# WGLab/NanoRepeat

Measured on NVIDIA B200. Metric: GCUPS, higher is better.
Workload: dtype u16x2 (2*score + mark + 64 per half, two reads per word); s32 (score*65536 - span) for reads > 384 bases

## Files before the change

### nanorepeat_b200/csrc/nr_api.cu

```cuda
#include "nr_batch.h"

#include <algorithm>
#if defined(__x86_64__)
#include <tmmintrin.h>
#endif
#include <atomic>
#include <cstdarg>
#include <cstdio>
#include <cstdlib>
#include <cstring>
#include <mutex>
#include <new>
#include <string>
#include <thread>
#include <memory>
#include <unordered_map>
#include <vector>

using namespace nrh;

namespace {

thread_local std::string g_err;
thread_local int g_code = 0;
thread_local nr_stats_t g_last_stats = {};

}

int nrh::fail(int code, const char* fmt, ...) {
    char buf[512];
    va_list ap;
    va_start(ap, fmt);
    vsnprintf(buf, sizeof buf, fmt, ap);
    va_end(ap);
    g_err = buf;
    g_code = code;
    return code;
}

namespace {

#define CUDA_TRY(expr)                                                                          \
    do {                                                                                        \
        cudaError_t e__ = (expr);                                                               \
        if (e__ != cudaSuccess)                                                                 \
            return fail(NR_ERR_CUDA, "%s failed: %s (%s:%d)", #expr, cudaGetErrorString(e__),   \
                        __FILE__, __LINE__);                                                    \
    } while (0)

using nr::kWarpsPerBlock;

enum BufKind { BUF_DEV = 0, BUF_PIN = 1, BUF_SCRATCH = 2 };
struct BufCache {
    std::unordered_map<size_t, std::vector<void*>> free_dev, free_pin, free_scratch;
    std::unordered_map<void*, long long> scratch_era;
    std::unordered_map<size_t, std::vector<void*>>& of(int kind) { return kind == BUF_PIN ? free_pin : kind == BUF_SCRATCH ? free_scratch : free_dev; }
    static size_t klass(size_t bytes) {
        size_t c = 4096;
        while (c < bytes) c <<= 1;
        return c;
    }
};

struct Context {
    bool ready = false;
    int device = -1;
    int sm_count = 0;
    int clock_khz = 0;
    cudaStream_t stream = nullptr;
    BufCache cache;
};
Context g_ctx;
std::mutex g_ctx_mu;
std::atomic<int> g_ladder_mode{3};
std::atomic<long long> g_launch_no{0};
constexpr long long kEpochs = 1023;
std::atomic<int> g_timing{0};

int ensure_init(int device) {
    std::lock_guard<std::mutex> lk(g_ctx_mu);
    if (g_ctx.ready) {
        if (device >= 0 && device != g_ctx.device)
            return fail(NR_ERR_ARG, "the library is already initialised on device %d (requested %d); call nr_shutdown() first",
                        g_ctx.device, device);
        cudaSetDevice(g_ctx.device);
        return NR_OK;
    }
    if (device < 0) {
        const char* e = getenv("NR_DEVICE");
        if (!e) e = getenv("LOCAL_RANK");
        device = e ? atoi(e) : 0;
    }
    int n = 0;
    cudaError_t err = cudaGetDeviceCount(&n);
    if (err != cudaSuccess || n == 0)
        return fail(NR_ERR_CUDA, "no CUDA device available (%s); libnanorepeat_b200 has no CPU fallback",
                    err == cudaSuccess ? "device count 0" : cudaGetErrorString(err));
    if (device >= n)
        return fail(NR_ERR_ARG, "device %d requested but only %d CUDA device(s) are visible", device, n);
    CUDA_TRY(cudaSetDevice(device));
    cudaDeviceProp prop;
    CUDA_TRY(cudaGetDeviceProperties(&prop, device));
    if (prop.major < 10)
        return fail(NR_ERR_CUDA, "device %d (%s, sm_%d%d) is not a Blackwell sm_100 part", device, prop.name,
                    prop.major, prop.minor);
    CUDA_TRY(cudaStreamCreateWithFlags(&g_ctx.stream, cudaStreamNonBlocking));
    g_ctx.device = device;
    g_ctx.sm_count = prop.multiProcessorCount;
    g_ctx.clock_khz = prop.clockRate;
    g_ctx.ready = true;
    return NR_OK;
}

void trim_cache_locked() {
    for (auto& kv : g_ctx.cache.free_dev) for (void* p : kv.second) cudaFree(p);
    for (auto& kv : g_ctx.cache.free_scratch) for (void* p : kv.second) { cudaFree(p); g_ctx.cache.scratch_era.erase(p); }
    for (auto& kv : g_ctx.cache.free_pin) for (void* p : kv.second) cudaFreeHost(p);
    g_ctx.cache.free_dev.clear(); g_ctx.cache.free_scratch.clear(); g_ctx.cache.free_pin.clear();
}

int cached_alloc(void** p, size_t bytes, int kind) {
    const size_t k = BufCache::klass(bytes);
    {
        std::lock_guard<std::mutex> lk(g_ctx_mu);
        auto& fl = g_ctx.cache.of(kind)[k];
        if (!fl.empty()) { *p = fl.back(); fl.pop_back(); return NR_OK; }
    }
    auto raw = [&]() { return kind == BUF_PIN ? cudaMallocHost(p, k) : cudaMalloc(p, k); };
    cudaError_t e = raw();
    if (e != cudaSuccess) {
        cudaGetLastError();
        { std::lock_guard<std::mutex> lk(g_ctx_mu); cudaDeviceSynchronize(); trim_cache_locked(); }
        e = raw();
    }
    if (e != cudaSuccess) {
        cudaGetLastError();
        return fail(NR_ERR_CUDA, "%s of %zu bytes failed: %s", kind == BUF_PIN ? "cudaMallocHost" : "cudaMalloc", k, cudaGetErrorString(e));
    }
    if (kind == BUF_SCRATCH) {
        CUDA_TRY(cudaMemsetAsync(*p, 0, k, g_ctx.stream));
        CUDA_TRY(cudaStreamSynchronize(g_ctx.stream));
        std::lock_guard<std::mutex> lk(g_ctx_mu);
        g_ctx.cache.scratch_era[*p] = g_launch_no.load() / kEpochs;
    }
    return NR_OK;
}

void cached_free(void* p, size_t bytes, int kind) {
    if (!p) return;
    std::lock_guard<std::mutex> lk(g_ctx_mu);
    g_ctx.cache.of(kind)[BufCache::klass(bytes)].push_back(p);
}

struct BadTable {
    uint8_t t[256];
    BadTable() {
        memset(t, 1, sizeof t);
        for (const char* p = "ACGTacgt"; *p; ++p) t[(unsigned char)*p] = 0;
    }
};
const BadTable g_bad;

#if defined(__x86_64__)
__attribute__((target("ssse3"))) inline uint32_t pack16_ssse3(const unsigned char* u, unsigned& bad) {
    const __m128i v = _mm_loadu_si128(reinterpret_cast<const __m128i*>(u));
    const __m128i l = _mm_or_si128(v, _mm_set1_epi8(0x20));
    const __m128i ok = _mm_or_si128(_mm_or_si128(_mm_cmpeq_epi8(l, _mm_set1_epi8('a')), _mm_cmpeq_epi8(l, _mm_set1_epi8('c'))),
                                    _mm_or_si128(_mm_cmpeq_epi8(l, _mm_set1_epi8('g')), _mm_cmpeq_epi8(l, _mm_set1_epi8('t'))));
    bad |= (unsigned)_mm_movemask_epi8(ok) ^ 0xffffu;
    const __m128i c = _mm_and_si128(_mm_srli_epi16(v, 1), _mm_set1_epi8(3));
    const __m128i p = _mm_maddubs_epi16(c, _mm_set1_epi16(0x0104));
    const __m128i q = _mm_madd_epi16(p, _mm_set1_epi32(0x00010010));
    const __m128i r = _mm_shuffle_epi8(q, _mm_set_epi8(-1, -1, -1, -1, -1, -1, -1, -1, -1, -1, -1, -1, 0, 4, 8, 12));
    return (uint32_t)_mm_cvtsi128_si32(r);
}
const bool g_have_ssse3 = __builtin_cpu_supports("ssse3");
#else
const bool g_have_ssse3 = false;
#endif

bool pack_seq(const char* s, int len, uint32_t* w) {
    const unsigned char* u = reinterpret_cast<const unsigned char*>(s);
    unsigned bad = 0;
    int i = 0;
    for (; i + 16 <= len; i += 16) {
#if defined(__x86_64__)
        if (g_have_ssse3) { w[i >> 4] = pack16_ssse3(u + i, bad); continue; }
#endif
        for (int j = 0; j < 16; ++j) bad |= g_bad.t[u[i + j]];
        uint32_t v = 0;
        for (int j = 0; j < 16; ++j) v |= ((u[i + j] >> 1) & 3u) << (30 - 2 * j);
        w[i >> 4] = v;
    }
    if (i < len) {
        uint32_t v = 0;
        for (int j = 0; i + j < len; ++j) {
            bad |= g_bad.t[u[i + j]];
            v |= ((u[i + j] >> 1) & 3u) << (30 - 2 * j);
        }
        w[i >> 4] = v;
    }
    return bad == 0;
}

void ambiguity_plane(const char* s, int len, uint32_t* m) {
    for (int i = 0; i < len; ++i)
        if (g_bad.t[(unsigned char)s[i]]) m[i >> 5] |= 1u << (i & 31);
}

template <class F>
void parallel_for(int n, int grain, F fn) {
    static const int share = [] { const char* e = getenv("LOCAL_WORLD_SIZE"); return e && atoi(e) > 0 ? atoi(e) : 1; }();
    int nt = (int)std::min<unsigned>(std::max(1u, std::thread::hardware_concurrency() / (unsigned)share), 8u);
    nt = std::min(nt, std::max(1, n / std::max(1, grain)));
    if (nt <= 1) { for (int i = 0; i < n; ++i) fn(i); return; }
    std::vector<std::thread> th;
    th.reserve(nt - 1);
    auto body = [&](int t) { for (int i = (int)((long long)n * t / nt), e = (int)((long long)n * (t + 1) / nt); i < e; ++i) fn(i); };
    for (int t = 1; t < nt; ++t) th.emplace_back(body, t);
    body(0);
    for (auto& x : th) x.join();
}


int exact_smem_int4(int R) { return 4 * ((R + 3) / 4) * 32; }
int ladder_smem_int4(int R) { return exact_smem_int4(R) + R * 32; }
int pair_ladder_smem_int4(int pair_R, int rest_R) { return std::max(exact_smem_int4(pair_R) + 3 * pair_R * 8, rest_R ? ladder_smem_int4(rest_R) : 0); }

int check_scoring(const nr_scoring_t* sc) {
    if (!sc) return fail(NR_ERR_ARG, "scoring is NULL");
    if (sc->match <= 0 || sc->mismatch < 0 || sc->gap_open1 < 0 || sc->gap_ext1 <= 0 || sc->gap_open2 < 0 ||
        sc->gap_ext2 <= 0)
        return fail(NR_ERR_ARG, "scoring values out of range");
    if (sc->ambiguous < 0 || sc->ambiguous > 4096) return fail(NR_ERR_ARG, "scoring values out of range");
    if (sc->gap_open1 + sc->gap_ext1 > 4096 || sc->gap_open2 + sc->gap_ext2 > 4096 || sc->mismatch > 4096 ||
        sc->match > 4096)
        return fail(NR_ERR_ARG, "scoring values too large for the packed kernels");
    return NR_OK;
}

nr::ScoreW score_words(const nr_scoring_t& sc) {
    nr::ScoreW k;
    k.sub_match = (sc.match << 16) - 1;
    k.sub_mismatch = -(sc.mismatch << 16) - 1;
    k.sub_amb = -(sc.ambiguous << 16) - 1;
    k.h_open1 = -((sc.gap_open1 + sc.gap_ext1) << 16) - 1;
    k.h_ext1 = -(sc.gap_ext1 << 16) - 1;
    k.h_open2 = -((sc.gap_open2 + sc.gap_ext2) << 16) - 1;
    k.h_ext2 = -(sc.gap_ext2 << 16) - 1;
    k.v_open1 = -((sc.gap_open1 + sc.gap_ext1) << 16);
    k.v_ext1 = -(sc.gap_ext1 << 16);
    k.v_open2 = -((sc.gap_open2 + sc.gap_ext2) << 16);
    k.v_ext2 = -(sc.gap_ext2 << 16);
    k.refund1 = sc.gap_open1 << 16;
    k.refund2 = sc.gap_open2 << 16;
    k.one = 1;
    k.mone = -1;
    k.four = 4u;
    k.min_score = std::max(1, sc.min_dp_score);
    return k;
}

int upload_batch(nr_batch* b) {
    PhaseTrace trace;
    int rc;
    if ((rc = cached_alloc(&b->d_blob, b->blob_bytes, BUF_DEV))) return rc;
    if ((rc = cached_alloc(&b->h_blob, b->blob_bytes, BUF_PIN))) return rc;
    if ((rc = cached_alloc((void**)&b->d_out, b->out_bytes, BUF_DEV))) return rc;
    if ((rc = cached_alloc((void**)&b->h_out, b->out_bytes, BUF_PIN))) return rc;
    if (b->scratch_bytes && (rc = cached_alloc((void**)&b->d_scratch, b->scratch_bytes, BUF_SCRATCH))) return rc;
    if (b->flags_bytes && (rc = cached_alloc((void**)&b->d_flags, b->flags_bytes, BUF_DEV))) return rc;
    if (b->state_bytes && (rc = cached_alloc((void**)&b->d_state, b->state_bytes, BUF_DEV))) return rc;
    if (b->round2_exit &&
        (rc = cached_alloc((void**)&b->d_kept, sizeof(uint32_t) * 128 * kWarpsPerBlock * (size_t)g_ctx.sm_count, BUF_DEV))) return rc;
    if (b->flag) {
        if ((rc = cached_alloc((void**)&b->d_sel, b->sel_bytes, BUF_DEV))) return rc;
        if ((rc = cached_alloc((void**)&b->h_sel, b->sel_bytes, BUF_PIN))) return rc;
    }
    if (!b->pairs3.empty()) {
        if ((rc = cached_alloc((void**)&b->d_prung, b->prung_bytes, BUF_DEV))) return rc;
        if ((rc = cached_alloc((void**)&b->d_redo, b->redo_bytes, BUF_DEV))) return rc;
        if ((rc = cached_alloc((void**)&b->h_redo_count, 64, BUF_PIN))) return rc;
        b->h_redo_count[0] = b->h_redo_count[1] = 0;
    }
    trace.mark("buffers (cached alloc)");
    char* h = static_cast<char*>(b->h_blob);
    char* d = static_cast<char*>(b->d_blob);
    for (const Section& s : b->blob) {
        if (s.bytes) memcpy(h + s.off, s.src, s.bytes);
        memset(h + s.off + s.bytes, 0, s.zeros);
    }
    memset(h + b->blob_bytes - 256, 0, 256);
    b->d_tasks = reinterpret_cast<nr::Task*>(d + b->blob[SEC_TASKS].off);
    b->d_ltasks = reinterpret_cast<nr::LadderTask*>(d + b->blob[SEC_TASKS].off);
    b->d_lregs = reinterpret_cast<nr::LadderRegion*>(d + b->blob[SEC_LREGS].off);
    b->d_order = reinterpret_cast<int32_t*>(d + b->blob[SEC_ORDER].off);
    b->d_pairs = d + b->blob[SEC_PAIRS].off;
    b->d_coop = reinterpret_cast<nr::CoopInfo*>(d + b->blob[SEC_COOP].off);
    b->d_coop_idx = reinterpret_cast<int32_t*>(d + b->blob[SEC_COOP_IDX].off);
    b->d_pool = reinterpret_cast<uint32_t*>(d + b->blob[SEC_POOL].off);
    b->d_counters = reinterpret_cast<int*>(d + b->blob_bytes - 256);
    trace.mark("blob staging (memcpy)");
    cudaStream_t st = g_ctx.stream;
    CUDA_TRY(cudaMemcpyAsync(d, h, b->blob_bytes, cudaMemcpyHostToDevice, st));
    CUDA_TRY(cudaMemsetAsync(b->d_out, 0, b->out_bytes, st));
    if (b->d_sel) CUDA_TRY(cudaMemsetAsync(b->d_sel, 0, b->sel_bytes, st));
    CUDA_TRY(cudaEventRecord(b->ev_uploaded, st));
    trace.mark("upload + memsets (async)");
    b->committed = true;
    return NR_OK;
}

int commit_batch(nr_batch* b) {
    const int rc = plan_batch(b, g_ctx.sm_count);
    return rc ? rc : upload_batch(b);
}

constexpr int kSpinSlot = 16;

int rest_args(nr_batch* b, const int32_t* order, int count, cudaStream_t st, nr::RestArgs* out) {
    nr::RestArgs ra;
    ra.order = order; ra.n_order = count;
    ra.scratch = b->d_scratch; ra.coop = b->d_coop; ra.coop_idx = b->d_coop_idx; ra.flags = b->d_flags;
    ra.spin = b->d_counters + kSpinSlot;
    ra.redo_long = b->d_redo ? b->d_redo + b->ltasks.size() : nullptr;
    ra.redo_long_count = b->d_counters + 4;
    const long long no = g_launch_no.fetch_add(1);
    ra.epoch = (int)(no % kEpochs) + 1;
    if (b->d_scratch) {
        bool stale;
        {
            std::lock_guard<std::mutex> lk(g_ctx_mu);
            long long& era = g_ctx.cache.scratch_era[b->d_scratch];
            stale = era != no / kEpochs;
            era = no / kEpochs;
        }
        if (stale) CUDA_TRY(cudaMemsetAsync(b->d_scratch, 0, b->scratch_bytes, st));
    }
    *out = ra;
    return NR_OK;
}

int launch_rest(nr_batch* b, cudaStream_t st, const nr::ScoreW& k, const int32_t* order, int count, int blocks,
                int R, const int* count_dev, int* counter) {
    const Launch& L = b->launch;
    nr::RestArgs ra;
    int rc;
    if ((rc = rest_args(b, order, count, st, &ra))) return rc;
    if (L.ladder) {
        if (!L.fixed) return fail(NR_ERR_ARG, "the ladder kernels are built for map-ont scoring only");
        const int stride = ladder_smem_int4(R);
        int wpb = kWarpsPerBlock;
        while (wpb > 4 && (size_t)wpb * stride * sizeof(int4) > nrl::kMaxDynShared) wpb -= 4;
        const size_t smem = (size_t)wpb * stride * sizeof(int4);
        if (smem > nrl::kMaxDynShared) return fail(NR_ERR_ARG, "launch needs %zu bytes of shared memory", smem);
        CUDA_TRY(nrl::launch_ladder(b->flag, blocks, wpb * 32, smem, st, b->d_ltasks, ra, count_dev,
                                    b->qsrc ? b->qsrc->d_pool : b->d_pool, b->d_pool, b->d_lregs, k, counter, stride, b->d_out, b->d_sel));
    } else {
        const int stride = exact_smem_int4(R);
        const size_t smem = (size_t)kWarpsPerBlock * stride * sizeof(int4);
        if (smem > nrl::kMaxDynShared) return fail(NR_ERR_ARG, "launch needs %zu bytes of shared memory", smem);
        CUDA_TRY(nrl::launch_exact(L.fixed, blocks, kWarpsPerBlock * 32, smem, st, b->d_tasks, ra, b->d_pool, k, counter, stride, b->d_out));
    }
    return NR_OK;
}

thread_local cudaStream_t t_aux_stream = nullptr;
cudaStream_t aux_stream_for(const nr_batch* b) {
    static const bool off = getenv("NR_ONE_STREAM") != nullptr;
    if (off || !b->coop.empty()) return nullptr;
    if (!t_aux_stream && cudaStreamCreateWithFlags(&t_aux_stream, cudaStreamNonBlocking) != cudaSuccess) {
        cudaGetLastError();
        t_aux_stream = nullptr;
    }
    return t_aux_stream;
}

int run_batch(nr_batch* b, cudaStream_t st) {
    if (!b->committed) return fail(NR_ERR_ARG, "batch was not committed");
    b->run_stream = st;
    const Launch& L = b->launch;
    const nr::ScoreW k = score_words(b->sc);
    if (st != g_ctx.stream) {
        CUDA_TRY(cudaStreamWaitEvent(st, b->ev_uploaded, 0));
        if (b->qsrc) CUDA_TRY(cudaStreamWaitEvent(st, b->qsrc->ev_uploaded, 0));
    }
    bool resumes = false;
    for (const nr::pr::Pair3& p : b->pairs3) resumes = resumes || p.state_off >= 0;
    if (resumes) {
        if (!b->qsrc->ran) return fail(NR_ERR_ARG, "nr_batch_run: the round-2 batch this round-3 batch resumes from has not been run");
        if (b->qsrc->run_stream != st) CUDA_TRY(cudaStreamWaitEvent(st, b->qsrc->ev_done, 0));
    }
    CUDA_TRY(cudaMemsetAsync(b->d_counters, 0, 32 * sizeof(int), st));
    if (b->flags_bytes) CUDA_TRY(cudaMemsetAsync(b->d_flags, 0, b->flags_bytes, st));
    int launches = 0;
    int rc;
    const bool timing = g_timing.load() != 0;
    if (timing)
        for (cudaEvent_t& e : b->ev_t)
            if (!e) CUDA_TRY(cudaEventCreate(&e));
    b->timed[0] = b->timed[1] = b->timed[2] = false;
    auto mark = [&](int i, cudaStream_t s) { return timing ? cudaEventRecord(b->ev_t[i], s) : cudaSuccess; };
    if (L.n_pairs || b->n_long_pairs) {
        const bool ladder_batch = L.ladder;
        nr::RestArgs ra;
        if ((rc = rest_args(b, b->d_order, L.count, st, &ra))) return rc;
        int wpb = kWarpsPerBlock;
        if (const char* e = getenv("NR_WPB")) wpb = std::max(4, std::min(kWarpsPerBlock, atoi(e)));
        const int blocks = std::max(1, std::min(g_ctx.sm_count, L.count + L.n_pairs));
        nr::pr::Deal deal = nr::pr::make_deal(L.count, L.n_pairs, wpb, blocks);
        if (getenv("NR_PLAIN_DEAL")) deal.nb_long = -1;
        CUDA_TRY(mark(2, st));
        if (!ladder_batch) {
            const int stride = std::max(exact_smem_int4(std::max(L.pair_R, L.R)),
                                        b->round2_exit ? exact_smem_int4(L.pair_R) + 3 * L.pair_R * 8 : 0);
            const size_t smem = (size_t)wpb * stride * sizeof(int4);
            if (smem > nrl::kMaxDynShared) return fail(NR_ERR_ARG, "launch needs %zu bytes of shared memory", smem);
            CUDA_TRY(nrl::launch_pair_round2(blocks, wpb * 32, smem, st, static_cast<const nr::pr::Pair2*>(b->d_pairs), deal, b->d_tasks,
                                             ra, b->d_pool, k, b->d_counters, stride, b->d_out, b->d_state, b->d_kept));
        } else {
            const int stride = pair_ladder_smem_int4(L.pair_R, L.R);
            const size_t smem = (size_t)wpb * stride * sizeof(int4);
            if (smem > nrl::kMaxDynShared) return fail(NR_ERR_ARG, "launch needs %zu bytes of shared memory", smem);
            CUDA_TRY(nrl::launch_pair_ladder(blocks, wpb * 32, smem, st, static_cast<const nr::pr::Pair3*>(b->d_pairs), deal, b->d_ltasks,
                                             ra, b->qsrc ? b->qsrc->d_pool : b->d_pool, b->d_pool, b->d_lregs, k, b->d_counters, stride,
                                             b->d_prung, b->d_out, b->d_sel, b->d_counters + 2, b->d_redo,
                                             b->qsrc ? b->qsrc->d_state : nullptr));
        }
        CUDA_TRY(cudaGetLastError());
        CUDA_TRY(mark(3, st));
        b->timed[1] = timing;
        ++launches;
        if (!b->pairs3.empty()) {
            CUDA_TRY(mark(4, st));
            if ((rc = launch_rest(b, st, k, b->d_redo, 0, std::max(1, std::min(g_ctx.sm_count, 2 * L.n_pairs)), L.redo_R,
                                  b->d_counters + 2, b->d_counters + 3))) return rc;
            CUDA_TRY(mark(5, st));
            b->timed[2] = timing;
            CUDA_TRY(cudaMemcpyAsync(b->h_redo_count, b->d_counters + 2, sizeof(int), cudaMemcpyDeviceToHost, st));
            CUDA_TRY(cudaMemcpyAsync(b->h_redo_count + 1, b->d_counters + 4, sizeof(int), cudaMemcpyDeviceToHost, st));
            ++launches;
        }
    } else if (L.count) {
        CUDA_TRY(mark(0, st));
        if ((rc = launch_rest(b, st, k, b->d_order, L.count, L.blocks, L.R, nullptr, b->d_counters))) return rc;
        CUDA_TRY(mark(1, st));
        b->timed[0] = timing;
        ++launches;
    }
    if (b->flag) {
        if (b->n_reads) CUDA_TRY(cudaMemcpyAsync(b->h_sel, b->d_sel, sizeof(int4) * b->n_reads, cudaMemcpyDeviceToHost, st));
    } else if (b->n_out) {
        CUDA_TRY(cudaMemcpyAsync(b->h_out, b->d_out, sizeof(int4) * b->n_out, cudaMemcpyDeviceToHost, st));
    }
    if (b->flags_bytes) {
        if (!b->h_spin) { int rc2 = cached_alloc((void**)&b->h_spin, 64, BUF_PIN); if (rc2) return rc2; }
        CUDA_TRY(cudaMemcpyAsync(b->h_spin, b->d_counters + kSpinSlot, sizeof(int), cudaMemcpyDeviceToHost, st));
    }
    CUDA_TRY(cudaEventRecord(b->ev_done, st));
    b->stats.kernel_launches = launches;
    b->long_redone = false;
    b->ran = true;
    return NR_OK;
}

int redo_long_reads(nr_batch* b);

int fetch_raw(nr_batch* b) {
    if (!b->ran) return fail(NR_ERR_ARG, "batch was not run");
    CUDA_TRY(cudaEventSynchronize(b->ev_done));
    if (b->h_spin && *b->h_spin)
        return fail(NR_ERR_CUDA, "a stripe of a long read gave up waiting for the stripe above it; the results of this batch are not valid");
    if (b->n_long_pairs && b->h_redo_count && b->h_redo_count[1] > 0 && !b->long_redone) return redo_long_reads(b);
    return NR_OK;
}

int add_seq(nr_batch* b, const char* s, int len, const char* what, int idx, uint32_t* word, bool ambiguous_ok = false) {
    if (!s && len > 0) return fail(NR_ERR_ARG, "%s %d is NULL", what, idx);
    if (len < 0) return fail(NR_ERR_ARG, "%s %d has negative length", what, idx);
    long long w = b->pool.add(s, len, ambiguous_ok);
    if (w < 0) return fail(NR_ERR_BAD_BASE, "%s %d contains a character other than ACGT", what, idx);
    if (w > 0xfffffff0LL || b->pool.words.size() > 0xfffffff0ULL) return fail(NR_ERR_TOO_LARGE, "sequence pool exceeds 2^32 words");
    *word = (uint32_t)w;
    return NR_OK;
}

struct ReadSrc {
    const char* const* cores;
    const int32_t* core_len;
    const char* concat;
    const int64_t* off;
    int gap;
    const char* ptr(int r) const { return cores ? cores[r] : concat + off[r]; }
    long long len(int r) const { return cores ? (long long)core_len[r] : (long long)(off[r + 1] - off[r] - gap); }
};

inline bool is_blank(char c) { return c == ' ' || c == '\n' || c == '\r' || c == '\t'; }

int add_reads(nr_batch* b, const ReadSrc& src, int n_reads, std::vector<uint32_t>& q_word, std::vector<int32_t>& q_len) {
    q_word.resize(n_reads);
    q_len.resize(n_reads);
    std::vector<const char*> ptr(n_reads);
    size_t w = b->pool.words.size();
    const size_t w0 = w;
    for (int r = 0; r < n_reads; ++r) {
        long long len = src.len(r);
        if (len < 0 || len > 0x7fffffffLL) return fail(NR_ERR_ARG, "core %d has a bad length", r);
        const char* p = src.ptr(r);
        if (len > 0 && !p) return fail(NR_ERR_ARG, "core %d is NULL", r);
        while (len > 0 && is_blank(p[len - 1])) --len;
        while (len > 0 && is_blank(*p)) { ++p; --len; }
        if (w > 0xfffffff0ULL) return fail(NR_ERR_TOO_LARGE, "sequence pool exceeds 2^32 words");
        ptr[r] = p;
        q_len[r] = (int32_t)len;
        q_word[r] = (uint32_t)w;
        w += (size_t)(len + 15) / 16 + 1;
    }
    b->pool.words.resize(w, 0u);
    uint32_t* words = b->pool.words.data();
    std::vector<uint8_t> amb(n_reads, 0);
    static const int kPackGrain = [] { const char* e = getenv("NR_PACK_GRAIN"); return e && atoi(e) > 0 ? atoi(e) : 8192; }();
    parallel_for(n_reads, kPackGrain, [&](int r) { amb[r] = !pack_seq(ptr[r], q_len[r], words + q_word[r]); });
    for (int r = 0; r < n_reads; ++r)
        if (amb[r]) {
            b->pool.link_plane(q_word[r], ptr[r], q_len[r]);
            ++b->n_ambiguous_reads;
        }
    if (b->pool.words.size() > 0xfffffff0ULL) { b->pool.words.resize(w0); return fail(NR_ERR_TOO_LARGE, "sequence pool exceeds 2^32 words"); }
    return NR_OK;
}

int add_round2(nr_batch* b, const char* left, int32_t n_left, const char* motif, int32_t motif_len, int32_t T,
               int32_t n_reads, const ReadSrc& src) {
    if (!b || b->kind != KIND_ROUND2 || b->committed) return fail(NR_ERR_ARG, "not an open round-2 batch");
    if (n_left < 0 || motif_len <= 0 || T < 0 || n_reads < 0 || !motif || (n_left > 0 && !left))
        return fail(NR_ERR_ARG, "nr_batch_add_round2: bad arguments");
    const size_t pool0 = b->pool.words.size();
    std::string tpl(left ? left : "", (size_t)n_left);
    tpl.reserve((size_t)n_left + (size_t)motif_len * T);
    for (int k = 0; k < T; ++k) tpl.append(motif, (size_t)motif_len);
    uint32_t tw = 0;
    int rc;
    bool bad_template = false;
    if ((rc = add_seq(b, tpl.data(), (int)tpl.size(), "round-2 template", 0, &tw))) {
        if (rc != NR_ERR_BAD_BASE) return rc;
        bad_template = true;
    }
    RegionInfo g;
    g.n_left = n_left; g.motif_len = motif_len; g.first_read = b->n_reads; g.n_reads = n_reads;
    g.left.assign(left ? left : "", (size_t)n_left);
    g.motif.assign(motif, (size_t)motif_len);
    b->regions.push_back(g);
    const size_t base = b->tasks.size();
    b->tasks.resize(base + n_reads);
    std::vector<uint32_t> qw;
    std::vector<int32_t> ql;
    if ((rc = add_reads(b, src, n_reads, qw, ql))) {
        b->tasks.resize(base);
        b->regions.pop_back();
        b->pool.words.resize(pool0);
        return rc;
    }
    for (int r = 0; r < n_reads; ++r) {
        nr::Task& t = b->tasks[base + r];
        t.q_word = qw[r];
        t.q_len = ql[r];
        t.t_word = tw;
        t.t_len = bad_template ? -1 : (int)tpl.size();
    }
    b->n_reads += n_reads;
    return NR_OK;
}

int add_round3_impl(nr_batch* b, const char* left, int32_t n_left, const char* right, int32_t n_right, const char* motif,
                    int32_t motif_len, int32_t n_reads, const ReadSrc& src, const int32_t* kmin, const int32_t* kmax,
                    const nr::Task* reuse) {
    for (int r = 0; r < n_reads; ++r)
        if (kmin[r] < 0) return fail(NR_ERR_ARG, "kmin[%d] < 0", r);
    if (b->flag && 2 * (long long)n_right > 65534)
        return fail(NR_ERR_TOO_LARGE, "right anchor of %d bases exceeds the flag ladder's range (32767); use nr_set_ladder_mode(1)", n_right);
    if (reuse && !b->ladder)
        return fail(NR_ERR_ARG, "reads of a round-2 batch can only be reused by the ladder kernels (nr_set_ladder_mode 1 or 2)");
    RegionInfo g;
    g.n_left = n_left; g.n_right = n_right; g.motif_len = motif_len; g.first_read = b->n_reads; g.n_reads = n_reads;
    const int region = (int)b->regions.size();
    b->regions.push_back(g);
    if (b->rung_off.empty()) b->rung_off.push_back(0);
    int klo = INT32_MAX, khi = -1;
    for (int r = 0; r < n_reads; ++r) {
        const long long n = kmax[r] >= kmin[r] ? (long long)kmax[r] - kmin[r] + 1 : 0;
        b->rung_off.push_back(b->rung_off.back() + n);
        b->kmin.push_back(kmin[r]);
        b->kmax.push_back(kmax[r]);
        b->read_region.push_back(region);
        if (n) { klo = std::min(klo, kmin[r]); khi = std::max(khi, kmax[r]); }
    }
    if (b->rung_off.back() > 0x7fffffffLL) return fail(NR_ERR_TOO_LARGE, "more than 2^31 rungs in one batch");
    const int first = b->n_reads;
    b->n_reads += n_reads;
    b->n_out = (size_t)b->rung_off.back();
    const int64_t* roff = b->rung_off.data() + first;
    int rc;
    bool bad_template = false;
    std::vector<uint32_t> qw;
    std::vector<int32_t> ql;
    if (b->ladder) {
        nr::LadderRegion lr = {};
        lr.n_left = n_left; lr.n_right = n_right; lr.m = motif_len;
        std::string fwd(left ? left : "", (size_t)n_left);
        for (int u = 0; u < std::max(khi, 0); ++u) fwd.append(motif, (size_t)motif_len);
        std::string rev(right ? right : "", (size_t)n_right);
        std::reverse(rev.begin(), rev.end());
        if ((rc = add_seq(b, fwd.data(), (int)fwd.size(), "ladder prefix", 0, &lr.fwd_word)) ||
            (rc = add_seq(b, rev.data(), (int)rev.size(), "right anchor", 0, &lr.rev_word))) {
            if (rc != NR_ERR_BAD_BASE) return rc;
            bad_template = true;
        }
        const int lreg = (int)b->lregs.size();
        b->lregs.push_back(lr);
        if (!reuse && (rc = add_reads(b, src, n_reads, qw, ql))) return rc;
        for (int r = 0; r < n_reads; ++r) {
            if (roff[r + 1] == roff[r]) continue;
            if (bad_template) { ++b->n_skipped; continue; }
            nr::LadderTask t = {};
            if (reuse) { t.q_word = reuse[r].q_word; t.q_len = reuse[r].q_len; }
            else { t.q_word = qw[r]; t.q_len = ql[r]; }
            if (t.q_len == 0) continue;
            t.kmin = kmin[r];
            t.kmax = kmax[r];
            t.out_off = (int32_t)roff[r];
            t.region = lreg;
            t.read = first + r;
            b->ltasks.push_back(t);
            b->lt_src.push_back(reuse ? (int32_t)(reuse - b->qsrc->tasks.data()) + r : -1);
        }
        return NR_OK;
    }
    std::vector<uint32_t> tpl_word;
    if (khi >= klo) {
        std::vector<uint8_t> used(khi - klo + 1, 0);
        for (int r = 0; r < n_reads; ++r)
            for (int k = kmin[r]; k <= kmax[r]; ++k) used[k - klo] = 1;
        tpl_word.assign(khi - klo + 1, 0);
        std::string tpl;
        for (int k = klo; k <= khi && !bad_template; ++k) {
            if (!used[k - klo]) continue;
            tpl.assign(left ? left : "", (size_t)n_left);
            for (int u = 0; u < k; ++u) tpl.append(motif, (size_t)motif_len);
            tpl.append(right ? right : "", (size_t)n_right);
            if ((rc = add_seq(b, tpl.data(), (int)tpl.size(), "ladder template", k, &tpl_word[k - klo]))) {
                if (rc != NR_ERR_BAD_BASE) return rc;
                bad_template = true;
            }
        }
    }
    if ((rc = add_reads(b, src, n_reads, qw, ql))) return rc;
    b->tasks.resize(b->n_out);
    for (int r = 0; r < n_reads; ++r) {
        for (int k = kmin[r]; k <= kmax[r]; ++k) {
            nr::Task& t = b->tasks[(size_t)(roff[r] + (k - kmin[r]))];
            t.q_word = qw[r];
            t.q_len = ql[r];
            t.t_word = bad_template ? 0u : tpl_word[k - klo];
            t.t_len = bad_template ? -1 : n_left + motif_len * k + n_right;
        }
    }
    return NR_OK;
}

int add_round3(nr_batch* b, const char* left, int32_t n_left, const char* right, int32_t n_right, const char* motif,
               int32_t motif_len, int32_t n_reads, const ReadSrc& src, const int32_t* kmin, const int32_t* kmax,
               const nr::Task* reuse = nullptr) {
    if (!b || b->kind != KIND_ROUND3 || b->committed) return fail(NR_ERR_ARG, "not an open round-3 batch");
    if (n_left < 0 || n_right < 0 || motif_len <= 0 || n_reads < 0 || !motif || (n_left > 0 && !left) ||
        (n_right > 0 && !right) || (n_reads > 0 && (!kmin || !kmax)))
        return fail(NR_ERR_ARG, "nr_batch_add_round3: bad arguments");
    const size_t n_regions = b->regions.size(), n_roff = b->rung_off.size(), n_k = b->kmin.size(), n_rr = b->read_region.size(),
                 n_lregs = b->lregs.size(), n_lt = b->ltasks.size(), n_src = b->lt_src.size(), n_tasks = b->tasks.size(),
                 n_words = b->pool.words.size(), n_out = b->n_out;
    const int n_reads0 = b->n_reads, n_skipped0 = b->n_skipped, n_amb0 = b->n_ambiguous_reads;
    const int rc = add_round3_impl(b, left, n_left, right, n_right, motif, motif_len, n_reads, src, kmin, kmax, reuse);
    if (rc) {
        b->regions.resize(n_regions); b->rung_off.resize(n_roff); b->kmin.resize(n_k); b->kmax.resize(n_k);
        b->read_region.resize(n_rr); b->lregs.resize(n_lregs); b->ltasks.resize(n_lt); b->lt_src.resize(n_src);
        b->tasks.resize(n_tasks); b->pool.words.resize(n_words);
        b->n_out = n_out; b->n_reads = n_reads0; b->n_skipped = n_skipped0; b->n_ambiguous_reads = n_amb0;
    }
    return rc;
}

void free_events(nr_batch* b) {
    for (cudaEvent_t* e : {&b->ev_uploaded, &b->ev_done, &b->ev_t[0], &b->ev_t[1], &b->ev_t[2],
                           &b->ev_t[3], &b->ev_t[4], &b->ev_t[5]})
        if (*e) { cudaEventDestroy(*e); *e = nullptr; }
}

nr_batch* new_batch(const nr_scoring_t* sc, BatchKind kind) {
    if (check_scoring(sc)) return nullptr;
    if (ensure_init(-1)) return nullptr;
    nr_batch* b = new (std::nothrow) nr_batch();
    if (!b) { fail(NR_ERR_NOMEM, "out of host memory"); return nullptr; }
    if (cudaEventCreateWithFlags(&b->ev_uploaded, cudaEventDisableTiming) != cudaSuccess ||
        cudaEventCreateWithFlags(&b->ev_done, cudaEventDisableTiming) != cudaSuccess) {
        fail(NR_ERR_CUDA, "cudaEventCreate failed");
        free_events(b);
        delete b;
        return nullptr;
    }
    b->kind = kind;
    b->sc = *sc;
    const int mode = is_map_ont(*sc) ? g_ladder_mode.load() : 0;
    b->ladder = kind == KIND_ROUND3 && mode != 0;
    b->flag = kind == KIND_ROUND3 && mode >= 2;
    b->pair = kind == KIND_ROUND3 && mode == 3;
    return b;
}

int redo_long_reads(nr_batch* b) {
    const int cnt = b->h_redo_count[1];
    std::vector<int32_t> tids((size_t)cnt);
    cudaStream_t st = b->run_stream ? b->run_stream : g_ctx.stream;
    CUDA_TRY(cudaMemcpyAsync(tids.data(), b->d_redo + b->ltasks.size(), sizeof(int32_t) * (size_t)cnt, cudaMemcpyDeviceToHost, st));
    CUDA_TRY(cudaStreamSynchronize(st));
    nr_batch* t = new_batch(&b->sc, KIND_ROUND3);
    if (!t) return g_code;
    t->ladder = true; t->flag = true; t->pair = false;
    t->qsrc = b->qsrc;
    if (t->qsrc) ++t->qsrc->refs;
    t->pool.words = b->pool.words;
    t->lregs = b->lregs;
    t->regions = b->regions;
    t->rung_off.push_back(0);
    for (int j = 0; j < cnt; ++j) {
        if (tids[j] < 0 || tids[j] >= (int)b->ltasks.size()) { nr_batch_destroy(t); return fail(NR_ERR_CUDA, "corrupt redo list"); }
        nr::LadderTask lt = b->ltasks[tids[j]];
        lt.read = j;
        lt.out_off = (int32_t)t->rung_off.back();
        lt.pad = 0;
        t->ltasks.push_back(lt);
        t->lt_src.push_back(-1);
        t->rung_off.push_back(t->rung_off.back() + (lt.kmax - lt.kmin + 1));
        t->kmin.push_back(lt.kmin); t->kmax.push_back(lt.kmax);
        t->read_region.push_back(0);
    }
    t->n_reads = cnt;
    t->n_out = (size_t)t->rung_off.back();
    int rc = commit_batch(t);
    if (!rc) rc = run_batch(t, st);
    if (!rc) rc = fetch_raw(t);
    if (!rc)
        for (int j = 0; j < cnt; ++j) b->h_sel[b->ltasks[tids[j]].read] = t->h_sel[j];
    nr_batch_destroy(t);
    if (!rc) b->long_redone = true;
    return rc;
}

}

extern "C" {

int nr_get_preset(const char* data_type, nr_scoring_t* out) {
    if (!data_type || !out) return fail(NR_ERR_ARG, "nr_get_preset: NULL argument");
    static const char* names[] = {"ont", "ont_sup", "ont_q20", "clr", "hifi"};
    for (const char* n : names) {
        if (strcmp(n, data_type) == 0) {
            nr_scoring_t s = {2, 4, 4, 2, 24, 1, 1, 80};
            *out = s;
            return NR_OK;
        }
    }
    return fail(NR_ERR_UNKNOWN_TYPE, "Unknown data type: %s", data_type);
}

int nr_init(int device) { return ensure_init(device); }

int nr_shutdown(void) {
    std::lock_guard<std::mutex> lk(g_ctx_mu);
    if (g_ctx.ready) {
        trim_cache_locked();
        cudaStreamDestroy(g_ctx.stream);
        g_ctx = Context();
    }
    return NR_OK;
}

const char* nr_last_error(void) { return g_err.c_str(); }

int nr_device_info(int32_t* device, int32_t* sm_count, int32_t* clock_khz) {
    int rc = ensure_init(-1);
    if (rc) return rc;
    if (device) *device = g_ctx.device;
    if (sm_count) *sm_count = g_ctx.sm_count;
    if (clock_khz) *clock_khz = g_ctx.clock_khz;
    return NR_OK;
}

int nr_set_ladder_mode(int mode) {
    if (mode < 0 || mode > 3) return fail(NR_ERR_ARG, "nr_set_ladder_mode: mode must be 0, 1, 2 or 3");
    g_ladder_mode.store(mode);
    return NR_OK;
}

int nr_limits(int32_t* max_score, int32_t* max_tlen) {
    if (max_score) *max_score = kMaxScore;
    if (max_tlen) *max_tlen = kMaxTlen;
    return NR_OK;
}

void nr_batch_destroy(nr_batch_t* b) {
    if (!b) return;
    if (--b->refs > 0) return;
    if (b->committed && b->ev_uploaded) cudaEventSynchronize(b->ev_uploaded);
    if (b->ran && b->ev_done) cudaEventSynchronize(b->ev_done);
    else if (b->ran && b->run_stream) cudaStreamSynchronize(b->run_stream);
    cached_free(b->d_blob, b->blob_bytes, BUF_DEV);
    cached_free(b->h_blob, b->blob_bytes, BUF_PIN);
    cached_free(b->d_out, b->out_bytes, BUF_DEV);
    cached_free(b->h_out, b->out_bytes, BUF_PIN);
    cached_free(b->d_scratch, b->scratch_bytes, BUF_SCRATCH);
    cached_free(b->d_flags, b->flags_bytes, BUF_DEV);
    cached_free(b->d_state, b->state_bytes, BUF_DEV);
    if (b->d_kept) cached_free(b->d_kept, sizeof(uint32_t) * 128 * kWarpsPerBlock * (size_t)g_ctx.sm_count, BUF_DEV);
    cached_free(b->d_sel, b->sel_bytes, BUF_DEV);
    cached_free(b->h_sel, b->sel_bytes, BUF_PIN);
    cached_free(b->d_prung, b->prung_bytes, BUF_DEV);
    cached_free(b->d_redo, b->redo_bytes, BUF_DEV);
    cached_free(b->h_redo_count, 64, BUF_PIN);
    cached_free(b->h_spin, 64, BUF_PIN);
    nr_batch* src = b->qsrc;
    free_events(b);
    delete b;
    if (src) nr_batch_destroy(src);
}

nr_batch_t* nr_batch_begin_round3_from(nr_batch_t* round2) {
    if (!round2 || round2->kind != KIND_ROUND2 || !round2->committed) {
        fail(NR_ERR_ARG, "nr_batch_begin_round3_from: needs a committed round-2 batch");
        return nullptr;
    }
    nr_batch* b = new_batch(&round2->sc, KIND_ROUND3);
    if (!b) return nullptr;
    if (!b->ladder) {
        fail(NR_ERR_ARG, "nr_batch_begin_round3_from: needs a ladder mode (nr_set_ladder_mode 1 or 2)");
        free_events(b);
        delete b;
        return nullptr;
    }
    b->qsrc = round2;
    ++round2->refs;
    return b;
}

int nr_batch_add_round3_reuse(nr_batch_t* b, int32_t region_index, const char* right, int32_t n_right,
                              const int32_t* kmin, const int32_t* kmax) {
    if (!b || !b->qsrc) return fail(NR_ERR_ARG, "nr_batch_add_round3_reuse: batch was not begun with nr_batch_begin_round3_from");
    const nr_batch* src = b->qsrc;
    if (region_index < 0 || region_index >= (int)src->regions.size())
        return fail(NR_ERR_ARG, "nr_batch_add_round3_reuse: region %d is not in the round-2 batch", region_index);
    const RegionInfo& g = src->regions[region_index];
    ReadSrc none = {nullptr, nullptr, nullptr, nullptr, 0};
    return add_round3(b, g.left.data(), g.n_left, right, n_right, g.motif.data(), g.motif_len, g.n_reads, none, kmin, kmax,
                      src->tasks.data() + g.first_read);
}

nr_batch_t* nr_batch_begin(const nr_scoring_t* sc, int32_t kind) {
    if (kind != NR_KIND_ROUND2 && kind != NR_KIND_ROUND3 && kind != NR_KIND_ROUND2_FLAGS) {
        fail(NR_ERR_ARG, "nr_batch_begin: kind must be NR_KIND_ROUND2, NR_KIND_ROUND2_FLAGS or NR_KIND_ROUND3");
        return nullptr;
    }
    nr_batch* b = new_batch(sc, kind == NR_KIND_ROUND3 ? KIND_ROUND3 : KIND_ROUND2);
    if (b && kind == NR_KIND_ROUND2_FLAGS) b->r2flags = b->pair = true;
    return b;
}

int nr_batch_add_round2(nr_batch_t* b, const char* left, int32_t n_left, const char* motif, int32_t motif_len,
                        int32_t T, int32_t n_reads, const char* cores_concat, const int64_t* core_off) {
    if (n_reads > 0 && (!cores_concat || !core_off)) return fail(NR_ERR_ARG, "nr_batch_add_round2: NULL reads");
    ReadSrc src = {nullptr, nullptr, cores_concat, core_off, 0};
    return add_round2(b, left, n_left, motif, motif_len, T, n_reads, src);
}

int nr_batch_add_round2_lines(nr_batch_t* b, const char* left, int32_t n_left, const char* motif, int32_t motif_len,
                              int32_t T, int32_t n_reads, const char* lines, int64_t lines_len) {
    if (n_reads < 0 || lines_len < 0 || (n_reads > 0 && !lines)) return fail(NR_ERR_ARG, "nr_batch_add_round2_lines: bad arguments");
    std::vector<int64_t> off;
    if (n_reads > 0) {
        off.reserve((size_t)n_reads + 1);
        int64_t pos = 0;
        for (;;) {
            off.push_back(pos);
            const char* nl = pos < lines_len ? static_cast<const char*>(memchr(lines + pos, '\n', (size_t)(lines_len - pos))) : nullptr;
            if (!nl) break;
            pos = nl - lines + 1;
        }
        off.push_back(lines_len + 1);
        if ((int64_t)off.size() != (int64_t)n_reads + 1)
            return fail(NR_ERR_BAD_BASE, "nr_batch_add_round2_lines: %lld lines for %d reads (a core holds a newline?)",
                        (long long)off.size() - 1, n_reads);
    }
    ReadSrc src = {nullptr, nullptr, lines, off.data(), 1};
    return add_round2(b, left, n_left, motif, motif_len, T, n_reads, src);
}

int nr_batch_add_round3(nr_batch_t* b, const char* left, int32_t n_left, const char* right, int32_t n_right,
                        const char* motif, int32_t motif_len, int32_t n_reads, const char* cores_concat,
                        const int64_t* core_off, const int32_t* kmin, const int32_t* kmax) {
    if (n_reads > 0 && (!cores_concat || !core_off)) return fail(NR_ERR_ARG, "nr_batch_add_round3: NULL reads");
    if (b && b->qsrc) return fail(NR_ERR_ARG, "nr_batch_add_round3: this batch reuses a round-2 batch's reads (nr_batch_add_round3_reuse)");
    ReadSrc src = {nullptr, nullptr, cores_concat, core_off, 0};
    return add_round3(b, left, n_left, right, n_right, motif, motif_len, n_reads, src, kmin, kmax);
}

int nr_batch_commit(nr_batch_t* b) {
    if (!b || b->committed) return fail(NR_ERR_ARG, "nr_batch_commit: NULL or already committed batch");
    return commit_batch(b);
}

nr_batch_t* nr_batch_create_tasks(const nr_scoring_t* sc, int32_t n_tasks, const char* const* queries,
                                  const int32_t* qlen, const char* const* targets, const int32_t* tlen) {
    if (n_tasks < 0 || (n_tasks > 0 && (!queries || !qlen || !targets || !tlen))) {
        fail(NR_ERR_ARG, "nr_batch_create_tasks: bad arguments");
        return nullptr;
    }
    nr_batch* b = new_batch(sc, KIND_TASKS);
    if (!b) return nullptr;
    b->tasks.resize(n_tasks);
    std::unordered_map<const char*, std::pair<int, uint32_t>> seen;
    for (int i = 0; i < n_tasks; ++i) {
        nr::Task& t = b->tasks[i];
        t.q_len = qlen[i];
        t.t_len = tlen[i];
        const char* ptrs[2] = {queries[i], targets[i]};
        const int lens[2] = {qlen[i], tlen[i]};
        uint32_t words[2];
        for (int s = 0; s < 2; ++s) {
            auto it = seen.find(ptrs[s]);
            if (it != seen.end() && it->second.first == lens[s]) { words[s] = it->second.second; continue; }
            const int rc = add_seq(b, ptrs[s], lens[s], s ? "target" : "query", i, &words[s], s == 0);
            if (rc == NR_ERR_BAD_BASE && s == 1) { words[1] = 0; t.t_len = -1; continue; }
            if (rc) { nr_batch_destroy(b); return nullptr; }
            seen[ptrs[s]] = std::make_pair(lens[s], words[s]);
        }
        t.q_word = words[0];
        t.t_word = words[1];
    }
    if (commit_batch(b)) { nr_batch_destroy(b); return nullptr; }
    return b;
}

nr_batch_t* nr_batch_create_round2(const nr_scoring_t* sc, const char* left, int32_t n_left, const char* motif,
                                   int32_t motif_len, int32_t T, int32_t n_reads, const char* const* cores,
                                   const int32_t* core_len) {
    if (n_reads > 0 && (!cores || !core_len)) { fail(NR_ERR_ARG, "nr_batch_create_round2: NULL reads"); return nullptr; }
    nr_batch* b = new_batch(sc, KIND_ROUND2);
    if (!b) return nullptr;
    ReadSrc src = {cores, core_len, nullptr, nullptr, 0};
    if (add_round2(b, left, n_left, motif, motif_len, T, n_reads, src) || commit_batch(b)) { nr_batch_destroy(b); return nullptr; }
    return b;
}

nr_batch_t* nr_batch_create_round3(const nr_scoring_t* sc, const char* left, int32_t n_left, const char* right,
                                   int32_t n_right, const char* motif, int32_t motif_len, int32_t n_reads,
                                   const char* const* cores, const int32_t* core_len, const int32_t* kmin,
                                   const int32_t* kmax) {
    if (n_reads > 0 && (!cores || !core_len)) { fail(NR_ERR_ARG, "nr_batch_create_round3: NULL reads"); return nullptr; }
    nr_batch* b = new_batch(sc, KIND_ROUND3);
    if (!b) return nullptr;
    ReadSrc src = {cores, core_len, nullptr, nullptr, 0};
    if (add_round3(b, left, n_left, right, n_right, motif, motif_len, n_reads, src, kmin, kmax) || commit_batch(b)) {
        nr_batch_destroy(b);
        return nullptr;
    }
    return b;
}

int nr_batch_run(nr_batch_t* b, void* stream) {
    if (!b) return fail(NR_ERR_ARG, "nr_batch_run: NULL batch");
    return run_batch(b, stream ? (cudaStream_t)stream : g_ctx.stream);
}

int nr_batch_fetch_alns(nr_batch_t* b, nr_aln_t* out) {
    if (!b || (!out && b->n_out)) return fail(NR_ERR_ARG, "nr_batch_fetch_alns: NULL argument");
    if (b->flag) return fail(NR_ERR_ARG, "nr_batch_fetch_alns: a flag-ladder batch has no (tstart, tend) records; use nr_batch_fetch_round3 or nr_set_ladder_mode(1)");
    if (b->r2flags) return fail(NR_ERR_ARG, "nr_batch_fetch_alns: a NR_KIND_ROUND2_FLAGS batch has no tstart; use nr_batch_fetch_round2");
    int rc = fetch_raw(b);
    if (rc) return rc;
    for (size_t i = 0; i < b->n_out; ++i) {
        out[i].score = b->h_out[i].x;
        out[i].tstart = b->h_out[i].y;
        out[i].tend = b->h_out[i].z;
    }
    return NR_OK;
}

int nr_batch_fetch_round2(nr_batch_t* b, int32_t* score, int32_t* tend, uint8_t* starts_by_left) {
    if (!b || b->kind != KIND_ROUND2) return fail(NR_ERR_ARG, "nr_batch_fetch_round2: not a round-2 batch");
    if (b->n_out && (!score || !tend || !starts_by_left)) return fail(NR_ERR_ARG, "nr_batch_fetch_round2: NULL output");
    int rc = fetch_raw(b);
    if (rc) return rc;
    for (const RegionInfo& g : b->regions)
        for (int r = g.first_read; r < g.first_read + g.n_reads; ++r) {
            const int4 a = b->h_out[r];
            score[r] = a.x;
            tend[r] = a.z;
            starts_by_left[r] = a.y <= g.n_left;
        }
    return NR_OK;
}

int nr_batch_fetch_round3(nr_batch_t* b, const int64_t* rung_offset, nr_rung_t* rungs, int64_t* sum_k,
                          int32_t* n_k, int32_t* top_score) {
    if (!b || b->kind != KIND_ROUND3) return fail(NR_ERR_ARG, "nr_batch_fetch_round3: not a round-3 batch");
    if (b->n_reads > 0 && (!sum_k || !n_k || !top_score)) return fail(NR_ERR_ARG, "nr_batch_fetch_round3: NULL output");
    if (rungs && !rung_offset) return fail(NR_ERR_ARG, "rungs given without rung_offset");
    if (rungs && b->pair) return fail(NR_ERR_ARG, "nr_batch_fetch_round3: the paired ladder (mode 3) keeps no rung records; use nr_set_ladder_mode(2)");
    if (b->flag) {
        int rc0 = fetch_raw(b);
        if (rc0) return rc0;
        if (rungs && b->n_out) {
            cudaStream_t st = b->run_stream ? b->run_stream : g_ctx.stream;
            CUDA_TRY(cudaMemcpyAsync(b->h_out, b->d_out, sizeof(int4) * b->n_out, cudaMemcpyDeviceToHost, st));
            CUDA_TRY(cudaStreamSynchronize(st));
        }
        for (int r = 0; r < b->n_reads; ++r) {
            const int4 v = b->h_sel[r];
            top_score[r] = v.x;
            n_k[r] = v.y;
            sum_k[r] = (int64_t)(((uint64_t)(uint32_t)v.w << 32) | (uint32_t)v.z);
        }
        if (rungs) {
            for (int r = 0; r < b->n_reads; ++r) {
                const int64_t o = b->rung_off[r];
                const int n = (int)(b->rung_off[r + 1] - o);
                for (int i = 0; i < n; ++i) {
                    const int4 a = b->h_out[o + i];
                    nr_rung_t& rg = rungs[rung_offset[r] + i];
                    rg.score = a.x;
                    rg.starts_in_left = a.y != 0;
                    rg.ends_in_right = a.z != 0;
                    rg.pad[0] = rg.pad[1] = 0;
                }
            }
        }
        b->stats.d2h_bytes = (int64_t)sizeof(int4) * (b->n_reads + (rungs ? (int64_t)b->n_out : 0));
        return NR_OK;
    }
    int rc = fetch_raw(b);
    if (rc) return rc;
    const int min_score = std::max(1, b->sc.min_dp_score);
    for (int r = 0; r < b->n_reads; ++r) {
        const RegionInfo& g = b->regions[b->read_region[r]];
        const int64_t o = b->rung_off[r];
        const int n = (int)(b->rung_off[r + 1] - o);
        int top = 0;
        for (int i = 0; i < n; ++i) {
            int s = b->h_out[o + i].x;
            if (s >= min_score && s > top) top = s;
        }
        int64_t sum = 0;
        int cnt = 0;
        for (int i = 0; i < n; ++i) {
            const int4 a = b->h_out[o + i];
            const int k = b->kmin[r] + i;
            const int tlen = g.n_left + g.motif_len * k + g.n_right;
            const bool in_right = a.x > 0 && tlen - a.z < g.n_right;
            const bool in_left = in_right && a.y < g.n_left;
            if (rungs) {
                nr_rung_t& rg = rungs[rung_offset[r] + i];
                rg.score = a.x;
                rg.starts_in_left = in_left;
                rg.ends_in_right = in_right;
                rg.pad[0] = rg.pad[1] = 0;
            }
            if (top > 0 && a.x == top && in_left) { sum += k; ++cnt; }
        }
        sum_k[r] = sum;
        n_k[r] = cnt;
        top_score[r] = top;
    }
    return NR_OK;
}

int nr_set_timing(int on) {
    g_timing.store(on ? 1 : 0);
    return NR_OK;
}

int nr_batch_launch_info(nr_batch_t* b, nr_launch_info_t* out) {
    if (!b || !out) return fail(NR_ERR_ARG, "nr_batch_launch_info: NULL argument");
    if (!b->committed) return fail(NR_ERR_ARG, "nr_batch_launch_info: batch was not committed");
    *out = {};
    out->paired_cells = out->planned_paired_cells = b->paired_cells;
    out->rest_cells = b->rest_cells;
    out->paired_useful_cells = out->planned_paired_useful_cells = b->paired_useful;
    out->rest_useful_cells = b->rest_useful;
    out->n_pairs = b->launch.n_pairs;
    out->n_rest = b->launch.count;
    if (b->ran) {
        CUDA_TRY(cudaEventSynchronize(b->ev_done));
        if (b->round2_exit) {
            unsigned long long skipped[2];
            CUDA_TRY(cudaMemcpy(skipped, b->d_counters + nr::pr::kExitSlot, sizeof(skipped), cudaMemcpyDeviceToHost));
            out->paired_cells -= 2 * (int64_t)skipped[0];
            out->paired_useful_cells -= (int64_t)(skipped[1] / 32);
        }
        if (b->h_redo_count) out->n_redo = *b->h_redo_count;
        if (b->timed[0]) CUDA_TRY(cudaEventElapsedTime(&out->rest_ms, b->ev_t[0], b->ev_t[1]));
        if (b->timed[1]) CUDA_TRY(cudaEventElapsedTime(&out->paired_ms, b->ev_t[2], b->ev_t[3]));
        if (b->timed[2]) CUDA_TRY(cudaEventElapsedTime(&out->redo_ms, b->ev_t[4], b->ev_t[5]));
    }
    return NR_OK;
}

int nr_batch_stats(const nr_batch_t* b, nr_stats_t* out) {
    if (!b || !out) return fail(NR_ERR_ARG, "nr_batch_stats: NULL argument");
    *out = b->stats;
    return NR_OK;
}

int nr_last_stats(nr_stats_t* out) {
    if (!out) return fail(NR_ERR_ARG, "nr_last_stats: NULL argument");
    *out = g_last_stats;
    return NR_OK;
}

int nr_score_tasks(const nr_scoring_t* sc, int32_t n_tasks, const char* const* queries, const int32_t* qlen,
                   const char* const* targets, const int32_t* tlen, nr_aln_t* out) {
    if (n_tasks > 0 && !out) return fail(NR_ERR_ARG, "nr_score_tasks: out is NULL");
    nr_batch_t* b = nr_batch_create_tasks(sc, n_tasks, queries, qlen, targets, tlen);
    if (!b) return g_code;
    int rc = nr_batch_run(b, nullptr);
    if (!rc) rc = nr_batch_fetch_alns(b, out);
    g_last_stats = b->stats;
    nr_batch_destroy(b);
    return rc;
}

int nr_round2_region(const nr_scoring_t* sc, const char* left, int32_t n_left, const char* motif,
                     int32_t motif_len, int32_t T, int32_t n_reads, const char* const* cores,
                     const int32_t* core_len, nr_aln_t* out) {
    if (n_reads > 0 && !out) return fail(NR_ERR_ARG, "nr_round2_region: out is NULL");
    nr_batch_t* b = nr_batch_create_round2(sc, left, n_left, motif, motif_len, T, n_reads, cores, core_len);
    if (!b) return g_code;
    int rc = nr_batch_run(b, nullptr);
    if (!rc) rc = nr_batch_fetch_alns(b, out);
    g_last_stats = b->stats;
    nr_batch_destroy(b);
    return rc;
}

int nr_round3_region(const nr_scoring_t* sc, const char* left, int32_t n_left, const char* right, int32_t n_right,
                     const char* motif, int32_t motif_len, int32_t n_reads, const char* const* cores,
                     const int32_t* core_len, const int32_t* kmin, const int32_t* kmax,
                     const int64_t* rung_offset, nr_rung_t* rungs, int64_t* sum_k, int32_t* n_k,
                     int32_t* top_score) {
    nr_batch_t* b = nr_batch_create_round3(sc, left, n_left, right, n_right, motif, motif_len, n_reads, cores,
                                           core_len, kmin, kmax);
    if (!b) return g_code;
    int rc = nr_batch_run(b, nullptr);
    if (!rc) rc = nr_batch_fetch_round3(b, rung_offset, rungs, sum_k, n_k, top_score);
    g_last_stats = b->stats;
    nr_batch_destroy(b);
    return rc;
}

}

namespace {

struct Group {
    int r0, r1;
    nr_batch* b2 = nullptr;
    nr_batch* b3 = nullptr;
    std::vector<int> regs;
    int rc = NR_OK;
    std::string err;
};

int host_threads() {
    static const int share = [] { const char* e = getenv("LOCAL_WORLD_SIZE"); return e && atoi(e) > 0 ? atoi(e) : 1; }();
    return (int)std::max(1u, std::thread::hardware_concurrency() / (unsigned)share);
}

int estimate_regions(const nr_scoring_t* sc, int fast_mode, int n_regions, const nr_region_t* regs, double* r1, double* r2,
                     uint8_t* r2_valid, double* r3, uint8_t* r3_state, int32_t* T_out, nr_stats_t* stats) {
    std::vector<long long> first(n_regions + 1, 0);
    for (int g = 0; g < n_regions; ++g) {
        const nr_region_t& R = regs[g];
        if (R.n_reads < 0 || R.motif_len <= 0 || !R.motif || (R.n_reads > 0 && (!R.reads || !R.dist_between_anchors)))
            return fail(NR_ERR_ARG, "nr_estimate_regions: region %d has bad arguments", g);
        first[g + 1] = first[g] + R.n_reads;
    }
    const long long total = first[n_regions];
    for (long long i = 0; i < total; ++i) { r2_valid[i] = 0; r3_state[i] = 0; r2[i] = 0.0; r3[i] = 0.0; }
    std::vector<int32_t> T(n_regions, 0);
    for (int g = 0; g < n_regions; ++g) {
        const nr_region_t& R = regs[g];
        if (R.n_reads == 0) continue;
        const double m = (double)R.motif_len;
        double mx = 0.0;
        for (int r = 0; r < R.n_reads; ++r) {
            const double v = (double)R.dist_between_anchors[r] / m;
            r1[first[g] + r] = v;
            if (r == 0 || v > mx) mx = v;
        }
        if (R.has_round1_max_dist) { const double v = (double)R.round1_max_dist / m; if (v > mx) mx = v; }
        int t = (int)(mx * 1.5) + 1;
        if ((double)t < mx + 10.0) t = (int)(mx + 10.0);
        if (t < 0) t = 0;
        T[g] = t;
        if (T_out) T_out[g] = t;
    }
    long long kMinReads = total >= 12288 ? 16384 : 4096;
    if (const char* e = getenv("NR_GROUP_READS")) kMinReads = std::max(256, atoi(e));
    long long total_bases = 0;
    for (int g = 0; g < n_regions; ++g) total_bases += regs[g].reads_len;
    const bool long_reads = total > 0 && total_bases / total > 1000;
    const int n_groups = long_reads ? 1 : (int)std::max<long long>(1, std::min<long long>(8, total / kMinReads));
    std::vector<Group> groups;
    {
        const double target = (double)total / n_groups;
        long long acc = 0;
        int start = 0;
        for (int g = 0; g < n_regions; ++g) {
            acc += regs[g].n_reads;
            if (acc >= target * (double)(groups.size() + 1) && (int)groups.size() < n_groups - 1) {
                Group G; G.r0 = start; G.r1 = g + 1; groups.push_back(G);
                start = g + 1;
            }
        }
        Group G; G.r0 = start; G.r1 = n_regions; groups.push_back(G);
    }
    int rc = NR_OK;
    auto cleanup = [&]() { for (Group& G : groups) { if (G.b3) nr_batch_destroy(G.b3); if (G.b2) nr_batch_destroy(G.b2); G.b2 = G.b3 = nullptr; } };
    auto add_stats = [&](const nr_batch* b) {
        if (!stats) return;
        stats->algorithmic_cells += b->stats.algorithmic_cells; stats->executed_cells += b->stats.executed_cells;
        stats->n_tasks += b->stats.n_tasks; stats->kernel_launches += b->stats.kernel_launches;
        stats->n_skipped += b->stats.n_skipped; stats->h2d_bytes += b->stats.h2d_bytes; stats->d2h_bytes += b->stats.d2h_bytes;
    };
    if (stats) *stats = {};
    const int min_score = std::max(1, sc->min_dp_score);
    PhaseTrace trace;
    trace.mark("estimate: round 1, grouping");
    for (Group& G : groups) {
        long long bases = 0;
        for (int g = G.r0; g < G.r1; ++g)
            if (regs[g].n_reads > 0) { G.regs.push_back(g); bases += regs[g].reads_len + regs[g].n_left + (long long)regs[g].motif_len * T[g]; }
        if (G.regs.empty()) continue;
        if (!(G.b2 = nr_batch_begin(sc, NR_KIND_ROUND2_FLAGS))) { cleanup(); return g_code; }
        G.b2->pool.words.reserve((size_t)(bases / 16 + 2 * (long long)G.regs.size() + 64));
        long long n_reads = 0;
        for (int g : G.regs) n_reads += regs[g].n_reads;
        G.b2->pool.words.reserve((size_t)(bases / 16 + 2 * n_reads + 4 * (long long)G.regs.size() + 64));
        G.b2->tasks.reserve((size_t)n_reads);
    }
    static const long long kPackJobReads = [] { const char* e = getenv("NR_PACK_JOB_READS"); return e && atoi(e) > 0 ? (long long)atoi(e) : 4096LL; }();
    struct Job { Group* G; size_t i0, i1; std::unique_ptr<nr_batch> part; int rc = NR_OK; std::string err; };
    std::vector<Job> jobs;
    {
        const int nt_all = host_threads();
        for (Group& G : groups) {
            if (!G.b2) continue;
            long long n_reads = 0;
            for (int g : G.regs) n_reads += regs[g].n_reads;
            const int parts = (int)std::max<long long>(1, std::min<long long>(std::min<long long>(nt_all, 16), n_reads / kPackJobReads));
            const double per = (double)n_reads / parts;
            long long acc = 0;
            size_t start = 0;
            int made = 0;
            for (size_t i = 0; i < G.regs.size(); ++i) {
                acc += regs[G.regs[i]].n_reads;
                if (made < parts - 1 && acc >= per * (made + 1)) { jobs.push_back({&G, start, i + 1, nullptr}); start = i + 1; ++made; }
            }
            if (start < G.regs.size()) jobs.push_back({&G, start, G.regs.size(), nullptr});
        }
        auto pack_job = [&](Job& J) {
            J.part.reset(new (std::nothrow) nr_batch());
            if (!J.part) { J.rc = NR_ERR_NOMEM; J.err = "out of host memory"; return; }
            nr_batch* pb = J.part.get();
            pb->kind = KIND_ROUND2;
            pb->sc = *sc;
            long long bases = 0, n_reads = 0;
            for (size_t i = J.i0; i < J.i1; ++i) {
                const nr_region_t& R = regs[J.G->regs[i]];
                bases += R.reads_len + R.n_left + (long long)R.motif_len * T[J.G->regs[i]];
                n_reads += R.n_reads;
            }
            pb->pool.words.reserve((size_t)(bases / 16 + 2 * n_reads + 4 * (long long)(J.i1 - J.i0) + 64));
            pb->tasks.reserve((size_t)n_reads);
            for (size_t i = J.i0; i < J.i1; ++i) {
                const int g = J.G->regs[i];
                const nr_region_t& R = regs[g];
                const int rc1 = nr_batch_add_round2_lines(pb, R.left, R.n_left, R.motif, R.motif_len, T[g], R.n_reads, R.reads, R.reads_len);
                if (rc1) { J.rc = rc1; J.err = g_err; return; }
            }
        };
        const int nt = std::min<int>((int)jobs.size(), nt_all);
        if (nt <= 1) {
            for (Job& J : jobs) pack_job(J);
        } else {
            std::atomic<int> next{0};
            auto work = [&]() { for (int i; (i = next.fetch_add(1)) < (int)jobs.size();) pack_job(jobs[i]); };
            std::vector<std::thread> th;
            for (int t = 1; t < nt; ++t) th.emplace_back(work);
            work();
            for (auto& x : th) x.join();
        }
        for (Job& J : jobs) {
            Group& G = *J.G;
            if (G.rc) continue;
            if (J.rc) { G.rc = J.rc; G.err = J.err; continue; }
            nr_batch* pb = J.part.get();
            nr_batch* b = G.b2;
            const size_t base_w = b->pool.words.size();
            if (base_w + pb->pool.words.size() > 0xfffffff0ULL) { G.rc = NR_ERR_TOO_LARGE; G.err = "sequence pool exceeds 2^32 words"; continue; }
            b->pool.words.insert(b->pool.words.end(), pb->pool.words.begin(), pb->pool.words.end());
            const size_t base_t = b->tasks.size();
            b->tasks.insert(b->tasks.end(), pb->tasks.begin(), pb->tasks.end());
            for (size_t t = base_t; t < b->tasks.size(); ++t) { b->tasks[t].q_word += (uint32_t)base_w; b->tasks[t].t_word += (uint32_t)base_w; }
            for (RegionInfo& ri : pb->regions) { ri.first_read += b->n_reads; b->regions.push_back(std::move(ri)); }
            b->n_reads += pb->n_reads;
            b->n_ambiguous_reads += pb->n_ambiguous_reads;
            J.part.reset();
        }
    }
    trace.mark("estimate: round-2 add (pack, threads)");
    for (Group& G : groups) {
        if (G.rc) { const int rc1 = G.rc; const std::string msg = G.err; cleanup(); return fail(rc1, "%s", msg.c_str()); }
        if (G.b2 && ((rc = nr_batch_commit(G.b2)) || (rc = nr_batch_run(G.b2, aux_stream_for(G.b2))))) { cleanup(); return rc; }
        trace.mark("estimate: round-2 commit + run");
    }
    std::vector<int32_t> kmin, kmax;
    for (Group& G : groups) {
        if (!G.b2) continue;
        if ((rc = fetch_raw(G.b2))) { cleanup(); return rc; }
        trace.mark("estimate: wait for round 2");
        if (!(G.b3 = nr_batch_begin_round3_from(G.b2))) { cleanup(); return g_code; }
        for (size_t i = 0; i < G.regs.size(); ++i) {
            const int g = G.regs[i];
            const nr_region_t& R = regs[g];
            const RegionInfo& info = G.b2->regions[i];
            const double m = (double)R.motif_len;
            kmin.assign(R.n_reads, 0);
            kmax.assign(R.n_reads, -1);
            for (int r = 0; r < R.n_reads; ++r) {
                const int4 a = G.b2->h_out[info.first_read + r];
                if (a.x < min_score || a.y > R.n_left || a.z < R.n_left) continue;
                const double v = (double)(a.z - R.n_left) / m;
                r2[first[g] + r] = v;
                r2_valid[first[g] + r] = 1;
                int buffer = std::max(15, (int)(v * 0.05));
                if (buffer > 150) buffer = 150;
                if (fast_mode) buffer = 15;
                kmax[r] = (int)(v + (double)buffer);
                kmin[r] = std::max((int)(v - (double)buffer), 0);
            }
            if ((rc = nr_batch_add_round3_reuse(G.b3, (int)i, R.right, R.n_right, kmin.data(), kmax.data()))) { cleanup(); return rc; }
        }
        trace.mark("estimate: select 2 + round-3 add");
        if ((rc = nr_batch_commit(G.b3)) || (rc = nr_batch_run(G.b3, aux_stream_for(G.b3)))) { cleanup(); return rc; }
        trace.mark("estimate: round-3 commit + run");
    }
    for (Group& G : groups) {
        if (!G.b3) continue;
        if ((rc = fetch_raw(G.b3))) { cleanup(); return rc; }
        trace.mark("estimate: wait for round 3");
        for (size_t i = 0; i < G.regs.size(); ++i) {
            const int g = G.regs[i];
            const RegionInfo& info = G.b3->regions[i];
            for (int r = 0; r < regs[g].n_reads; ++r) {
                const long long o = first[g] + r;
                if (!r2_valid[o]) continue;
                const int4 v = G.b3->h_sel[info.first_read + r];
                if (v.x <= 0) continue;
                if (v.y > 0) {
                    const long long sum = (long long)(((unsigned long long)(unsigned)v.w << 32) | (unsigned)v.z);
                    r3[o] = (double)sum / (double)v.y;
                    r3_state[o] = 1;
                } else {
                    r3[o] = r2[o];
                    r3_state[o] = 2;
                }
            }
        }
        add_stats(G.b2);
        add_stats(G.b3);
    }
    trace.mark("estimate: select 3");
    cleanup();
    trace.mark("estimate: destroy batches");
    return NR_OK;
}

}

extern "C" int nr_estimate_regions(const nr_scoring_t* sc, int32_t fast_mode, int32_t n_regions, const nr_region_t* regions,
                                   double* r1, double* r2, uint8_t* r2_valid, double* r3, uint8_t* r3_state, int32_t* T_out,
                                   nr_stats_t* stats) {
    if (check_scoring(sc)) return g_code;
    if (n_regions < 0 || (n_regions > 0 && !regions)) return fail(NR_ERR_ARG, "nr_estimate_regions: bad arguments");
    long long total = 0;
    for (int g = 0; g < n_regions; ++g) total += std::max(0, regions[g].n_reads);
    if (total > 0 && (!r1 || !r2 || !r2_valid || !r3 || !r3_state)) return fail(NR_ERR_ARG, "nr_estimate_regions: NULL output");
    if (!is_map_ont(*sc) || g_ladder_mode.load() == 0)
        return fail(NR_ERR_ARG, "nr_estimate_regions needs map-ont scoring and a shared-sweep ladder mode (1-3)");
    return estimate_regions(sc, fast_mode, n_regions, regions, r1, r2, r2_valid, r3, r3_state, T_out, stats);
}

namespace nri {
int ensure_init() { return ::ensure_init(-1); }
cudaStream_t stream() { return g_ctx.stream; }
int sm_count() { return g_ctx.sm_count; }
int fail_msg(int code, const char* msg) { return fail(code, "%s", msg); }
int last_code() { return g_code; }
bool pack(const char* s, int len, uint32_t* w) { return pack_seq(s, len, w); }
void ambiguity(const char* s, int len, uint32_t* m) { ambiguity_plane(s, len, m); }
int alloc(void** p, size_t bytes, bool pinned) { return cached_alloc(p, bytes, pinned ? BUF_PIN : BUF_DEV); }
void release(void* p, size_t bytes, bool pinned) { cached_free(p, bytes, pinned ? BUF_PIN : BUF_DEV); }
int check(const nr_scoring_t* sc) { return check_scoring(sc); }
}
```

### nanorepeat_b200/csrc/nr_batch.h

```cpp
#pragma once
#include "nr_internal.h"
#include "nr_launch.h"

#include <chrono>
#include <cmath>
#include <cstdio>
#include <cstdlib>
#include <functional>
#include <string>
#include <thread>
#include <vector>

namespace nrh {

constexpr int kMaxScore = 32767;
constexpr int kMaxTlen = 65535 - 64;

int fail(int code, const char* fmt, ...);

struct Pool {
    std::vector<uint32_t> words;
    long long add(const char* s, int len, bool ambiguous_ok = false) {
        const size_t w0 = words.size();
        const size_t nw = (size_t)(len + 15) / 16 + 1;
        words.resize(w0 + nw, 0u);
        if (!nri::pack(s, len, words.data() + w0)) {
            if (!ambiguous_ok) { words.resize(w0); return -1; }
            link_plane(w0, s, len);
        }
        return (long long)w0;
    }
    void link_plane(size_t w0, const char* s, int len) {
        const size_t at = words.size();
        words.resize(at + (size_t)(len + 31) / 32, 0u);
        nri::ambiguity(s, len, words.data() + at);
        words[w0 + (size_t)(len + 15) / 16] = (uint32_t)(at - w0);
    }
};

struct Launch {
    bool ladder;
    int R;
    int count;
    int blocks;
    bool fixed;
    int n_pairs;
    int pair_R;
    int pair_blocks;
    int redo_R;
};

struct RegionInfo {
    int n_left = 0, n_right = 0, motif_len = 0;
    int first_read = 0, n_reads = 0;
    std::string left, motif;
};

enum BlobSection { SEC_TASKS, SEC_LREGS, SEC_ORDER, SEC_PAIRS, SEC_COOP, SEC_COOP_IDX, SEC_POOL, kBlobSections };
struct Section {
    const void* src;
    size_t bytes, zeros;
    size_t off;
};

enum BatchKind { KIND_TASKS = 0, KIND_ROUND2 = NR_KIND_ROUND2, KIND_ROUND3 = NR_KIND_ROUND3 };

inline size_t align_up(size_t x, size_t a) { return (x + a - 1) / a * a; }

inline bool is_map_ont(const nr_scoring_t& c) {
    return c.match == 2 && c.mismatch == 4 && c.gap_open1 == 4 && c.gap_ext1 == 2 && c.gap_open2 == 24 && c.gap_ext2 == 1 &&
           c.ambiguous == 1;
}

struct PhaseTrace {
    const bool on = getenv("NR_TRACE") != nullptr;
    std::chrono::steady_clock::time_point t0 = std::chrono::steady_clock::now();
    void mark(const char* what) {
        if (!on) return;
        const auto t1 = std::chrono::steady_clock::now();
        fprintf(stderr, "[nr trace] %-28s %8.1f us   (ends at %10.1f us, thread %04x)\n", what,
                std::chrono::duration<double, std::micro>(t1 - t0).count(), std::fmod(std::chrono::duration<double, std::micro>(t1.time_since_epoch()).count(), 1e8),
                (unsigned)(std::hash<std::thread::id>()(std::this_thread::get_id()) & 0xffff));
        t0 = t1;
    }
};

}

struct nr_batch {
    nrh::BatchKind kind = nrh::KIND_TASKS;
    nr_scoring_t sc = {};
    bool committed = false;
    std::vector<nr::Task> tasks;
    std::vector<nr::LadderTask> ltasks;
    std::vector<nr::LadderRegion> lregs;
    bool ladder = false;
    bool flag = false;
    bool pair = false;
    bool r2flags = false;
    std::vector<nr::pr::Pair2> pairs2;
    std::vector<nr::pr::Pair3> pairs3;
    int n_pairs2_single = 0, n_pairs3_single = 0;
    bool long_redone = false;
    int n_long_pairs = 0;
    void* d_pairs = nullptr;
    uint2* d_prung = nullptr;
    size_t prung_bytes = 0;
    int32_t* d_redo = nullptr;
    size_t redo_bytes = 0;
    cudaEvent_t ev_t[6] = {};
    bool timed[3] = {};
    int* h_redo_count = nullptr;
    int* h_spin = nullptr;
    long long paired_cells = 0, rest_cells = 0;
    long long paired_useful = 0, rest_useful = 0;
    bool round2_exit = false;
    size_t n_out = 0;
    std::vector<int32_t> order;
    std::vector<nr::CoopInfo> coop;
    std::vector<int32_t> coop_idx;
    nr::CoopInfo* d_coop = nullptr;
    int32_t* d_coop_idx = nullptr;
    std::vector<int32_t> lt_src;
    uint32_t* d_state = nullptr;
    uint32_t* d_kept = nullptr;
    size_t state_bytes = 0;
    int* d_flags = nullptr;
    size_t flags_bytes = 0;
    nrh::Launch launch = {};
    nrh::Pool pool;
    std::vector<nrh::RegionInfo> regions;
    int n_reads = 0;
    int n_skipped = 0;
    int n_ambiguous_reads = 0;
    std::vector<int32_t> read_region;
    std::vector<int32_t> kmin, kmax;
    std::vector<int64_t> rung_off;
    nrh::Section blob[nrh::kBlobSections] = {};
    void* d_blob = nullptr;
    size_t blob_bytes = 0;
    void* h_blob = nullptr;
    nr::Task* d_tasks = nullptr;
    nr::LadderTask* d_ltasks = nullptr;
    nr::LadderRegion* d_lregs = nullptr;
    int32_t* d_order = nullptr;
    uint32_t* d_pool = nullptr;
    int* d_counters = nullptr;
    int4* d_out = nullptr;
    size_t out_bytes = 0;
    int4* d_scratch = nullptr;
    size_t scratch_bytes = 0;
    int4* h_out = nullptr;
    int4* d_sel = nullptr;
    int4* h_sel = nullptr;
    size_t sel_bytes = 0;
    nr_stats_t stats = {};
    bool ran = false;
    cudaStream_t run_stream = nullptr;
    cudaEvent_t ev_uploaded = nullptr;
    cudaEvent_t ev_done = nullptr;
    int refs = 1;
    nr_batch* qsrc = nullptr;
};

namespace nrh {
int plan_batch(nr_batch* b, int sm_count);
}
```

### nanorepeat_b200/csrc/nr_kernels.cuh

```cuda
#pragma once
#include <cuda_runtime.h>
#include <stdint.h>

namespace nr {

struct Task {
    uint32_t q_word;
    int32_t  q_len;
    uint32_t t_word;
    int32_t  t_len;
};

struct LadderTask {
    uint32_t q_word;
    int32_t  q_len;
    int32_t  kmin, kmax;
    int32_t  out_off;
    int32_t  region;
    int32_t  read;
    int32_t  pad;
};

struct LadderRegion {
    uint32_t fwd_word;
    uint32_t rev_word;
    int32_t  n_left, n_right, m;
};

struct ScoreW {
    int sub_match, sub_mismatch;
    int sub_amb;
    int h_open1, h_ext1, h_open2, h_ext2;
    int v_open1, v_ext1, v_open2, v_ext2;
    int refund1, refund2;
    int one, mone;
    unsigned four;
    int min_score;
};

template <bool FIXED> struct ScoreView;
template <> struct ScoreView<false> : ScoreW {
    __device__ __forceinline__ explicit ScoreView(const ScoreW& w) : ScoreW(w) {}
};
template <> struct ScoreView<true> {
    static constexpr int sub_match = (2 << 16) - 1, sub_mismatch = -(4 << 16) - 1, sub_amb = -(1 << 16) - 1;
    static constexpr int h_open1 = -(6 << 16) - 1, h_ext1 = -(2 << 16) - 1, h_open2 = -(25 << 16) - 1, h_ext2 = -(1 << 16) - 1;
    static constexpr int v_open1 = -(6 << 16), v_ext1 = -(2 << 16), v_open2 = -(25 << 16), v_ext2 = -(1 << 16);
    static constexpr int refund1 = 4 << 16, refund2 = 24 << 16;
    int one, mone;
    unsigned four;
    int min_score;
    __device__ __forceinline__ explicit ScoreView(const ScoreW& w) : one(w.one), mone(w.mone), four(w.four), min_score(w.min_score) {}
};

constexpr int kPadScore = -(16384 << 16);
constexpr unsigned kFull = 0xffffffffu;
constexpr int kExact = 0, kBwd = 1, kFwd = 2;
typedef unsigned long long u64;

__device__ __forceinline__ int w_cap(int w) { return (w + 0xffff) & (int)0xffff0000; }

__device__ __forceinline__ int madd(int a, int mul, int b) {
    int d;
    asm("mad.lo.s32 %0, %1, %2, %3;" : "=r"(d) : "r"(a), "r"(mul), "r"(b));
    return d;
}

template <class SC>
__device__ __forceinline__ void cell_w32(int hd, int dmul, int s, const SC& sc, int& h, int& e1, int& e2, int& f1,
                                         int& f2) {
    const int t = __vimax3_s32(madd(hd, dmul, s), e1, e2);
    h = __vimax3_s32_relu(t, f1, f2);
    e1 = __viaddmax_s32(h, sc.h_open1, madd(e1, sc.one, sc.h_ext1));
    e2 = __viaddmax_s32(h, sc.h_open2, madd(e2, sc.one, sc.h_ext2));
    f1 = __viaddmax_s32(h, sc.v_open1, madd(f1, sc.one, sc.v_ext1));
    f2 = __viaddmax_s32(h, sc.v_open2, madd(f2, sc.one, sc.v_ext2));
}

template <class SC>
__device__ __forceinline__ void jcand(int wf, int wb, const SC& sc, int& bhi, int& blo) {
    const int cf = madd(wf, sc.one, -1) | 0xffff;
    const int khi = madd(cf, sc.one, wb);
    const int klo = madd(cf, sc.mone, wf);
    if (khi > bhi) { bhi = khi; blo = klo; }
    else if (khi == bhi) blo = max(blo, klo);
}
constexpr int kJuncNone = -(3 << 29);
__device__ __forceinline__ void junction_unbias(int& bhi, int& blo) {
    if (bhi == kJuncNone) { bhi = 0; blo = 0; } else { bhi += 1; blo -= 1; }
}

__device__ __forceinline__ u64 key_of_best(int w, int j) {
    if (w <= 0) return 0ull;
    const unsigned cap = (unsigned)w_cap(w);
    const unsigned span = cap - (unsigned)w;
    return ((u64)(cap >> 16) << 32) | ((u64)(0xffffu - (unsigned)j) << 16) | (u64)(0xffffu - span);
}

__device__ __forceinline__ u64 key_of_junction(int khi, int klo) {
    if (khi <= 0) return 0ull;
    const unsigned cap = (unsigned)w_cap(khi);
    const unsigned ext = cap - (unsigned)khi;
    return ((u64)(cap >> 16) << 32) | ((u64)(0xffffu - ext) << 16) | (u64)(0xffffu - (unsigned)(-klo));
}

__device__ __forceinline__ ulonglong2 load_bnd(const ulonglong2* p) {
    ulonglong2 v;
    asm volatile("ld.volatile.global.v2.u64 {%0, %1}, [%2];" : "=l"(v.x), "=l"(v.y) : "l"(p) : "memory");
    return v;
}
__device__ __forceinline__ void store_bnd(ulonglong2* p, int h, int f1, int f2, int tag) {
    const unsigned long long t = (unsigned long long)(unsigned)tag << 48;
    const unsigned long long lo = (unsigned long long)(unsigned)h | ((unsigned long long)((unsigned)f1 & 0xffffu) << 32) | t;
    const unsigned long long hi = (unsigned long long)((unsigned)f1 >> 16) | ((unsigned long long)(unsigned)f2 << 16) | t;
    asm volatile("st.global.cg.v2.u64 [%0], {%1, %2};" :: "l"(p), "l"(lo), "l"(hi) : "memory");
}
__device__ __forceinline__ bool bnd_valid(const ulonglong2& v, int tag) {
    return (int)(v.x >> 48) == tag && (int)(v.y >> 48) == tag;
}
__device__ __forceinline__ int4 unpack_bnd(const ulonglong2& v) {
    return make_int4((int)(unsigned)v.x, (int)((unsigned)(v.x >> 32) & 0xffffu) | (int)((unsigned)v.y << 16), (int)(unsigned)(v.y >> 16), 0);
}
__device__ __forceinline__ ulonglong2 load_tok(const ulonglong2* p) {
    ulonglong2 v;
    asm volatile("ld.volatile.global.v2.u64 {%0, %1}, [%2];" : "=l"(v.x), "=l"(v.y) : "l"(p) : "memory");
    return v;
}
__device__ __forceinline__ int peek_cols(const int* flag) {
    int v;
    asm volatile("ld.acquire.gpu.global.s32 %0, [%1];" : "=r"(v) : "l"(flag) : "memory");
    return v;
}
constexpr int kSpinLimit = 1 << 23;
__device__ __forceinline__ void wait_cols(const int* flag, int need, int lane, int* spin) {
    if (lane == 0)
        for (int tries = 0; peek_cols(flag) < need; ++tries) {
            if (tries > kSpinLimit) { *spin = 1; break; }
            __nanosleep(100);
        }
    __syncwarp();
}

__device__ __forceinline__ u64 shfl_up64(u64 v) {
    unsigned lo = __shfl_up_sync(kFull, (unsigned)v, 1);
    unsigned hi = __shfl_up_sync(kFull, (unsigned)(v >> 32), 1);
    return ((u64)hi << 32) | lo;
}

__device__ __forceinline__ u64 warp_max64(u64 key) {
#pragma unroll
    for (int o = 16; o > 0; o >>= 1) {
        u64 other = __shfl_xor_sync(kFull, key, o);
        key = other > key ? other : key;
    }
    return key;
}

__device__ __forceinline__ int4 finalize_rung(u64 P, u64 J, int c, int r_score, int r_end, int r_start) {
    int bs = 0, be = 0, bst = 0;
    if (P) {
        const int s = (int)(P >> 32), j = 0xffff - (int)((P >> 16) & 0xffffu), span = 0xffff - (int)(P & 0xffffu);
        bs = s; be = j; bst = j - span;
    }
    if (J) {
        const int s = (int)(J >> 32), e = c + 0xffff - (int)((J >> 16) & 0xffffu), st = c - (0xffff - (int)(J & 0xffffu));
        if (s > bs || (s == bs && (e < be || (e == be && st > bst)))) { bs = s; be = e; bst = st; }
    }
    if (r_score > 0) {
        const int e = c + r_end, st = c + r_start;
        if (r_score > bs || (r_score == bs && (e < be || (e == be && st > bst)))) { bs = r_score; be = e; bst = st; }
    }
    return make_int4(bs, bst, be, 0);
}

__device__ __forceinline__ int4 finalize_flag_rung(int P, int J, int rcand) {
    const int np = max(J, rcand);
    const int s_np = np > 0 ? w_cap(np) : 0;
    const int s_p = w_cap(P);
    const int in_right = s_np > s_p;
    return make_int4(max(s_p, s_np) >> 16, in_right & np & 1, in_right, 0);
}

template <int R>
struct StripeCfg {
    static constexpr int CH = (R + 3) / 4;
    static constexpr int PROF_INT4 = 4 * CH * 32;
    static constexpr int BVEC_INT4 = R * 32;
};

__device__ __forceinline__ uint32_t read_ambiguity_plane(const uint32_t* __restrict__ qwords, int q_len) {
    return qwords[(q_len + 15) >> 4];
}
__device__ __forceinline__ bool read_base_ambiguous(const uint32_t* __restrict__ qwords, uint32_t plane, int qi) {
    return (qwords[plane + (qi >> 5)] >> (qi & 31)) & 1u;
}

template <int R, class SC>
__device__ __forceinline__ void build_profile(int4* prof, const uint32_t* __restrict__ qwords, int q_len,
                                              int row0, int lane, const SC& sc, bool reverse) {
    constexpr int CH = StripeCfg<R>::CH;
    int* p = reinterpret_cast<int*>(prof);
    const uint32_t amb = q_len > 0 ? read_ambiguity_plane(qwords, q_len) : 0u;
#pragma unroll
    for (int r = 0; r < 4 * CH; ++r) {
        const int i = row0 + r;
        int code = 4;
        if (r < R && i < q_len) {
            const int qi = reverse ? q_len - 1 - i : i;
            code = (qwords[qi >> 4] >> (30 - 2 * (qi & 15))) & 3;
            if (amb && read_base_ambiguous(qwords, amb, qi)) code = 5;
        }
#pragma unroll
        for (int c = 0; c < 4; ++c) {
            const int v = (code == 4) ? kPadScore : code == 5 ? sc.sub_amb : (code == c ? sc.sub_match : sc.sub_mismatch);
            p[((c * CH + (r >> 2)) * 32 + lane) * 4 + (r & 3)] = v;
        }
    }
}

template <int R>
__device__ __forceinline__ int bvec_pos(int idx0) {
    const int stripe = idx0 / (32 * R), in = idx0 - stripe * (32 * R);
    return stripe * (32 * R) + (in % R) * 32 + in / R;
}

template <class SC, int DEC>
struct ModeScore {
    int sub_match, sub_mismatch, sub_amb, h_open1, h_ext1, h_open2, h_ext2, v_open1, v_ext1, v_open2, v_ext2, one;
    __device__ __forceinline__ explicit ModeScore(const SC& sc)
        : sub_match(sc.sub_match + 1 - DEC), sub_mismatch(sc.sub_mismatch + 1 - DEC), sub_amb(sc.sub_amb + 1 - DEC),
          h_open1(sc.h_open1 + 1 - DEC),
          h_ext1(sc.h_ext1 + 1 - DEC), h_open2(sc.h_open2 + 1 - DEC), h_ext2(sc.h_ext2 + 1 - DEC), v_open1(sc.v_open1),
          v_ext1(sc.v_ext1), v_open2(sc.v_open2), v_ext2(sc.v_ext2), one(sc.one) {}
};

constexpr int kBwdF = 3, kFwdF = 4;

template <int R, int MODE, bool MULTI>
struct Sweep {
    static constexpr bool kIsFwd = MODE == kFwd || MODE == kFwdF;
    static constexpr bool kIsBwd = MODE == kBwd || MODE == kBwdF;
    static constexpr int DEC = MODE == kFwdF ? 0 : MODE == kBwdF ? 2 : 1;
    const int4* prof;
    const uint32_t* twords;
    int t_len, lane;
    bool top, bot;
    const ulonglong2* bnd_in;
    ulonglong2* bnd_out;
    int tag_in, tag_out;
    int* spin;
    int4* bdst;
    int q_len, brow0;
    const int4* bsm;
    int4* bsm_w;
    const int4* bglob_rows;
    const int* bdone;
    int bdone_need, n_right;
    bool late_pending;
    const ulonglong2* tok_in;
    ulonglong2* tok_out;
    int4* out;
    int jnext, m, kcnt, zone_start;
    int r_score, r_end, r_start;
    int rcand, mark_col;
    int k0, min_score;
    int sel_top, sel_n;
    long long sel_sum;
    int H[R], E1[R], E2[R];
    int hup_prev, h_out, f1_out, f2_out;
    int best, bestor, bestst;
    int nz;
    uint32_t twl, w0, w1;
    int wi, wmax, wsh;
    const char* prof_lane;
    int4 bcur;
    ulonglong2 bnxt;
    u64 tokP, tokJ;

    __device__ __forceinline__ uint32_t tword(int i) const { return __ldg(&twords[min(max(i, 0), wmax)]); }

    template <class MS>
    __device__ __forceinline__ void init(const MS& sc) {
#pragma unroll
        for (int r = 0; r < R; ++r) { H[r] = 0; E1[r] = sc.h_open1; E2[r] = sc.h_open2; }
        hup_prev = 0;
        h_out = 0; f1_out = 0; f2_out = 0;
        best = 0; bestor = kIsBwd ? 0 : 0xffff; bestst = 0;
        nz = lane != 0;
        wmax = (t_len + 15) >> 4;
        wi = (-lane) >> 4;
        wsh = 2 * ((-lane) & 15);
        w0 = tword(wi); w1 = tword(wi + 1);
        twl = 0;
        prof_lane = reinterpret_cast<const char*>(prof + lane);
        bcur = make_int4(0, 0, 0, 0); bnxt = make_ulonglong2(0ull, 0ull);
        if (MULTI && top) bnxt = load_bnd(&bnd_in[lane < t_len ? lane : t_len - 1]);
        tokP = 0; tokJ = 0;
    }

    __device__ __forceinline__ void refill() {
        twl = __funnelshift_l(w1, w0, wsh);
        w0 = w1;
        ++wi;
        w1 = tword(wi + 1);
    }

    __device__ __forceinline__ unsigned next_base(unsigned four) {
        unsigned lo, hi;
        asm("{\n\t.reg .u64 p;\n\tmul.wide.u32 p, %2, %3;\n\tmov.b64 {%0, %1}, p;\n\t}" : "=r"(lo), "=r"(hi) : "r"(twl), "r"(four));
        twl = lo;
        return hi;
    }

    __device__ __forceinline__ int best_col() const { return bestst - lane + 1; }

    template <bool JUNC, class MS, class SC>
    __device__ __forceinline__ int cells(const int4* pp, int hd, int mul0, int cm, int& f1, int& f2, const MS& ms,
                                         const SC& sc, int& jhi, int& jlo) {
        constexpr int CH = StripeCfg<R>::CH;
#pragma unroll
        for (int c = 0; c < CH; ++c) {
            const int4 sv = pp[c * 32];
            const int s4[4] = {sv.x, sv.y, sv.z, sv.w};
#pragma unroll
            for (int u = 0; u < 4; ++u) {
                const int r = 4 * c + u;
                if (r < R) {
                    const int hleft = H[r];
                    const int e1pre = E1[r], e2pre = E2[r];
                    int h;
                    cell_w32(hd, r == 0 ? mul0 : ms.one, s4[u], ms, h, E1[r], E2[r], f1, f2);
                    if (JUNC) {
                        const int4 b = bsm[r * 32 + lane];
                        if (MODE == kFwdF) {
                            jhi = __vimax3_s32(jhi, madd(h, ms.one, b.x), madd(e1pre, ms.one, b.y));
                            jhi = max(jhi, madd(e2pre, ms.one, b.z));
                        } else {
                            jcand(h, b.x, sc, jhi, jlo);
                            jcand(e1pre, b.y, sc, jhi, jlo);
                            jcand(e2pre, b.z, sc, jhi, jlo);
                        }
                    }
                    hd = hleft;
                    H[r] = h;
                    if (r & 1) cm = __vimax3_s32(cm, h, H[r - 1]);
                    else if (r == R - 1) cm = max(cm, h);
                }
            }
        }
        return cm;
    }

    __device__ __forceinline__ void select_rung(const int4& rec, int k) {
        if (rec.x >= min_score) {
            if (rec.x > sel_top) { sel_top = rec.x; sel_n = 0; sel_sum = 0; }
            if (rec.x == sel_top && rec.y) { ++sel_n; sel_sum += k; }
        }
    }

    __device__ __forceinline__ void mark_started_in_left() {
#pragma unroll
        for (int r = 0; r < R; ++r) {
            H[r] = __viaddmax_s32(H[r], -1, 0);
            E1[r] -= E1[r] > 0;
            E2[r] -= E2[r] > 0;
        }
        hup_prev = __viaddmax_s32(hup_prev, -1, 0);
    }

    template <bool FAST, bool ZONE, class MS, class SC>
    __device__ __forceinline__ void step(int st, const MS& ms, const SC& sc) {
        constexpr bool zone = !FAST && kIsFwd && ZONE;
        constexpr int CH = StripeCfg<R>::CH;
        int hup = __shfl_up_sync(kFull, h_out, 1);
        int f1 = __shfl_up_sync(kFull, f1_out, 1);
        int f2 = __shfl_up_sync(kFull, f2_out, 1);
        u64 tP = 0, tJ = 0;
        if (zone) {
            if (MODE == kFwdF) {
                tP = (unsigned)__shfl_up_sync(kFull, (int)tokP, 1);
                tJ = (unsigned)__shfl_up_sync(kFull, (int)tokJ, 1);
            } else {
                tP = shfl_up64(tokP); tJ = shfl_up64(tokJ);
            }
        }
        int mul0;
        if (MULTI && top) {
            if ((st & 31) == 0) {
                ulonglong2 raw = bnxt;
                const int cj = st + lane;
                for (int tries = 0; !__all_sync(kFull, bnd_valid(raw, tag_in) || cj >= t_len); ++tries) {
                    if (tries > kSpinLimit) { *spin = 1; break; }
                    if (tries > 3) __nanosleep(32);
                    raw = load_bnd(&bnd_in[cj < t_len ? cj : t_len - 1]);
                }
                bcur = unpack_bnd(raw);
                const int nj = st + 32 + lane;
                bnxt = load_bnd(&bnd_in[nj < t_len ? nj : t_len - 1]);
            }
            const int bh = __shfl_sync(kFull, bcur.x, st & 31);
            const int bf1 = __shfl_sync(kFull, bcur.y, st & 31);
            const int bf2 = __shfl_sync(kFull, bcur.z, st & 31);
            if (lane == 0) { hup = bh; f1 = bf1; f2 = bf2; }
            mul0 = ms.one;
        } else {
            f1 = madd(f1, nz, 0);
            f2 = madd(f2, nz, 0);
            mul0 = nz;
        }
        const unsigned tb = next_base(sc.four);
        const int jj = st - lane;
        if (FAST || (jj >= 0 && jj < t_len)) {
            const int4* pp = reinterpret_cast<const int4*>(prof_lane + tb * (unsigned)(CH * 512));
            const int hd = hup_prev;
            hup_prev = hup;
            const bool last_col = !FAST && kIsBwd && jj == t_len - 1;
            if (kIsBwd && !FAST) {
                if (last_col) {
#pragma unroll
                    for (int r = 0; r < R; ++r) {
                        const int idx0 = q_len - 2 - (brow0 + r);
                        if (idx0 >= 0) {
                            int* d = reinterpret_cast<int*>(&bdst[bvec_pos<R>(idx0)]);
                            d[1] = E1[r] + sc.refund1;
                            d[2] = E2[r] + sc.refund2;
                        }
                    }
                }
            }
            int cm, jhi = kJuncNone, jlo = 0;
            const bool junc = zone && (jj + 1 == jnext);
            const int cm0 = MODE == kFwdF ? best : 0;
            cm = cells<zone>(pp, hd, mul0, cm0, f1, f2, ms, sc, jhi, jlo);
            h_out = H[R - 1]; f1_out = f1; f2_out = f2;
            if (kIsBwd) {
                const int key = madd(cm, ms.one, DEC * st);
                if (key > bestor) { bestor = key; bestst = st; }
                if (last_col) {
#pragma unroll
                    for (int r = 0; r < R; ++r) {
                        const int idx0 = q_len - 2 - (brow0 + r);
                        if (idx0 >= 0) reinterpret_cast<int*>(&bdst[bvec_pos<R>(idx0)])[0] = H[r];
                    }
                }
            } else if (MODE == kFwdF) {
                best = cm;
                if (!FAST && jj == mark_col) mark_started_in_left();
            } else {
                if (cm > bestor) { best = cm; bestor = cm | 0xffff; bestst = st; }
            }
            if (junc) {
                if (MODE == kFwdF) {
                    if (lane == 0) {
                        if (MULTI && top) {
                            ulonglong2 t = load_tok(&tok_in[kcnt]);
                            for (int tries = 0; (int)(t.x >> 32) != tag_in || (int)(t.y >> 32) != tag_in; ++tries) {
                                if (tries > kSpinLimit) { *spin = 1; break; }
                                if (tries > 3) __nanosleep(32);
                                t = load_tok(&tok_in[kcnt]);
                            }
                            tP = (unsigned)t.x; tJ = (unsigned)t.y;
                        } else { tP = 0; tJ = (unsigned)kJuncNone; }
                    }
                    const int myP = max((int)tP, best), myJ = max((int)tJ, jj == mark_col ? jhi - 1 : jhi);
                    tokP = (unsigned)myP; tokJ = (unsigned)myJ;
                    if (lane == 31) {
                        if (MULTI && bot) __stcg(&tok_out[kcnt], make_ulonglong2(tokP | ((u64)(unsigned)tag_out << 32), tokJ | ((u64)(unsigned)tag_out << 32)));
                        else {
                            const int4 rec = finalize_flag_rung(myP, myJ, rcand);
                            out[kcnt] = rec;
                            select_rung(rec, k0 + kcnt);
                        }
                    }
                } else {
                    junction_unbias(jhi, jlo);
                    if (lane == 0) {
                        if (MULTI && top) { __threadfence(); const ulonglong2 t = load_tok(&tok_in[kcnt]); tP = t.x; tJ = t.y; }
                        else { tP = 0; tJ = 0; }
                    }
                    const u64 myP = key_of_best(best, best_col()), myJ = key_of_junction(jhi, jlo);
                    tokP = myP > tP ? myP : tP;
                    tokJ = myJ > tJ ? myJ : tJ;
                    if (lane == 31) {
                        if (MULTI && bot) { __stcg(&tok_out[kcnt], make_ulonglong2(tokP, tokJ)); __threadfence(); }
                        else out[kcnt] = finalize_rung(tokP, tokJ, jj + 1, r_score, r_end, r_start);
                    }
                }
                jnext += m;
                ++kcnt;
            }
            if (MULTI && bot && lane == 31) store_bnd(&bnd_out[jj], h_out, f1_out, f2_out, tag_out);
        }
    }

    __device__ __forceinline__ void late_load() {
        u64 rkey = 0;
        if (bglob_rows) {
            wait_cols(bdone, bdone_need, lane, spin);
            rkey = __ldcg(reinterpret_cast<const u64*>(bdone + 2));
        }
#pragma unroll
        for (int r = 0; r < R; ++r)
            bsm_w[r * 32 + lane] = (bglob_rows && brow0 + r < q_len - 1) ? __ldcg(&bglob_rows[r * 32 + lane])
                                   : (brow0 + r < q_len ? make_int4(0, kPadScore, kPadScore, 0) : make_int4(kPadScore, kPadScore, kPadScore, 0));
        r_score = 0; r_end = 0; r_start = 0; rcand = kJuncNone;
        if (rkey) {
            if (MODE == kFwdF) {
                rcand = (int)(unsigned)rkey - 2 * n_right;
            } else {
                r_score = (int)(rkey >> 32);
                r_end = n_right - (int)((rkey >> 16) & 0xffffu);
                r_start = n_right - (0xffff - (int)(rkey & 0xffffu));
            }
        }
        __syncwarp();
        late_pending = false;
    }

    template <class MS, class SC>
    __device__ __forceinline__ void slow_until(int& st, int end, const MS& ms, const SC& sc) {
        const int pre = kIsFwd ? min(end, zone_start) : end;
#pragma unroll 1
        for (; st < pre; ++st) {
            if ((st & 15) == 0) refill();
            step<false, false>(st, ms, sc);
        }
        if (kIsFwd) {
#pragma unroll 1
            for (; st < end; ++st) {
                if (MULTI && late_pending) late_load();
                if ((st & 15) == 0) refill();
                step<false, true>(st, ms, sc);
            }
        }
    }

    static constexpr int kUnroll = (MULTI && MODE != kExact) ? 1 : 4;
    template <class MS, class SC>
    __device__ __forceinline__ void fast_until(int& st, int end, const MS& ms, const SC& sc) {
        for (; st + 16 <= end; st += 16) {
            refill();
#pragma unroll 1
            for (int b = 0; b < 16; b += kUnroll) {
#pragma unroll
                for (int u = 0; u < kUnroll; ++u) step<true, false>(st + b + u, ms, sc);
            }
        }
    }

    template <class SC>
    __device__ __forceinline__ void run(const SC& sc, int zone_start_) {
        const ModeScore<SC, DEC> ms(sc);
        init(ms);
        zone_start = zone_start_;
        const int nsteps = t_len + 31;
        int fast_end = ((t_len - 1) >> 4) << 4;
        if (kIsFwd) fast_end = min(fast_end, (zone_start >> 4) << 4);
        int st = 0;
        slow_until(st, min(32, nsteps), ms, sc);
        if (MODE == kFwdF && mark_col >= 0) {
            fast_until(st, min(fast_end, (mark_col >> 4) << 4), ms, sc);
            slow_until(st, min(nsteps, ((mark_col + 32 + 15) >> 4) << 4), ms, sc);
        }
        fast_until(st, fast_end, ms, sc);
        slow_until(st, nsteps, ms, sc);
    }

    __device__ __forceinline__ void bwd_best(int& key, int& col) const {
        key = bestor - DEC * (lane - 1);
        col = best_col();
    }
};

__host__ __device__ constexpr bool is_coop_height(int R) { return R == 4 || R == 6 || R == 8 || R == 12 || R == 16; }
__host__ __device__ constexpr int coop_height_at_least(int R) { return R <= 4 ? 4 : R <= 6 ? 6 : R <= 8 ? 8 : R <= 12 ? 12 : 16; }

constexpr int kMinR = 4;
constexpr int kMaxRExact = 16;
constexpr int kMaxRLadder = 12;
constexpr int kMaxRLadderOwn = 16;

__host__ __device__ __forceinline__ void stripe_shape(int q_len, int max_r, int& R, int& n_stripes) {
    if (q_len <= 32 * max_r) {
        n_stripes = 1;
        R = (q_len + 31) / 32;
        if (R < kMinR) R = kMinR;
    } else {
        n_stripes = (q_len + 32 * max_r - 1) / (32 * max_r);
        R = (q_len + 32 * n_stripes - 1) / (32 * n_stripes);
    }
}

struct CoopInfo {
    long long data_off;
    int flag_off;
    int bnd_stride, b_stride, tok_stride;
    int n_stripes;
    int rows;
};
constexpr int kCoopFlagInts(int S) { return 2 * S + 4; }
__device__ __forceinline__ int stripe_tag(int epoch, int s) { return ((epoch & 0x3ff) << 6) | (s & 63); }

struct RestArgs {
    const int32_t* order;
    int n_order;
    int4* scratch;
    const CoopInfo* coop;
    const int32_t* coop_idx;
    int* flags;
    int* spin;
    int epoch;
    int32_t* redo_long;
    int* redo_long_count;
};

template <int R, class SC>
__device__ __noinline__ u64 exact_task(const Task& tk, const uint32_t* __restrict__ pool, const SC& sc, int4* prof, int lane) {
    __syncwarp();
    build_profile<R>(prof, pool + tk.q_word, tk.q_len, lane * R, lane, ModeScore<SC, 1>(sc), false);
    __syncwarp();
    Sweep<R, kExact, false> sw;
    sw.prof = prof; sw.twords = pool + tk.t_word; sw.t_len = tk.t_len; sw.lane = lane;
    sw.top = false; sw.bot = false;
    sw.run(sc, 0);
    return key_of_best(sw.best, sw.best_col());
}

template <int R, class SC>
__device__ __forceinline__ u64 exact_dispatch(int r, const Task& tk, const uint32_t* __restrict__ pool, const SC& sc,
                                              int4* prof, int lane) {
    if (r == R) return exact_task<R>(tk, pool, sc, prof, lane);
    if constexpr (R < kMaxRExact) return exact_dispatch<R + 1>(r, tk, pool, sc, prof, lane);
    return 0ull;
}

template <int R, class SC>
__device__ __noinline__ void exact_stripe(const Task& tk, int tid, int s, const CoopInfo& ci, const RestArgs& ra,
                                             const uint32_t* __restrict__ pool, const SC& sc, int4* prof, int lane, int4* out) {
    const int S = ci.n_stripes;
    const int epoch = ra.epoch;
    int* F = ra.flags + ci.flag_off;
    ulonglong2* bnd_a = reinterpret_cast<ulonglong2*>(ra.scratch + ci.data_off);
    ulonglong2* bnd_b = bnd_a + ci.bnd_stride;
    __syncwarp();
    build_profile<R>(prof, pool + tk.q_word, tk.q_len, s * 32 * R + lane * R, lane, ModeScore<SC, 1>(sc), false);
    __syncwarp();
    Sweep<R, kExact, true> sw;
    sw.prof = prof; sw.twords = pool + tk.t_word; sw.t_len = tk.t_len; sw.lane = lane;
    sw.top = s > 0; sw.bot = s + 1 < S;
    sw.bnd_in = (s & 1) ? bnd_a : bnd_b; sw.bnd_out = (s & 1) ? bnd_b : bnd_a;
    sw.tag_in = stripe_tag(epoch, s - 1); sw.tag_out = stripe_tag(epoch, s); sw.spin = ra.spin;
    sw.run(sc, 0);
    const u64 key = warp_max64(key_of_best(sw.best, sw.best_col()));
    if (lane == 0) {
        u64* K = reinterpret_cast<u64*>(F + 2 * S + 2);
        atomicMax(K, key);
        __threadfence();
        if (atomicAdd(F + 2 * S, 1) == S - 1) {
            __threadfence();
            out[tid] = finalize_rung(atomicMax(K, 0ull), 0ull, 0, 0, 0, 0);
        }
    }
}

template <int R, class SC>
__device__ __forceinline__ void exact_stripe_dispatch(int r, const Task& tk, int tid, int s, const CoopInfo& ci, const RestArgs& ra,
                                                      const uint32_t* __restrict__ pool, const SC& sc, int4* prof,
                                                      int lane, int4* out) {
    if constexpr (is_coop_height(R))
        if (r == R) { exact_stripe<R>(tk, tid, s, ci, ra, pool, sc, prof, lane, out); return; }
    if constexpr (R < kMaxRExact) exact_stripe_dispatch<R + 1>(r, tk, tid, s, ci, ra, pool, sc, prof, lane, out);
}

__host__ __device__ __forceinline__ int coop_rows(int q_len, int n_stripes) {
    const int R = (q_len + 32 * n_stripes - 1) / (32 * n_stripes);
    return R < kMinR ? kMinR : R;
}

constexpr int kWarpsPerBlock = 16;

constexpr int kCodeBits = 7, kCodeFwd = 64;
struct TaskCursor {
    int n_order, lane, warp, wpb;
    int* counter;
    bool first;
    __device__ __forceinline__ TaskCursor(int n_order_, int* counter_)
        : n_order(n_order_), lane(threadIdx.x & 31), warp(threadIdx.x >> 5), wpb(blockDim.x >> 5), counter(counter_), first(true) {}
    __device__ __forceinline__ int next() {
        if (first) {
            first = false;
            const int oi = warp * (int)gridDim.x + (int)blockIdx.x;
            return oi < n_order ? oi : -1;
        }
        int oi = 0;
        if (lane == 0) oi = atomicAdd(counter, 1);
        oi = __shfl_sync(kFull, oi, 0) + wpb * (int)gridDim.x;
        return oi < n_order ? oi : -1;
    }
};


template <class SC>
__device__ __forceinline__ void exact_entry(int e, const Task* __restrict__ tasks, const uint32_t* __restrict__ pool, const SC& sc,
                                            const RestArgs& ra, int4* prof, int lane, int4* out) {
    const int tid = e >> kCodeBits, code = e & ((1 << kCodeBits) - 1);
    const Task tk = tasks[tid];
    if (code == 0) {
        int R, n_stripes;
        stripe_shape(tk.q_len, kMaxRExact, R, n_stripes);
        const u64 key = warp_max64(exact_dispatch<kMinR>(R, tk, pool, sc, prof, lane));
        if (lane == 0) out[tid] = finalize_rung(key, 0ull, 0, 0, 0, 0);
    } else {
        const CoopInfo ci = ra.coop[ra.coop_idx[tid]];
        exact_stripe_dispatch<kMinR>(ci.rows, tk, tid, code - 1, ci, ra, pool, sc, prof, lane, out);
    }
}

template <bool FIXED>
__global__ void __launch_bounds__(32 * kWarpsPerBlock, 1)
exact_kernel(const Task* __restrict__ tasks, RestArgs ra, const uint32_t* __restrict__ pool, ScoreW scw, int* counter,
             int smem_stride, int4* out) {
    extern __shared__ int4 smem[];
    const ScoreView<FIXED> sc(scw);
    const int lane = threadIdx.x & 31;
    const int warp = threadIdx.x >> 5;
    int4* prof = smem + warp * smem_stride;
    TaskCursor cur(ra.n_order, counter);
    for (;;) {
        const int oi = cur.next();
        if (oi < 0) break;
        exact_entry(ra.order[oi], tasks, pool, sc, ra, prof, lane, out);
    }
}

struct LadderCtx {
    const uint32_t* qwords;
    const uint32_t* pool;
    LadderRegion reg;
    int q_len;
};

template <bool FLAG>
__device__ __forceinline__ u64 bwd_key(int key, int col) {
    if (key < 65536) return 0ull;
    if (FLAG) return (u64)(unsigned)key;
    return ((u64)((unsigned)key >> 16) << 32) | ((u64)((unsigned)key & 0xffffu) << 16) | (u64)(0xffffu - (unsigned)col);
}

template <bool FLAG>
__device__ __forceinline__ void r_only(u64 rkey, int n_right, int& r_score, int& r_end, int& r_start, int& rcand) {
    r_score = 0; r_end = 0; r_start = 0; rcand = kJuncNone;
    if (!rkey) return;
    if (FLAG) {
        rcand = (int)(unsigned)rkey - 2 * n_right;
    } else {
        r_score = (int)(rkey >> 32);
        r_end = n_right - (int)((rkey >> 16) & 0xffffu);
        r_start = n_right - (0xffff - (int)(rkey & 0xffffu));
    }
}

__device__ __forceinline__ int4 bvec_default(int idx0, int q_len) {
    return idx0 < q_len ? make_int4(0, kPadScore, kPadScore, 0) : make_int4(kPadScore, kPadScore, kPadScore, 0);
}

template <int R, bool MULTI, bool FLAG, class SW, class SC>
__device__ __forceinline__ void setup_fwd(SW& sw, const LadderTask& tk, const LadderCtx& cx, const SC& sc, int4* prof,
                                          const int4* bsm, int lane, int4* out, int r_score, int r_end, int r_start, int rcand) {
    const int c_first = cx.reg.n_left + cx.reg.m * tk.kmin;
    sw.prof = prof; sw.twords = cx.pool + cx.reg.fwd_word; sw.t_len = cx.reg.n_left + cx.reg.m * tk.kmax; sw.lane = lane;
    sw.bsm = bsm;
    sw.out = out + tk.out_off;
    sw.m = cx.reg.m;
    sw.jnext = c_first > 0 ? c_first : cx.reg.m;
    sw.kcnt = c_first > 0 ? 0 : 1;
    sw.r_score = r_score; sw.r_end = r_end; sw.r_start = r_start;
    sw.rcand = rcand; sw.mark_col = cx.reg.n_left - 1;
    sw.k0 = tk.kmin; sw.min_score = sc.min_score;
    sw.sel_top = 0; sw.sel_n = 0; sw.sel_sum = 0;
    if (FLAG && c_first == 0) {
        const int4 rec = finalize_flag_rung(0, kJuncNone, rcand);
        if (rec.x >= sc.min_score) { sw.sel_top = rec.x; sw.sel_n = rec.y ? 1 : 0; }
    }
}

template <bool FLAG, class SW>
__device__ __forceinline__ void finish_read(const SW& sw, const LadderTask& tk, const LadderCtx& cx, int lane, int4* out, int4* sel,
                                            int r_score, int r_end, int r_start, int rcand) {
    if (FLAG) {
        if (lane == 31) sel[tk.read] = make_int4(sw.sel_top, sw.sel_n, (int)(unsigned)sw.sel_sum, (int)(sw.sel_sum >> 32));
    }
    if (cx.reg.n_left + cx.reg.m * tk.kmin == 0 && lane == 0)
        out[tk.out_off] = FLAG ? finalize_flag_rung(0, kJuncNone, rcand) : finalize_rung(0ull, 0ull, 0, r_score, r_end, r_start);
}

template <int R, bool FLAG, class SC>
__device__ __noinline__ void ladder_task(const LadderTask& tk, const LadderCtx& cx, const SC& sc, int4* prof, int lane,
                                            int4* out, int4* sel) {
    constexpr int BWD = FLAG ? kBwdF : kBwd, FWD = FLAG ? kFwdF : kFwd;
    int4* bsm = prof + StripeCfg<R>::PROF_INT4;
    const int q_len = cx.q_len;
    __syncwarp();
#pragma unroll
    for (int r = 0; r < R; ++r) bsm[r * 32 + lane] = bvec_default(lane * R + r, q_len);
    __syncwarp();
    u64 rkey = 0;
    if (cx.reg.n_right > 0) {
        build_profile<R>(prof, cx.qwords, q_len, lane * R, lane, ModeScore<SC, Sweep<R, BWD, false>::DEC>(sc), true);
        __syncwarp();
        Sweep<R, BWD, false> sw;
        sw.prof = prof; sw.twords = cx.pool + cx.reg.rev_word; sw.t_len = cx.reg.n_right; sw.lane = lane;
        sw.top = false; sw.bot = false;
        sw.bdst = bsm; sw.q_len = q_len; sw.brow0 = lane * R;
        sw.run(sc, 0);
        int key, col;
        sw.bwd_best(key, col);
        rkey = warp_max64(bwd_key<FLAG>(key, col));
    }
    int r_score, r_end, r_start, rcand;
    r_only<FLAG>(rkey, cx.reg.n_right, r_score, r_end, r_start, rcand);
    Sweep<R, FWD, false> sw;
    setup_fwd<R, false, FLAG>(sw, tk, cx, sc, prof, bsm, lane, out, r_score, r_end, r_start, rcand);
    sw.top = false; sw.bot = false;
    if (sw.t_len > 0) {
        __syncwarp();
        build_profile<R>(prof, cx.qwords, q_len, lane * R, lane, ModeScore<SC, Sweep<R, FWD, false>::DEC>(sc), false);
        __syncwarp();
        sw.run(sc, sw.jnext - 1);
    }
    finish_read<FLAG>(sw, tk, cx, lane, out, sel, r_score, r_end, r_start, rcand);
}

template <int R, bool FLAG, class SC>
__device__ __noinline__ void ladder_bwd_stripe(const LadderTask& tk, const LadderCtx& cx, int s, const CoopInfo& ci,
                                                  const RestArgs& ra, const SC& sc, int4* prof, int lane) {
    constexpr int BWD = FLAG ? kBwdF : kBwd;
    const int S = ci.n_stripes;
    const int epoch = ra.epoch;
    int* F = ra.flags + ci.flag_off;
    ulonglong2* bnd_a = reinterpret_cast<ulonglong2*>(ra.scratch + ci.data_off);
    ulonglong2* bnd_b = bnd_a + ci.bnd_stride;
    int4* bglob = ra.scratch + ci.data_off + 4 * ci.bnd_stride;
    __syncwarp();
    build_profile<R>(prof, cx.qwords, cx.q_len, s * 32 * R + lane * R, lane, ModeScore<SC, Sweep<R, BWD, true>::DEC>(sc), true);
    __syncwarp();
    Sweep<R, BWD, true> sw;
    sw.prof = prof; sw.twords = cx.pool + cx.reg.rev_word; sw.t_len = cx.reg.n_right; sw.lane = lane;
    sw.top = s > 0; sw.bot = s + 1 < S;
    sw.bnd_in = (s & 1) ? bnd_a : bnd_b; sw.bnd_out = (s & 1) ? bnd_b : bnd_a;
    sw.tag_in = stripe_tag(epoch, s - 1); sw.tag_out = stripe_tag(epoch, s); sw.spin = ra.spin;
    sw.bdst = bglob; sw.q_len = cx.q_len; sw.brow0 = s * 32 * R + lane * R;
    sw.run(sc, 0);
    int key, col;
    sw.bwd_best(key, col);
    const u64 rkey = warp_max64(bwd_key<FLAG>(key, col));
    __syncwarp();
    if (lane == 0) {
        atomicMax(reinterpret_cast<u64*>(F + 2 * S + 2), rkey);
        __threadfence();
        atomicAdd(F + 2 * S, 1);
    }
}

template <int R, bool FLAG, class SC>
__device__ __noinline__ void ladder_fwd_stripe(const LadderTask& tk, const LadderCtx& cx, int s, const CoopInfo& ci,
                                                  const RestArgs& ra, const SC& sc, int4* prof, int lane, int4* out,
                                                  int4* sel) {
    constexpr int FWD = FLAG ? kFwdF : kFwd;
    const int S = ci.n_stripes;
    const int epoch = ra.epoch;
    int* F = ra.flags + ci.flag_off;
    ulonglong2* bnd_a = reinterpret_cast<ulonglong2*>(ra.scratch + ci.data_off + 2 * ci.bnd_stride);
    ulonglong2* bnd_b = bnd_a + ci.bnd_stride;
    int4* bglob = ra.scratch + ci.data_off + 4 * ci.bnd_stride;
    ulonglong2* tok_a = reinterpret_cast<ulonglong2*>(bglob + ci.b_stride);
    ulonglong2* tok_b = tok_a + ci.tok_stride;
    int4* bsm = prof + StripeCfg<R>::PROF_INT4;
    Sweep<R, FWD, true> sw;
    setup_fwd<R, true, FLAG>(sw, tk, cx, sc, prof, bsm, lane, out, 0, 0, 0, kJuncNone);
    sw.top = s > 0; sw.bot = s + 1 < S;
    sw.bsm_w = bsm;
    sw.bglob_rows = cx.reg.n_right > 0 ? bglob + s * 32 * R : nullptr;
    sw.bdone = F + 2 * S; sw.bdone_need = S; sw.n_right = cx.reg.n_right;
    sw.q_len = cx.q_len; sw.brow0 = s * 32 * R + lane * R;
    sw.late_pending = true;
    sw.spin = ra.spin;
    __syncwarp();
    if (sw.t_len == 0 || cx.reg.n_left + cx.reg.m * tk.kmin == 0) {
        sw.late_load();
        if (FLAG && cx.reg.n_left + cx.reg.m * tk.kmin == 0) {
            const int4 rec = finalize_flag_rung(0, kJuncNone, sw.rcand);
            sw.sel_top = 0; sw.sel_n = 0;
            if (rec.x >= sc.min_score) { sw.sel_top = rec.x; sw.sel_n = rec.y ? 1 : 0; }
        }
    }
    if (sw.t_len > 0) {
        build_profile<R>(prof, cx.qwords, cx.q_len, s * 32 * R + lane * R, lane, ModeScore<SC, Sweep<R, FWD, true>::DEC>(sc), false);
        __syncwarp();
        sw.bnd_in = (s & 1) ? bnd_a : bnd_b; sw.bnd_out = (s & 1) ? bnd_b : bnd_a;
        sw.tok_in = (s & 1) ? tok_a : tok_b; sw.tok_out = (s & 1) ? tok_b : tok_a;
        sw.tag_in = stripe_tag(epoch, s - 1); sw.tag_out = stripe_tag(epoch, s);
        sw.run(sc, sw.jnext - 1);
    }
    if (s == S - 1) finish_read<FLAG>(sw, tk, cx, lane, out, sel, sw.r_score, sw.r_end, sw.r_start, sw.rcand);
}

template <int R, bool FLAG, int MAXR, class SC>
__device__ __forceinline__ void ladder_dispatch(int r, const LadderTask& tk, const LadderCtx& cx, const SC& sc, int4* prof,
                                                int lane, int4* out, int4* sel) {
    if (r == R) { ladder_task<R, FLAG>(tk, cx, sc, prof, lane, out, sel); return; }
    if constexpr (R < MAXR) ladder_dispatch<R + 1, FLAG, MAXR>(r, tk, cx, sc, prof, lane, out, sel);
}

template <int R, bool FLAG, class SC>
__device__ __forceinline__ void ladder_stripe_dispatch(int r, const LadderTask& tk, const LadderCtx& cx, int code, const CoopInfo& ci,
                                                       const RestArgs& ra, const SC& sc, int4* prof, int lane, int4* out,
                                                       int4* sel) {
    if constexpr (is_coop_height(R))
        if (r == R) {
            if (code < kCodeFwd) ladder_bwd_stripe<R, FLAG>(tk, cx, code - 1, ci, ra, sc, prof, lane);
            else ladder_fwd_stripe<R, FLAG>(tk, cx, code - kCodeFwd, ci, ra, sc, prof, lane, out, sel);
            return;
        }
    if constexpr (R < kMaxRLadder) ladder_stripe_dispatch<R + 1, FLAG>(r, tk, cx, code, ci, ra, sc, prof, lane, out, sel);
}

template <bool FLAG, int MAXR, class SC>
__device__ __forceinline__ void ladder_entry(int e, const LadderTask* __restrict__ tasks, const uint32_t* __restrict__ qpool,
                                             const uint32_t* __restrict__ pool, const LadderRegion* __restrict__ regs, const SC& sc,
                                             const RestArgs& ra, int4* prof, int lane, int4* out, int4* sel) {
    const int tid = e >> kCodeBits, code = e & ((1 << kCodeBits) - 1);
    const LadderTask tk = tasks[tid];
    LadderCtx cx;
    cx.qwords = qpool + tk.q_word;
    cx.pool = pool;
    cx.reg = regs[tk.region];
    cx.q_len = tk.q_len;
    if (code == 0) {
        int R, n_stripes;
        stripe_shape(tk.q_len, MAXR, R, n_stripes);
        ladder_dispatch<kMinR, FLAG, MAXR>(R, tk, cx, sc, prof, lane, out, sel);
    } else {
        const CoopInfo ci = ra.coop[tk.pad];
        ladder_stripe_dispatch<kMinR, FLAG>(ci.rows, tk, cx, code, ci, ra, sc, prof, lane, out, sel);
    }
}

template <bool FIXED, bool FLAG>
__global__ void __launch_bounds__(32 * kWarpsPerBlock, 1)
ladder_kernel(const LadderTask* __restrict__ tasks, RestArgs ra, const int* __restrict__ n_order_dev,
              const uint32_t* __restrict__ qpool, const uint32_t* __restrict__ pool, const LadderRegion* __restrict__ regs, ScoreW scw, int* counter,
              int smem_stride, int4* out, int4* sel) {
    extern __shared__ int4 smem[];
    const ScoreView<FIXED> sc(scw);
    const int lane = threadIdx.x & 31;
    const int warp = threadIdx.x >> 5;
    int4* prof = smem + warp * smem_stride;
    TaskCursor cur(n_order_dev ? *n_order_dev : ra.n_order, counter);
    for (;;) {
        const int oi = cur.next();
        if (oi < 0) break;
        ladder_entry<FLAG, kMaxRLadderOwn>(ra.order[oi], tasks, qpool, pool, regs, sc, ra, prof, lane, out, sel);
    }
}

}
```

### nanorepeat_b200/csrc/nr_launch.h

```cpp
#pragma once
#include "nr_kernels.cuh"
#include "nr_pair_kernels.cuh"

namespace nrl {

constexpr size_t kMaxDynShared = (size_t)nr::kWarpsPerBlock * 14 * 1024;

cudaError_t launch_exact(bool fixed, int blocks, int threads, size_t smem, cudaStream_t st, const nr::Task* tasks,
                         const nr::RestArgs& ra, const uint32_t* pool, const nr::ScoreW& k, int* counter, int stride, int4* out);
cudaError_t launch_ladder(bool flag, int blocks, int threads, size_t smem, cudaStream_t st, const nr::LadderTask* tasks,
                          const nr::RestArgs& ra, const int* n_order_dev, const uint32_t* qpool, const uint32_t* pool,
                          const nr::LadderRegion* regs, const nr::ScoreW& k, int* counter, int stride, int4* out, int4* sel);
cudaError_t launch_pair_round2(int blocks, int threads, size_t smem, cudaStream_t st, const nr::pr::Pair2* pairs,
                               const nr::pr::Deal& deal, const nr::Task* tasks, const nr::RestArgs& ra, const uint32_t* pool,
                               const nr::ScoreW& k, int* counter, int stride, int4* out, uint32_t* state,
                               uint32_t* kept);
cudaError_t launch_pair_ladder(int blocks, int threads, size_t smem, cudaStream_t st, const nr::pr::Pair3* pairs,
                               const nr::pr::Deal& deal, const nr::LadderTask* tasks, const nr::RestArgs& ra,
                               const uint32_t* qpool, const uint32_t* pool, const nr::LadderRegion* regs, const nr::ScoreW& k,
                               int* counter, int stride, uint2* prung, int4* out, int4* sel, int* redo_count, int32_t* redo,
                               const uint32_t* qstate);

template <class F>
inline cudaError_t prepare(F fn, bool& done) {
    if (done) return cudaSuccess;
    cudaError_t e = cudaFuncSetAttribute(fn, cudaFuncAttributeMaxDynamicSharedMemorySize, (int)kMaxDynShared);
    if (e == cudaSuccess) e = cudaFuncSetAttribute(fn, cudaFuncAttributePreferredSharedMemoryCarveout, cudaSharedmemCarveoutMaxShared);
    if (e == cudaSuccess) done = true;
    return e;
}

}
```

### nanorepeat_b200/csrc/nr_launch_ladder.cu

```cuda
#include "nr_launch.h"
#include <mutex>
namespace nrl {
cudaError_t launch_ladder(bool flag, int blocks, int threads, size_t smem, cudaStream_t st, const nr::LadderTask* tasks,
                          const nr::RestArgs& ra, const int* n_order_dev, const uint32_t* qpool, const uint32_t* pool,
                          const nr::LadderRegion* regs, const nr::ScoreW& k, int* counter, int stride, int4* out, int4* sel) {
    static std::mutex mu;
    static bool done[2] = {false, false};
    {
        std::lock_guard<std::mutex> lk(mu);
        cudaError_t e = flag ? prepare(nr::ladder_kernel<true, true>, done[1]) : prepare(nr::ladder_kernel<true, false>, done[0]);
        if (e != cudaSuccess) return e;
    }
    if (flag) nr::ladder_kernel<true, true><<<blocks, threads, smem, st>>>(tasks, ra, n_order_dev, qpool, pool, regs, k, counter, stride, out, sel);
    else nr::ladder_kernel<true, false><<<blocks, threads, smem, st>>>(tasks, ra, n_order_dev, qpool, pool, regs, k, counter, stride, out, sel);
    return cudaGetLastError();
}
}
```

### nanorepeat_b200/csrc/nr_launch_pair2.cu

```cuda
#define NR_DEFINE_PAIR_ROUND2_KERNEL
#include "nr_launch.h"
#include <mutex>
namespace nrl {
cudaError_t launch_pair_round2(int blocks, int threads, size_t smem, cudaStream_t st, const nr::pr::Pair2* pairs,
                               const nr::pr::Deal& deal, const nr::Task* tasks, const nr::RestArgs& ra, const uint32_t* pool,
                               const nr::ScoreW& k, int* counter, int stride, int4* out, uint32_t* state,
                               uint32_t* kept) {
    static std::mutex mu;
    static bool done = false;
    {
        std::lock_guard<std::mutex> lk(mu);
        cudaError_t e = prepare(nr::pr::pair_round2_kernel, done);
        if (e != cudaSuccess) return e;
    }
    nr::pr::pair_round2_kernel<<<blocks, threads, smem, st>>>(pairs, deal, tasks, ra, pool, k, counter, stride, out, state, kept);
    return cudaGetLastError();
}
}
```

### nanorepeat_b200/csrc/nr_launch_pair3.cu

```cuda
#define NR_DEFINE_PAIR_LADDER_KERNEL
#include "nr_launch.h"
#include <mutex>
namespace nrl {
cudaError_t launch_pair_ladder(int blocks, int threads, size_t smem, cudaStream_t st, const nr::pr::Pair3* pairs,
                               const nr::pr::Deal& deal, const nr::LadderTask* tasks, const nr::RestArgs& ra,
                               const uint32_t* qpool, const uint32_t* pool, const nr::LadderRegion* regs, const nr::ScoreW& k,
                               int* counter, int stride, uint2* prung, int4* out, int4* sel, int* redo_count, int32_t* redo,
                               const uint32_t* qstate) {
    static std::mutex mu;
    static bool done = false;
    {
        std::lock_guard<std::mutex> lk(mu);
        cudaError_t e = prepare(nr::pr::pair_ladder_kernel, done);
        if (e != cudaSuccess) return e;
    }
    nr::pr::pair_ladder_kernel<<<blocks, threads, smem, st>>>(pairs, deal, tasks, ra, qpool, pool, regs, k, counter, stride, prung,
                                                             out, sel, redo_count, redo, qstate);
    return cudaGetLastError();
}
}
```

### nanorepeat_b200/csrc/nr_pair_kernels.cuh

```cuda
#pragma once
#include "nr_kernels.cuh"

namespace nr {
namespace pr {

typedef unsigned u32;
constexpr int kBias = 64;
__host__ __device__ constexpr u32 pk2(int hi, int lo) { return ((u32)(hi & 0xffff) << 16) | (u32)(lo & 0xffff); }
__host__ __device__ constexpr u32 pk(int v) { return pk2(v, v); }
__host__ __device__ constexpr u32 sub2(int v) { return 0u - (((u32)v << 16) | (u32)v); }

constexpr int kMatch = 4, kMismatch = 8, kAmbiguous = 2, kOpen1 = 12, kExt1 = 4, kOpen2 = 50, kExt2 = 2, kRefund1 = 8, kRefund2 = 48;
constexpr u32 kFloorFwd = pk(kBias + 1);
constexpr u32 kFloorBwd = pk(kBias);
constexpr u32 kOnes = 0x00010001u;

__device__ __forceinline__ u32 pmadd(u32 a, u32 mul, u32 b) {
    u32 d;
    asm("mad.lo.u32 %0, %1, %2, %3;" : "=r"(d) : "r"(a), "r"(mul), "r"(b));
    return d;
}

template <u32 FLOOR>
__device__ __forceinline__ void cell(u32 hd, u32 s, u32 one, u32& h, u32& e1, u32& e2, u32& f1, u32& f2) {
    const u32 d = __viaddmax_u16x2(hd, s, FLOOR);
    const u32 t = __vimax3_u16x2(d, e1, e2);
    h = __vimax3_u16x2(t, f1, f2);
    e1 = __viaddmax_u16x2(h, pk(-kOpen1), pmadd(e1, one, sub2(kExt1)));
    e2 = __viaddmax_u16x2(h, pk(-kOpen2), pmadd(e2, one, sub2(kExt2)));
    f1 = __viaddmax_u16x2(h, pk(-kOpen1), pmadd(f1, one, sub2(kExt1)));
    f2 = __viaddmax_u16x2(h, pk(-kOpen2), pmadd(f2, one, sub2(kExt2)));
}

struct Pair2 {
    int32_t a, b;
    int32_t mark_col;
    int32_t state_off;
    int32_t check_col;
    int32_t period;
    int32_t pad[2];
};

constexpr int kExitSlot = 24;

struct Pair3 {
    int32_t a, b;
    int32_t rung_off;
    int32_t state_off;
    int32_t R;
    int32_t pad[3];
};

__host__ __device__ constexpr int state_words(int R) { return 3 * R + 1; }

template <int R>
__device__ __forceinline__ void build_profile(uint4* prof, const uint32_t* __restrict__ qa, int q_a,
                                              const uint32_t* __restrict__ qb, int q_b, int row0, int lane, bool reverse) {
    constexpr int CH = StripeCfg<R>::CH;
    u32* p = reinterpret_cast<u32*>(prof);
    const uint32_t amb_a = q_a > 0 ? read_ambiguity_plane(qa, q_a) : 0u, amb_b = q_b > 0 ? read_ambiguity_plane(qb, q_b) : 0u;
#pragma unroll
    for (int r = 0; r < 4 * CH; ++r) {
        const int i = row0 + r;
        int ca = 4, cb = 4;
        if (r < R && i < q_a) {
            const int qi = reverse ? q_a - 1 - i : i;
            ca = (qa[qi >> 4] >> (30 - 2 * (qi & 15))) & 3;
            if (amb_a && read_base_ambiguous(qa, amb_a, qi)) ca = 5;
        }
        if (r < R && i < q_b) {
            const int qi = reverse ? q_b - 1 - i : i;
            cb = (qb[qi >> 4] >> (30 - 2 * (qi & 15))) & 3;
            if (amb_b && read_base_ambiguous(qb, amb_b, qi)) cb = 5;
        }
#pragma unroll
        for (int c = 0; c < 4; ++c)
            p[((c * CH + (r >> 2)) * 32 + lane) * 4 + (r & 3)] =
                pk2(ca == 5 ? -kAmbiguous : ca == c ? kMatch : -kMismatch, cb == 5 ? -kAmbiguous : cb == c ? kMatch : -kMismatch);
    }
}

constexpr int kP2 = 0, kPB = 1, kPF = 2;

template <int R, int MODE, bool MULTI = false>
struct Sweep {
    static constexpr u32 FLOOR = MODE == kPB ? kFloorBwd : kFloorFwd;
    static constexpr bool kMarks = MODE != kPB;
    bool top, bot;
    const ulonglong2* bnd_in;
    ulonglong2* bnd_out;
    int tag_in, tag_out;
    int* spin;
    int4 bcur;
    ulonglong2 bnxt;
    const ulonglong2* tok_in;
    ulonglong2* tok_out;
    const u32* bstage;
    int b_stride, brow0;
    const int* bdone;
    int bdone_need;
    bool late_pending;
    u32* bsm_w;
    const uint4* prof;
    const uint32_t* twords;
    int t_len, lane;
    int mark_col;
    int q_a, q_b;
    const u32* bsm;
    uint2* rung_out;
    int jnext, m, kcnt, zone_start;
    int col0;
    const u32* resume;
    u32* save;
    int save_col;
    bool exits;
    int check_col, period;
    int next_check;
    int exit_st;
    u32* kept_io;
    u32 H[R], E1[R], E2[R];
    u32 hup_prev, h_out, f1_out, f2_out;
    u32 best;
    u32 bestc, raw_hi, raw_lo;
    int st_hi, st_lo;
    u32 nz, bz;
    uint32_t twl, w0, w1;
    int wi, wmax, wsh;
    const char* prof_lane;
    u32 tokP, tokJ;

    __device__ __forceinline__ uint32_t tword(int i) const { return __ldg(&twords[min(max(i, 0), wmax)]); }

    __device__ __forceinline__ void init() {
        if (MODE == kPF && resume) {
#pragma unroll
            for (int r = 0; r < R; ++r) {
                H[r] = __ldcg(&resume[r * 32 + lane]);
                E1[r] = __ldcg(&resume[(R + r) * 32 + lane]);
                E2[r] = __ldcg(&resume[(2 * R + r) * 32 + lane]);
            }
            hup_prev = lane ? __ldcg(&resume[(R - 1) * 32 + lane - 1]) : FLOOR;
            best = __ldcg(&resume[3 * R * 32 + lane]);
        } else {
#pragma unroll
            for (int r = 0; r < R; ++r) { H[r] = FLOOR; E1[r] = FLOOR + sub2(kOpen1); E2[r] = FLOOR + sub2(kOpen2); }
            hup_prev = FLOOR;
            best = 0;
        }
        h_out = FLOOR; f1_out = FLOOR; f2_out = FLOOR;
        bestc = FLOOR | kOnes; raw_hi = 0; raw_lo = 0; st_hi = 0; st_lo = 0;
        nz = lane != 0; bz = lane != 0 ? 0u : FLOOR;
        wmax = (t_len + 15) >> 4;
        wi = (col0 - lane) >> 4;
        wsh = 2 * ((col0 - lane) & 15);
        w0 = tword(wi); w1 = tword(wi + 1);
        twl = 0;
        prof_lane = reinterpret_cast<const char*>(prof + lane);
        tokP = 0; tokJ = 0;
        if (MULTI) {
            bcur = make_int4(0, 0, 0, 0); bnxt = make_ulonglong2(0ull, 0ull);
            if (top) bnxt = load_bnd(&bnd_in[lane < t_len ? lane : t_len - 1]);
            late_pending = MODE == kPF;
        }
    }

    __device__ __forceinline__ void refill() {
        twl = __funnelshift_l(w1, w0, wsh);
        w0 = w1;
        ++wi;
        w1 = tword(wi + 1);
    }

    __device__ __forceinline__ unsigned next_base(unsigned four) {
        unsigned lo, hi;
        asm("{\n\t.reg .u64 p;\n\tmul.wide.u32 p, %2, %3;\n\tmov.b64 {%0, %1}, p;\n\t}" : "=r"(lo), "=r"(hi) : "r"(twl), "r"(four));
        twl = lo;
        return hi;
    }

    template <bool JUNC, bool KEEP_E = false>
    __device__ __forceinline__ u32 cells(const uint4* pp, u32 hd, u32 cm, u32& f1, u32& f2, u32 one, u32& jhi, bool keep = false) {
        constexpr int CH = StripeCfg<R>::CH;
        u32 jprev = 0;
#pragma unroll
        for (int c = 0; c < CH; ++c) {
            const uint4 sv = pp[c * 32];
            const u32 s4[4] = {sv.x, sv.y, sv.z, sv.w};
#pragma unroll
            for (int u = 0; u < 4; ++u) {
                const int r = 4 * c + u;
                if (r < R) {
                    const u32 hleft = H[r];
                    const u32 e1pre = E1[r], e2pre = E2[r];
                    u32 h;
                    cell<FLOOR>(hd, s4[u], one, h, E1[r], E2[r], f1, f2);
                    if (KEEP_E) { E1[r] = keep ? e1pre : E1[r]; E2[r] = keep ? e2pre : E2[r]; }
                    if (JUNC) {
                        const u32 bx = bsm[(0 * R + r) * 32 + lane], by = bsm[(1 * R + r) * 32 + lane], bz = bsm[(2 * R + r) * 32 + lane];
                        const u32 t = __vimax3_u16x2(pmadd(h, one, bx), pmadd(e1pre, one, by), pmadd(e2pre, one, bz));
                        if (r & 1) jhi = __vimax3_u16x2(jhi, jprev, t);
                        else if (r == R - 1) jhi = __vmaxu2(jhi, t);
                        jprev = t;
                    }
                    hd = hleft;
                    H[r] = h;
                    if (r & 1) cm = __vimax3_u16x2(cm, h, H[r - 1]);
                    else if (r == R - 1) cm = __vmaxu2(cm, h);
                }
            }
        }
        return cm;
    }

    __device__ __forceinline__ void mark_started_inside() {
#pragma unroll
        for (int r = 0; r < R; ++r) {
            H[r] = __viaddmax_u16x2(H[r], pk(-1), FLOOR);
            E1[r] = __viaddmax_u16x2(E1[r], pk(-1), __vminu2(E1[r], FLOOR));
            E2[r] = __viaddmax_u16x2(E2[r], pk(-1), __vminu2(E2[r], FLOOR));
        }
        hup_prev = __viaddmax_u16x2(hup_prev, pk(-1), FLOOR);
    }

    __device__ __forceinline__ void late_load() {
        wait_cols(bdone, bdone_need, lane, spin);
#pragma unroll
        for (int r = 0; r < R; ++r) {
            const int idx0 = brow0 + lane * R + r;
            const int ia = q_a - 2 - idx0, ib = q_b - 2 - idx0;
#pragma unroll
            for (int c = 0; c < 3; ++c) {
                const u32 da = c == 0 ? (idx0 < q_a ? (u32)kBias : 0u) : 0u, db = c == 0 ? (idx0 < q_b ? (u32)kBias : 0u) : 0u;
                const u32 a = ia >= 0 ? __ldcg(&bstage[c * b_stride + ia]) >> 16 : da;
                const u32 b = ib >= 0 ? __ldcg(&bstage[c * b_stride + ib]) & 0xffffu : db;
                bsm_w[(c * R + r) * 32 + lane] = (a << 16) | b;
            }
        }
        __syncwarp();
        late_pending = false;
    }

    __device__ __forceinline__ void store_stage(u32* stage, int stride, int row0) {
#pragma unroll
        for (int r = 0; r < R; ++r) {
            const int i = row0 + lane * R + r;
            __stcg(&stage[0 * stride + i], H[r]);
            __stcg(&stage[1 * stride + i], E1[r] + pk(kRefund1));
            __stcg(&stage[2 * stride + i], E2[r] + pk(kRefund2));
        }
    }

    __device__ __forceinline__ void store_junction_vectors(u32* stage, u32* bvec_fwd) {
        __syncwarp();
#pragma unroll
        for (int r = 0; r < R; ++r) {
            stage[(0 * R + r) * 32 + lane] = H[r];
            stage[(1 * R + r) * 32 + lane] = E1[r] + pk(kRefund1);
            stage[(2 * R + r) * 32 + lane] = E2[r] + pk(kRefund2);
        }
        __syncwarp();
#pragma unroll
        for (int r = 0; r < R; ++r) {
            const int idx0 = lane * R + r;
            const int ia = q_a - 2 - idx0, ib = q_b - 2 - idx0;
#pragma unroll
            for (int c = 0; c < 3; ++c) {
                const u32 da = c == 0 ? (idx0 < q_a ? (u32)kBias : 0u) : 0u, db = c == 0 ? (idx0 < q_b ? (u32)kBias : 0u) : 0u;
                const u32 a = ia >= 0 ? stage[(c * R + ia % R) * 32 + ia / R] >> 16 : da;
                const u32 b = ib >= 0 ? stage[(c * R + ib % R) * 32 + ib / R] & 0xffffu : db;
                bvec_fwd[(c * R + r) * 32 + lane] = (a << 16) | b;
            }
        }
    }

    template <bool FAST, bool TRACK, bool SPECIAL = false>
    __device__ __forceinline__ void step(int st, u32 one, unsigned four) {
        const bool zone = MODE == kPF && (FAST ? SPECIAL : st >= zone_start);
        constexpr int CH = StripeCfg<R>::CH;
        u32 hup = __shfl_up_sync(kFull, h_out, 1);
        u32 f1 = __shfl_up_sync(kFull, f1_out, 1);
        u32 f2 = __shfl_up_sync(kFull, f2_out, 1);
        u32 tP = 0, tJ = 0;
        if (zone) {
            tP = __shfl_up_sync(kFull, tokP, 1);
            tJ = __shfl_up_sync(kFull, tokJ, 1);
        }
        if (MULTI && top) {
            if ((st & 31) == 0) {
                ulonglong2 raw = bnxt;
                const int cj = st + lane;
                for (int tries = 0; !__all_sync(kFull, bnd_valid(raw, tag_in) || cj >= t_len); ++tries) {
                    if (tries > kSpinLimit) { *spin = 1; break; }
                    if (tries > 3) __nanosleep(32);
                    raw = load_bnd(&bnd_in[cj < t_len ? cj : t_len - 1]);
                }
                bcur = unpack_bnd(raw);
                const int nj = st + 32 + lane;
                bnxt = load_bnd(&bnd_in[nj < t_len ? nj : t_len - 1]);
            }
            const u32 bh = __shfl_sync(kFull, (u32)bcur.x, st & 31);
            const u32 bf1 = __shfl_sync(kFull, (u32)bcur.y, st & 31);
            const u32 bf2 = __shfl_sync(kFull, (u32)bcur.z, st & 31);
            if (lane == 0) { hup = bh; f1 = bf1; f2 = bf2; }
        } else {
            hup = pmadd(hup, nz, bz);
            f1 = pmadd(f1, nz, bz);
            f2 = pmadd(f2, nz, bz);
        }
        const unsigned tb = next_base(four);
        const int rel = st - lane;
        const int jj = rel + col0;
        const bool anyj = zone && __any_sync(kFull, jj + 1 == jnext && jj < t_len);
        if (FAST || (rel >= 0 && jj < t_len)) {
            const uint4* pp = reinterpret_cast<const uint4*>(prof_lane + tb * (unsigned)(CH * 512));
            const u32 hd = hup_prev;
            hup_prev = hup;
            constexpr bool kChecks = !FAST || SPECIAL;
            const bool last_col = !FAST && MODE == kPB && jj == t_len - 1;
            u32 cm, jhi = 0;
            const u32 cm0 = (MODE == kP2 && TRACK) ? 0u : best;
            if (zone && anyj) cm = cells<true>(pp, hd, cm0, f1, f2, one, jhi);
            else if (MODE == kPB && !FAST) cm = cells<false, true>(pp, hd, cm0, f1, f2, one, jhi, last_col);
            else cm = cells<false>(pp, hd, cm0, f1, f2, one, jhi);
            h_out = H[R - 1]; f1_out = f1; f2_out = f2;
            if (MODE == kP2 && TRACK) {
                const u32 nb = __vmaxu2(bestc, cm | kOnes);
                const u32 x = nb ^ bestc;
                bestc = nb;
                if (x > 0xffffu) { st_hi = st; raw_hi = cm; }
                if (x & 0xffffu) { st_lo = st; raw_lo = cm; }
                if (kChecks && save && jj == save_col) {
#pragma unroll
                    for (int r = 0; r < R; ++r) {
                        __stcg(&save[r * 32 + lane], H[r]);
                        __stcg(&save[(R + r) * 32 + lane], E1[r]);
                        __stcg(&save[(2 * R + r) * 32 + lane], E2[r]);
                    }
                    __stcg(&save[3 * R * 32 + lane], bestc);
                }
            } else {
                best = cm;
            }
            if (zone && jj + 1 == jnext) {
                if (lane == 0) {
                    tP = 0; tJ = 0;
                    if (MULTI && top) {
                        ulonglong2 t = load_tok(&tok_in[kcnt]);
                        for (int tries = 0; (int)(t.x >> 32) != tag_in || (int)(t.y >> 32) != tag_in; ++tries) {
                            if (tries > kSpinLimit) { *spin = 1; break; }
                            if (tries > 3) __nanosleep(32);
                            t = load_tok(&tok_in[kcnt]);
                        }
                        tP = (u32)t.x; tJ = (u32)t.y;
                    }
                }
                const u32 jv = jj == mark_col ? jhi - kOnes : jhi;
                tokP = __vmaxu2(tP, best);
                tokJ = __vmaxu2(tJ, jv);
                if (lane == 31) {
                    if (MULTI && bot) __stcg(&tok_out[kcnt], make_ulonglong2(tokP | ((u64)(unsigned)tag_out << 32), tokJ | ((u64)(unsigned)tag_out << 32)));
                    else rung_out[kcnt] = make_uint2(tokP, tokJ);
                }
                jnext += m;
                ++kcnt;
            }
            if (kMarks && kChecks && jj == mark_col) mark_started_inside();
            if (MULTI && bot && lane == 31) store_bnd(&bnd_out[jj], (int)h_out, (int)f1_out, (int)f2_out, tag_out);
        }
    }

    __device__ __forceinline__ void slow_until(int& st, int end, u32 one, unsigned four) {
#pragma unroll 1
        for (; st < end; ++st) {
            if (MULTI && MODE == kPF && late_pending && st >= zone_start) late_load();
            if ((st & 15) == 0) refill();
            step<false, true>(st, one, four);
        }
    }

#ifndef NR_PAIR3_UNROLL
#define NR_PAIR3_UNROLL 2
#endif
#ifndef NR_PAIR2_UNROLL
#define NR_PAIR2_UNROLL 4
#endif
#ifndef NR_PAIR2_MULTI_UNROLL
#define NR_PAIR2_MULTI_UNROLL 4
#endif
    static constexpr int kUnroll = MODE == kP2 ? (MULTI ? NR_PAIR2_MULTI_UNROLL : NR_PAIR2_UNROLL) : (MULTI ? 1 : NR_PAIR3_UNROLL);
    template <bool TRACK, bool SPECIAL = false, bool EXIT = false>
    __device__ __forceinline__ void fast_until(int& st, int end, u32 one, unsigned four) {
        for (; st + 16 <= end; st += 16) {
            if (EXIT && st == next_check) {
                if (dominated_then_keep()) { exit_st = st; return; }
                next_check += (int)__ldcg(kept_io + 96 + lane);
            }
            refill();
#pragma unroll 1
            for (int b = 0; b < 16; b += kUnroll) {
#pragma unroll
                for (int u = 0; u < kUnroll; ++u) step<true, TRACK, SPECIAL>(st + b + u, one, four);
            }
        }
    }

    __device__ __forceinline__ bool dominated_then_keep() {
        u32* g = kept_io + lane;
        const u32 khp = __ldcg(g), kf1 = __ldcg(g + 32), kf2 = __ldcg(g + 64);
        u32 acc = (__vmaxu2(hup_prev, khp) ^ khp) | (__vmaxu2(f1_out, kf1) ^ kf1) | (__vmaxu2(f2_out, kf2) ^ kf2);
        __stcg(g, hup_prev); __stcg(g + 32, f1_out); __stcg(g + 64, f2_out);
        u32* snap = reinterpret_cast<u32*>(const_cast<uint4*>(prof) + StripeCfg<R>::PROF_INT4);
#pragma unroll
        for (int r = 0; r < R; ++r) {
            u32* k = snap + r * 32 + lane;
            const u32 kh = k[0], ke1 = k[R * 32], ke2 = k[2 * R * 32];
            acc |= (__vmaxu2(H[r], kh) ^ kh) | (__vmaxu2(E1[r], ke1) ^ ke1) | (__vmaxu2(E2[r], ke2) ^ ke2);
            k[0] = H[r]; k[R * 32] = E1[r]; k[2 * R * 32] = E2[r];
        }
        return __all_sync(kFull, acc == 0);
    }

    __device__ __forceinline__ void run(u32 one, unsigned four, int zone_start_) {
        init();
        zone_start = zone_start_;
        exit_st = -1;
        const int n = t_len - col0;
        const int nsteps = n + 31;
        const int inside_end = ((n - 1) >> 4) << 4;
        const int mc = mark_col - col0;
        int st = 0;
        slow_until(st, min(32, nsteps), one, four);
        if (MODE == kPB) {
            fast_until<true>(st, inside_end, one, four);
        } else if (MODE == kP2) {
            if (mc >= 0) {
                const int zs = max(mc - 2, 0);
                const int before = st;
                fast_until<false>(st, min(inside_end, (zs >> 4) << 4), one, four);
                if (st != before) {
                    const u32 nb = __vmaxu2(bestc, best | kOnes);
                    const u32 x = nb ^ bestc;
                    bestc = nb;
                    if (x > 0xffffu) { st_hi = lane; raw_hi = 0; }
                    if (x & 0xffffu) { st_lo = lane; raw_lo = 0; }
                }
                slow_until(st, min(nsteps, ((mc + 32 + 15) >> 4) << 4), one, four);
            }
            if (MULTI) {
                fast_until<true>(st, inside_end, one, four);
            } else {
                next_check = -1;
                if (exits && mc >= 0) {
                    const int c0 = max(st, ((check_col - col0 + 32 + 15) >> 4) << 4);
                    if (c0 + period < inside_end) next_check = c0;
                    __stcg(kept_io + lane, 0u); __stcg(kept_io + 32 + lane, 0u); __stcg(kept_io + 64 + lane, 0u);
                    __stcg(kept_io + 96 + lane, (u32)period);
                }
                fast_until<true, false, true>(st, inside_end, one, four);
                if (exit_st >= 0) return;
            }
        } else {
            const int first = min(zone_start, mc >= 0 ? mc : zone_start);
            fast_until<true>(st, min(inside_end, (first >> 4) << 4), one, four);
            if (MULTI && late_pending && st + 16 <= inside_end) late_load();
            fast_until<true, true>(st, inside_end, one, four);
        }
        slow_until(st, nsteps, one, four);
    }
};

constexpr int kMaxRPair3 = 16;
constexpr int kMaxRPair2 = kMaxRPair3;
constexpr int kPairEntry = 1 << 30;

__host__ __device__ __forceinline__ int pair_rows(int q_len) {
    int R = (q_len + 31) / 32;
    return R < kMinR ? kMinR : R;
}

struct Deal {
    int n_rest, n_pairs;
    int static_rest;
    int nb_long;
    int static_pairs;
};
__host__ __device__ inline Deal make_deal(int n_rest, int n_pairs, int wpb, int grid) {
    Deal d;
    d.n_rest = n_rest; d.n_pairs = n_pairs;
    d.static_rest = n_rest < wpb * grid ? n_rest : wpb * grid;
    d.nb_long = (d.static_rest + wpb - 1) / wpb;
    const int room = wpb * (grid - d.nb_long);
    d.static_pairs = n_pairs < room ? n_pairs : room;
    return d;
}
__device__ __forceinline__ int next_item(const Deal& dl, bool& first, int* counter) {
    if (dl.nb_long < 0) {
        const int n = dl.n_rest + dl.n_pairs;
        if (first) {
            first = false;
            const int i = (threadIdx.x >> 5) * (int)gridDim.x + (int)blockIdx.x;
            return i < n ? i : -1;
        }
        int i = 0;
        if ((threadIdx.x & 31) == 0) i = atomicAdd(counter, 1);
        i = __shfl_sync(kFull, i, 0) + (blockDim.x >> 5) * (int)gridDim.x;
        return i < n ? i : -1;
    }
    if (first) {
        first = false;
        const int wpb = blockDim.x >> 5, warp = threadIdx.x >> 5, blk = (int)blockIdx.x;
        if (blk < dl.nb_long) {
            const int e = blk * wpb + warp;
            if (e < dl.static_rest) return e;
        } else {
            const int p = warp * ((int)gridDim.x - dl.nb_long) + (blk - dl.nb_long);
            if (p < dl.static_pairs) return dl.n_rest + p;
        }
    }
    int d = 0;
    if ((threadIdx.x & 31) == 0) d = atomicAdd(counter, 1);
    d = __shfl_sync(kFull, d, 0);
    const int rest_left = dl.n_rest - dl.static_rest;
    if (d < rest_left) return dl.static_rest + d;
    const int p = dl.static_pairs + d - rest_left;
    return p < dl.n_pairs ? dl.n_rest + p : -1;
}

template <int R>
__device__ __forceinline__ void pair2_task(const Pair2& pt, const Task* __restrict__ tasks, const uint32_t* __restrict__ pool,
                                           uint4* prof, int lane, u32 one, unsigned four, int4* out, u32* state,
                                           unsigned long long* skipped, u32* kept) {
    const Task ta = tasks[pt.a];
    Task tb = ta;
    int q_b = 0;
    if (pt.b >= 0) { tb = tasks[pt.b]; q_b = tb.q_len; }
    __syncwarp();
    build_profile<R>(prof, pool + ta.q_word, ta.q_len, pool + tb.q_word, q_b, lane * R, lane, false);
    __syncwarp();
    Sweep<R, kP2> sw;
    sw.prof = prof; sw.twords = pool + ta.t_word; sw.t_len = ta.t_len; sw.lane = lane;
    sw.mark_col = pt.mark_col;
    sw.col0 = 0; sw.resume = nullptr;
    sw.save_col = pt.mark_col - 2;
    sw.save = (state && pt.state_off >= 0 && sw.save_col >= 0) ? state + (size_t)pt.state_off * 32 : nullptr;
    sw.exits = pt.check_col >= 0;
    sw.check_col = pt.check_col; sw.period = pt.period;
    sw.kept_io = kept + (size_t)((blockIdx.x * (blockDim.x >> 5) + (threadIdx.x >> 5)) * 128);
    sw.run(one, four, 0);
    if (sw.exit_st >= 0 && lane == 0) {
        const unsigned long long cols32 = 32ull * (unsigned)ta.t_len - (32ull * (unsigned)sw.exit_st - 496ull);
        atomicAdd(&skipped[0], (unsigned long long)R * cols32);
        atomicAdd(&skipped[1], (unsigned long long)(ta.q_len + q_b) * cols32);
    }
#pragma unroll
    for (int half = 0; half < 2; ++half) {
        const u32 cls = half ? (sw.bestc & 0xffffu) : (sw.bestc >> 16);
        const u32 raw = half ? (sw.raw_lo & 0xffffu) : (sw.raw_hi >> 16);
        const int st = half ? sw.st_lo : sw.st_hi;
        const int score = (int)(cls - (kBias + 1)) >> 1;
        const int col = st - lane;
        unsigned key = 0;
        if (score > 0) key = ((unsigned)score << 17) | ((0xffffu - (unsigned)col) << 1) | (raw & 1u);
        key = __reduce_max_sync(kFull, key);
        const int tid = half ? pt.b : pt.a;
        if (lane == 0 && tid >= 0) {
            int4 rec = make_int4(0, 0, 0, 0);
            if (key) {
                const int c = 0xffff - (int)((key >> 1) & 0xffffu);
                const bool inside = c <= pt.mark_col || !(key & 1u);
                rec = make_int4((int)(key >> 17), inside ? 0 : pt.mark_col + 1, c + 1, 0);
            }
            out[tid] = rec;
        }
    }
}

template <int R>
__device__ __noinline__ void pair2_stripe(const Pair2& pt, int s, const Task* __restrict__ tasks, const uint32_t* __restrict__ pool,
                                          const RestArgs& ra, uint4* prof, int lane, u32 one, unsigned four, int4* out) {
    const CoopInfo ci = ra.coop[pt.state_off];
    const int S = ci.n_stripes;
    int* F = ra.flags + ci.flag_off;
    ulonglong2* bnd_a = reinterpret_cast<ulonglong2*>(ra.scratch + ci.data_off);
    ulonglong2* bnd_b = bnd_a + ci.bnd_stride;
    const Task ta = tasks[pt.a];
    Task tb = ta;
    int q_b = 0;
    if (pt.b >= 0) { tb = tasks[pt.b]; q_b = tb.q_len; }
    __syncwarp();
    build_profile<R>(prof, pool + ta.q_word, ta.q_len, pool + tb.q_word, q_b, s * 32 * R + lane * R, lane, false);
    __syncwarp();
    Sweep<R, kP2, true> sw;
    sw.prof = prof; sw.twords = pool + ta.t_word; sw.t_len = ta.t_len; sw.lane = lane;
    sw.mark_col = pt.mark_col;
    sw.col0 = 0; sw.resume = nullptr; sw.save = nullptr; sw.save_col = -1;
    sw.top = s > 0; sw.bot = s + 1 < S;
    sw.bnd_in = (s & 1) ? bnd_a : bnd_b; sw.bnd_out = (s & 1) ? bnd_b : bnd_a;
    sw.tag_in = stripe_tag(ra.epoch, s - 1); sw.tag_out = stripe_tag(ra.epoch, s); sw.spin = ra.spin;
    sw.run(one, four, 0);
    unsigned keys[2];
#pragma unroll
    for (int half = 0; half < 2; ++half) {
        const u32 cls = half ? (sw.bestc & 0xffffu) : (sw.bestc >> 16);
        const u32 raw = half ? (sw.raw_lo & 0xffffu) : (sw.raw_hi >> 16);
        const int st = half ? sw.st_lo : sw.st_hi;
        const int score = (int)(cls - (kBias + 1)) >> 1;
        unsigned key = 0;
        if (score > 0) key = ((unsigned)score << 17) | ((0xffffu - (unsigned)(st - lane)) << 1) | (raw & 1u);
        keys[half] = __reduce_max_sync(kFull, key);
    }
    if (lane == 0) {
        unsigned* K = reinterpret_cast<unsigned*>(F + 2 * S + 2);
        atomicMax(&K[0], keys[0]);
        atomicMax(&K[1], keys[1]);
        __threadfence();
        if (atomicAdd(F + 2 * S, 1) == S - 1) {
            __threadfence();
#pragma unroll
            for (int half = 0; half < 2; ++half) {
                const int tid = half ? pt.b : pt.a;
                if (tid < 0) continue;
                const unsigned key = atomicMax(&K[half], 0u);
                int4 rec = make_int4(0, 0, 0, 0);
                if (key) {
                    const int c = 0xffff - (int)((key >> 1) & 0xffffu);
                    const bool inside = c <= pt.mark_col || !(key & 1u);
                    rec = make_int4((int)(key >> 17), inside ? 0 : pt.mark_col + 1, c + 1, 0);
                }
                out[tid] = rec;
            }
        }
    }
}

template <int R>
__device__ __forceinline__ void pair2_stripe_dispatch(int r, const Pair2& pt, int s, const Task* __restrict__ tasks,
                                                      const uint32_t* __restrict__ pool, const RestArgs& ra, uint4* prof, int lane,
                                                      u32 one, unsigned four, int4* out) {
    if constexpr (is_coop_height(R))
        if (r == R) { pair2_stripe<R>(pt, s, tasks, pool, ra, prof, lane, one, four, out); return; }
    if constexpr (R < kMaxRLadder) pair2_stripe_dispatch<R + 1>(r, pt, s, tasks, pool, ra, prof, lane, one, four, out);
}

template <int R>
__device__ __forceinline__ void pair2_dispatch(int r, const Pair2& pt, const Task* __restrict__ tasks,
                                               const uint32_t* __restrict__ pool, uint4* prof, int lane, u32 one,
                                               unsigned four, int4* out, u32* state, unsigned long long* skipped, u32* kept) {
    if (r == R) { pair2_task<R>(pt, tasks, pool, prof, lane, one, four, out, state, skipped, kept); return; }
    if constexpr (R < kMaxRPair2) pair2_dispatch<R + 1>(r, pt, tasks, pool, prof, lane, one, four, out, state, skipped, kept);
}

#ifdef NR_DEFINE_PAIR_ROUND2_KERNEL
__global__ void __launch_bounds__(32 * kWarpsPerBlock, 1)
pair_round2_kernel(const Pair2* __restrict__ pairs, Deal dl, const Task* __restrict__ tasks, RestArgs ra,
                   const uint32_t* __restrict__ pool, ScoreW scw, int* counter, int smem_stride, int4* out, u32* state,
                   u32* kept) {
    extern __shared__ uint4 psmem[];
    const ScoreView<true> sc(scw);
    const int lane = threadIdx.x & 31, warp = threadIdx.x >> 5;
    uint4* prof = psmem + warp * smem_stride;
    bool first = true;
    for (;;) {
        const int i = next_item(dl, first, counter);
        if (i < 0) break;
        if (i < ra.n_order) {
            const int e = ra.order[i];
            if (e & kPairEntry) {
                const Pair2 mp = pairs[(e & ~kPairEntry) >> kCodeBits];
                pair2_stripe_dispatch<kMinR>(ra.coop[mp.state_off].rows, mp, (e & ((1 << kCodeBits) - 1)) - 1, tasks, pool, ra, prof, lane,
                                             (u32)sc.one, sc.four, out);
            } else {
                exact_entry(e, tasks, pool, sc, ra, reinterpret_cast<int4*>(prof), lane, out);
            }
            continue;
        }
        const Pair2 pt = pairs[i - ra.n_order];
        int q = tasks[pt.a].q_len;
        if (pt.b >= 0) q = max(q, tasks[pt.b].q_len);
        pair2_dispatch<kMinR>(pair_rows(q), pt, tasks, pool, prof, lane, (u32)sc.one, sc.four, out, state,
                              reinterpret_cast<unsigned long long*>(counter + kExitSlot), kept);
    }
}
#endif

__device__ __forceinline__ void rung_of(u32 P, u32 J, u32 rc, int& score, bool& in_right, bool& unmarked) {
    const u32 np = max(J, rc);
    const int s_p = (int)(P - kBias) >> 1;
    const int s_np = (int)(np - 2 * kBias) >> 1;
    in_right = s_np > s_p;
    score = max(s_p, s_np);
    unmarked = np & 1u;
}

__device__ __forceinline__ void pair3_select(const Pair3& pt, const LadderTask& ta, const LadderTask& tb, int kmin, u32 rcand,
                                             const uint2* rungs, int lane, int min_score, int4* sel, int* redo_count, int32_t* redo,
                                             int redo_shift) {
#pragma unroll
    for (int half = 0; half < 2; ++half) {
        const int tid = half ? pt.b : pt.a;
        if (tid < 0) continue;
        const LadderTask& tk = half ? tb : ta;
        const u32 rc = half ? (rcand & 0xffffu) : (rcand >> 16);
        int top = 0;
        for (int k = tk.kmin + lane; k <= tk.kmax; k += 32) {
            const uint2 t = rungs[k - kmin];
            int s; bool ir, um;
            rung_of(half ? (t.x & 0xffffu) : (t.x >> 16), half ? (t.y & 0xffffu) : (t.y >> 16), rc, s, ir, um);
            if (s >= min_score) top = max(top, s);
        }
        top = __reduce_max_sync(kFull, top);
        int n = 0, sum = 0, unsure = 0;
        if (top > 0) {
            for (int k = tk.kmin + lane; k <= tk.kmax; k += 32) {
                const uint2 t = rungs[k - kmin];
                int s; bool ir, um;
                rung_of(half ? (t.x & 0xffffu) : (t.x >> 16), half ? (t.y & 0xffffu) : (t.y >> 16), rc, s, ir, um);
                if (s == top && ir) {
                    if (um) unsure = 1;
                    else { ++n; sum += k; }
                }
            }
        }
        n = __reduce_add_sync(kFull, n);
        sum = __reduce_add_sync(kFull, sum);
        unsure = __any_sync(kFull, unsure);
        if (lane == 0) {
            sel[tk.read] = make_int4(top, n, sum, 0);
            if (unsure) redo[atomicAdd(redo_count, 1)] = tid << redo_shift;
        }
    }
}

template <int R>
__device__ __forceinline__ void pair3_task(const Pair3& pt, const LadderTask* __restrict__ tasks,
                                           const uint32_t* __restrict__ qpool, const uint32_t* __restrict__ pool,
                                           const LadderRegion* __restrict__ regs, uint4* prof, int lane, u32 one,
                                           unsigned four, int min_score, uint2* prung, int4* sel, int* redo_count,
                                           int32_t* redo, const u32* __restrict__ qstate) {
    const bool ha = pt.a >= 0, hb = pt.b >= 0;
    const LadderTask tv = tasks[ha ? pt.a : pt.b];
    LadderTask ta = tv, tb = tv;
    int q_a = 0, q_b = 0;
    if (ha) { ta = tasks[pt.a]; q_a = ta.q_len; }
    if (hb) { tb = tasks[pt.b]; q_b = tb.q_len; }
    const LadderRegion reg = regs[tv.region];
    const int kmin = (ha && hb) ? min(ta.kmin, tb.kmin) : tv.kmin;
    const int kmax = (ha && hb) ? max(ta.kmax, tb.kmax) : tv.kmax;
    u32* bsm = reinterpret_cast<u32*>(prof + StripeCfg<R>::PROF_INT4);
    uint2* rungs = prung + pt.rung_off;
    __syncwarp();
    build_profile<R>(prof, qpool + ta.q_word, q_a, qpool + tb.q_word, q_b, lane * R, lane, true);
    __syncwarp();
    u32 rcand;
    {
        Sweep<R, kPB> sw;
        sw.prof = prof; sw.twords = pool + reg.rev_word; sw.t_len = reg.n_right; sw.lane = lane;
        sw.mark_col = -1; sw.q_a = q_a; sw.q_b = q_b;
        sw.col0 = 0; sw.resume = nullptr; sw.save = nullptr; sw.save_col = -1;
        sw.run(one, four, 0);
        const u32 ra = __reduce_max_sync(kFull, sw.best >> 16), rb = __reduce_max_sync(kFull, sw.best & 0xffffu);
        rcand = pk2((int)ra + kBias + 1, (int)rb + kBias + 1);
        sw.store_junction_vectors(reinterpret_cast<u32*>(prof), bsm);
    }
    __syncwarp();
    build_profile<R>(prof, qpool + ta.q_word, q_a, qpool + tb.q_word, q_b, lane * R, lane, false);
    __syncwarp();
    {
        Sweep<R, kPF> sw;
        sw.prof = prof; sw.twords = pool + reg.fwd_word; sw.t_len = reg.n_left + reg.m * kmax; sw.lane = lane;
        sw.mark_col = reg.n_left - 1; sw.bsm = bsm; sw.rung_out = rungs;
        sw.m = reg.m; sw.jnext = reg.n_left + reg.m * kmin; sw.kcnt = 0;
        sw.save = nullptr; sw.save_col = -1;
        const bool resumes = qstate && pt.state_off >= 0;
        sw.col0 = resumes ? reg.n_left - 1 : 0;
        sw.resume = resumes ? qstate + (size_t)pt.state_off * 32 : nullptr;
        sw.run(one, four, sw.jnext - 1 - sw.col0);
    }
    __syncwarp();
    pair3_select(pt, ta, tb, kmin, rcand, rungs, lane, min_score, sel, redo_count, redo, kCodeBits);
}

template <int R>
__device__ __noinline__ void pair3_bwd_stripe(const Pair3& pt, int s, const LadderTask* __restrict__ tasks,
                                              const uint32_t* __restrict__ qpool, const uint32_t* __restrict__ pool,
                                              const LadderRegion* __restrict__ regs, const RestArgs& ra, uint4* prof, int lane,
                                              u32 one, unsigned four) {
    const CoopInfo ci = ra.coop[pt.pad[0]];
    const int S = ci.n_stripes;
    int* F = ra.flags + ci.flag_off;
    ulonglong2* bnd_a = reinterpret_cast<ulonglong2*>(ra.scratch + ci.data_off);
    ulonglong2* bnd_b = bnd_a + ci.bnd_stride;
    u32* stage = reinterpret_cast<u32*>(ra.scratch + ci.data_off + 4 * ci.bnd_stride);
    const LadderTask ta = tasks[pt.a], tb = tasks[pt.b];
    const LadderRegion reg = regs[ta.region];
    __syncwarp();
    build_profile<R>(prof, qpool + ta.q_word, ta.q_len, qpool + tb.q_word, tb.q_len, s * 32 * R + lane * R, lane, true);
    __syncwarp();
    Sweep<R, kPB, true> sw;
    sw.prof = prof; sw.twords = pool + reg.rev_word; sw.t_len = reg.n_right; sw.lane = lane;
    sw.mark_col = -1; sw.q_a = ta.q_len; sw.q_b = tb.q_len;
    sw.col0 = 0; sw.resume = nullptr; sw.save = nullptr; sw.save_col = -1;
    sw.top = s > 0; sw.bot = s + 1 < S;
    sw.bnd_in = (s & 1) ? bnd_a : bnd_b; sw.bnd_out = (s & 1) ? bnd_b : bnd_a;
    sw.tag_in = stripe_tag(ra.epoch, s - 1); sw.tag_out = stripe_tag(ra.epoch, s); sw.spin = ra.spin;
    sw.run(one, four, 0);
    sw.store_stage(stage, ci.b_stride, s * 32 * R);
    const u32 ba = __reduce_max_sync(kFull, sw.best >> 16), bb = __reduce_max_sync(kFull, sw.best & 0xffffu);
    __syncwarp();
    if (lane == 0) {
        unsigned* K = reinterpret_cast<unsigned*>(F + 2 * S + 2);
        atomicMax(&K[0], ba);
        atomicMax(&K[1], bb);
        __threadfence();
        atomicAdd(F + 2 * S, 1);
    }
}

template <int R>
__device__ __noinline__ void pair3_fwd_stripe(const Pair3& pt, int s, const LadderTask* __restrict__ tasks,
                                              const uint32_t* __restrict__ qpool, const uint32_t* __restrict__ pool,
                                              const LadderRegion* __restrict__ regs, const RestArgs& ra, uint4* prof, int lane,
                                              u32 one, unsigned four, int min_score, uint2* prung, int4* sel, int* redo_count,
                                              int32_t* redo) {
    const CoopInfo ci = ra.coop[pt.pad[0]];
    const int S = ci.n_stripes;
    int* F = ra.flags + ci.flag_off;
    ulonglong2* bnd_a = reinterpret_cast<ulonglong2*>(ra.scratch + ci.data_off + 2 * ci.bnd_stride);
    ulonglong2* bnd_b = bnd_a + ci.bnd_stride;
    const u32* stage = reinterpret_cast<const u32*>(ra.scratch + ci.data_off + 4 * ci.bnd_stride);
    ulonglong2* tok_a = reinterpret_cast<ulonglong2*>(ra.scratch + ci.data_off + 4 * ci.bnd_stride + (3 * ci.b_stride + 3) / 4);
    ulonglong2* tok_b = tok_a + ci.tok_stride;
    const LadderTask ta = tasks[pt.a], tb = tasks[pt.b];
    const LadderRegion reg = regs[ta.region];
    const int kmin = min(ta.kmin, tb.kmin), kmax = max(ta.kmax, tb.kmax);
    u32* bsm = reinterpret_cast<u32*>(prof + StripeCfg<R>::PROF_INT4);
    uint2* rungs = prung + pt.rung_off;
    __syncwarp();
    build_profile<R>(prof, qpool + ta.q_word, ta.q_len, qpool + tb.q_word, tb.q_len, s * 32 * R + lane * R, lane, false);
    __syncwarp();
    Sweep<R, kPF, true> sw;
    sw.prof = prof; sw.twords = pool + reg.fwd_word; sw.t_len = reg.n_left + reg.m * kmax; sw.lane = lane;
    sw.mark_col = reg.n_left - 1; sw.bsm = bsm; sw.bsm_w = bsm; sw.rung_out = rungs;
    sw.m = reg.m; sw.jnext = reg.n_left + reg.m * kmin; sw.kcnt = 0;
    sw.q_a = ta.q_len; sw.q_b = tb.q_len;
    sw.save = nullptr; sw.save_col = -1; sw.col0 = 0; sw.resume = nullptr;
    sw.top = s > 0; sw.bot = s + 1 < S;
    sw.bnd_in = (s & 1) ? bnd_a : bnd_b; sw.bnd_out = (s & 1) ? bnd_b : bnd_a;
    sw.tok_in = (s & 1) ? tok_a : tok_b; sw.tok_out = (s & 1) ? tok_b : tok_a;
    sw.tag_in = stripe_tag(ra.epoch, s - 1); sw.tag_out = stripe_tag(ra.epoch, s); sw.spin = ra.spin;
    sw.bstage = stage; sw.b_stride = ci.b_stride; sw.brow0 = s * 32 * R;
    sw.bdone = F + 2 * S; sw.bdone_need = S;
    sw.run(one, four, sw.jnext - 1);
    if (s == S - 1) {
        __syncwarp();
        if (sw.late_pending) wait_cols(sw.bdone, sw.bdone_need, lane, ra.spin);
        const unsigned* K = reinterpret_cast<const unsigned*>(F + 2 * S + 2);
        const u32 rcand = pk2((int)__ldcg(&K[0]) + kBias + 1, (int)__ldcg(&K[1]) + kBias + 1);
        pair3_select(pt, ta, tb, kmin, rcand, rungs, lane, min_score, sel, ra.redo_long_count, ra.redo_long, 0);
    }
}

template <int R>
__device__ __forceinline__ void pair3_stripe_dispatch(int r, const Pair3& pt, int code, const LadderTask* __restrict__ tasks,
                                                      const uint32_t* __restrict__ qpool, const uint32_t* __restrict__ pool,
                                                      const LadderRegion* __restrict__ regs, const RestArgs& ra, uint4* prof,
                                                      int lane, u32 one, unsigned four, int min_score, uint2* prung, int4* sel,
                                                      int* redo_count, int32_t* redo) {
    if constexpr (is_coop_height(R))
        if (r == R) {
            if (code < kCodeFwd) pair3_bwd_stripe<R>(pt, code - 1, tasks, qpool, pool, regs, ra, prof, lane, one, four);
            else pair3_fwd_stripe<R>(pt, code - kCodeFwd, tasks, qpool, pool, regs, ra, prof, lane, one, four, min_score, prung, sel,
                                     redo_count, redo);
            return;
        }
    if constexpr (R < kMaxRLadder)
        pair3_stripe_dispatch<R + 1>(r, pt, code, tasks, qpool, pool, regs, ra, prof, lane, one, four, min_score, prung, sel, redo_count, redo);
}

template <int R>
__device__ __forceinline__ void pair3_dispatch(int r, const Pair3& pt, const LadderTask* __restrict__ tasks,
                                               const uint32_t* __restrict__ qpool, const uint32_t* __restrict__ pool,
                                               const LadderRegion* __restrict__ regs, uint4* prof, int lane, u32 one,
                                               unsigned four, int min_score, uint2* prung, int4* sel, int* redo_count,
                                               int32_t* redo, const u32* __restrict__ qstate) {
    if (r == R) { pair3_task<R>(pt, tasks, qpool, pool, regs, prof, lane, one, four, min_score, prung, sel, redo_count, redo, qstate); return; }
    if constexpr (R < kMaxRPair3)
        pair3_dispatch<R + 1>(r, pt, tasks, qpool, pool, regs, prof, lane, one, four, min_score, prung, sel, redo_count, redo, qstate);
}

#ifdef NR_DEFINE_PAIR_LADDER_KERNEL
__global__ void __launch_bounds__(32 * kWarpsPerBlock, 1)
pair_ladder_kernel(const Pair3* __restrict__ pairs, Deal dl, const LadderTask* __restrict__ tasks, RestArgs ra,
                   const uint32_t* __restrict__ qpool, const uint32_t* __restrict__ pool,
                   const LadderRegion* __restrict__ regs, ScoreW scw, int* counter,
                   int smem_stride, uint2* prung, int4* out, int4* sel, int* redo_count, int32_t* redo,
                   const u32* __restrict__ qstate) {
    extern __shared__ uint4 psmem[];
    const ScoreView<true> sc(scw);
    const int lane = threadIdx.x & 31, warp = threadIdx.x >> 5;
    uint4* prof = psmem + warp * smem_stride;
    bool first = true;
    for (;;) {
        const int i = next_item(dl, first, counter);
        if (i < 0) break;
        if (i < ra.n_order) {
            const int e = ra.order[i];
            if (e & kPairEntry) {
                const Pair3 mp = pairs[(e & ~kPairEntry) >> kCodeBits];
                pair3_stripe_dispatch<kMinR>(mp.R, mp, e & ((1 << kCodeBits) - 1), tasks, qpool, pool, regs, ra, prof, lane, (u32)sc.one,
                                             sc.four, sc.min_score, prung, sel, redo_count, redo);
            } else {
                ladder_entry<true, kMaxRLadder>(e, tasks, qpool, pool, regs, sc, ra, reinterpret_cast<int4*>(prof), lane, out, sel);
            }
            continue;
        }
        const Pair3 pt = pairs[i - ra.n_order];
        int rows = pt.R;
        if (rows <= 0) {
            int q = pt.a >= 0 ? tasks[pt.a].q_len : 0;
            if (pt.b >= 0) q = max(q, tasks[pt.b].q_len);
            rows = pair_rows(q);
        }
        pair3_dispatch<kMinR>(rows, pt, tasks, qpool, pool, regs, prof, lane, (u32)sc.one, sc.four, sc.min_score, prung, sel, redo_count, redo, qstate);
    }
}
#endif

}
}
```

Baseline: 71040.

## Chain paired batch runs with programmatic dependent launch and double-banked counters

Enables programmatic dependent launch for the paired round-2/round-3 and redo kernels so the next kernel's prologue (profile build, static items) overlaps the previous kernel's tail, with grid_dep_wait placed before dependent reads and writes. Counters and flags are double-banked and each kernel zeros the next bank at its end, replacing the per-run memsets. Device-to-host result copies are deferred to fetch time when chaining, and the redo launch is capped at a few blocks. This adds complexity around ordering correctness and moves the copies into synchronous calls at fetch.

Result: faster. 76640 (median of 6 runs) (+7.9%).

```diff
diff --git a/nanorepeat_b200/csrc/nr_api.cu b/nanorepeat_b200/csrc/nr_api.cu
--- a/nanorepeat_b200/csrc/nr_api.cu
+++ b/nanorepeat_b200/csrc/nr_api.cu
@@ -269,7 +269,7 @@
     if ((rc = cached_alloc((void**)&b->d_out, b->out_bytes, BUF_DEV))) return rc;
     if ((rc = cached_alloc((void**)&b->h_out, b->out_bytes, BUF_PIN))) return rc;
     if (b->scratch_bytes && (rc = cached_alloc((void**)&b->d_scratch, b->scratch_bytes, BUF_SCRATCH))) return rc;
-    if (b->flags_bytes && (rc = cached_alloc((void**)&b->d_flags, b->flags_bytes, BUF_DEV))) return rc;
+    if (b->flags_bytes && (rc = cached_alloc((void**)&b->d_flags, 2 * b->flags_bytes, BUF_DEV))) return rc;
     if (b->state_bytes && (rc = cached_alloc((void**)&b->d_state, b->state_bytes, BUF_DEV))) return rc;
     if (b->round2_exit &&
         (rc = cached_alloc((void**)&b->d_kept, sizeof(uint32_t) * 128 * kWarpsPerBlock * (size_t)g_ctx.sm_count, BUF_DEV))) return rc;
@@ -305,6 +305,7 @@
     CUDA_TRY(cudaMemcpyAsync(d, h, b->blob_bytes, cudaMemcpyHostToDevice, st));
     CUDA_TRY(cudaMemsetAsync(b->d_out, 0, b->out_bytes, st));
     if (b->d_sel) CUDA_TRY(cudaMemsetAsync(b->d_sel, 0, b->sel_bytes, st));
+    if (b->d_flags) CUDA_TRY(cudaMemsetAsync(b->d_flags, 0, 2 * b->flags_bytes, st));
     CUDA_TRY(cudaEventRecord(b->ev_uploaded, st));
     trace.mark("upload + memsets (async)");
     b->committed = true;
@@ -316,15 +317,24 @@
     return rc ? rc : upload_batch(b);
 }
 
+constexpr int kRedoBlocks = 8;
 constexpr int kSpinSlot = 16;
+
+int* counters(const nr_batch* b) { return b->d_counters + 32 * b->bank; }
+int* flags(const nr_batch* b) { return b->d_flags ? b->d_flags + (size_t)b->bank * (b->flags_bytes / sizeof(int)) : nullptr; }
+
+bool pdl_enabled() {
+    const char* e = getenv("NR_PDL");
+    return !(e && atoi(e) == 0);
+}
 
 int rest_args(nr_batch* b, const int32_t* order, int count, cudaStream_t st, nr::RestArgs* out) {
     nr::RestArgs ra;
     ra.order = order; ra.n_order = count;
-    ra.scratch = b->d_scratch; ra.coop = b->d_coop; ra.coop_idx = b->d_coop_idx; ra.flags = b->d_flags;
-    ra.spin = b->d_counters + kSpinSlot;
+    ra.scratch = b->d_scratch; ra.coop = b->d_coop; ra.coop_idx = b->d_coop_idx; ra.flags = flags(b);
+    ra.spin = counters(b) + kSpinSlot;
     ra.redo_long = b->d_redo ? b->d_redo + b->ltasks.size() : nullptr;
-    ra.redo_long_count = b->d_counters + 4;
+    ra.redo_long_count = counters(b) + 4;
     const long long no = g_launch_no.fetch_add(1);
     ra.epoch = (int)(no % kEpochs) + 1;
     if (b->d_scratch) {
@@ -342,7 +352,7 @@
 }
 
 int launch_rest(nr_batch* b, cudaStream_t st, const nr::ScoreW& k, const int32_t* order, int count, int blocks,
-                int R, const int* count_dev, int* counter) {
+                int R, const int* count_dev, int* counter, bool pdl) {
     const Launch& L = b->launch;
     nr::RestArgs ra;
     int rc;
@@ -355,7 +365,7 @@
         const size_t smem = (size_t)wpb * stride * sizeof(int4);
         if (smem > nrl::kMaxDynShared) return fail(NR_ERR_ARG, "launch needs %zu bytes of shared memory", smem);
         CUDA_TRY(nrl::launch_ladder(b->flag, blocks, wpb * 32, smem, st, b->d_ltasks, ra, count_dev,
-                                    b->qsrc ? b->qsrc->d_pool : b->d_pool, b->d_pool, b->d_lregs, k, counter, stride, b->d_out, b->d_sel));
+                                    b->qsrc ? b->qsrc->d_pool : b->d_pool, b->d_pool, b->d_lregs, k, counter, stride, b->d_out, b->d_sel, pdl));
     } else {
         const int stride = exact_smem_int4(R);
         const size_t smem = (size_t)kWarpsPerBlock * stride * sizeof(int4);
@@ -376,14 +386,15 @@
     return t_aux_stream;
 }
 
-int run_batch(nr_batch* b, cudaStream_t st) {
+int run_batch(nr_batch* b, cudaStream_t st, bool chain) {
     if (!b->committed) return fail(NR_ERR_ARG, "batch was not committed");
     b->run_stream = st;
     const Launch& L = b->launch;
     const nr::ScoreW k = score_words(b->sc);
-    if (st != g_ctx.stream) {
+    if (st != g_ctx.stream && st != b->upload_ordered) {
         CUDA_TRY(cudaStreamWaitEvent(st, b->ev_uploaded, 0));
         if (b->qsrc) CUDA_TRY(cudaStreamWaitEvent(st, b->qsrc->ev_uploaded, 0));
+        b->upload_ordered = st;
     }
     bool resumes = false;
     for (const nr::pr::Pair3& p : b->pairs3) resumes = resumes || p.state_off >= 0;
@@ -391,20 +402,29 @@
         if (!b->qsrc->ran) return fail(NR_ERR_ARG, "nr_batch_run: the round-2 batch this round-3 batch resumes from has not been run");
         if (b->qsrc->run_stream != st) CUDA_TRY(cudaStreamWaitEvent(st, b->qsrc->ev_done, 0));
     }
-    CUDA_TRY(cudaMemsetAsync(b->d_counters, 0, 32 * sizeof(int), st));
-    if (b->flags_bytes) CUDA_TRY(cudaMemsetAsync(b->d_flags, 0, b->flags_bytes, st));
+    const bool paired = L.n_pairs || b->n_long_pairs;
+    b->bank = paired ? (int)(b->n_runs & 1) : 0;
+    ++b->n_runs;
+    if (!paired) {
+        CUDA_TRY(cudaMemsetAsync(counters(b), 0, 32 * sizeof(int), st));
+        if (b->flags_bytes) CUDA_TRY(cudaMemsetAsync(flags(b), 0, b->flags_bytes, st));
+    }
     int launches = 0;
     int rc;
     const bool timing = g_timing.load() != 0;
+    const bool pdl = chain && paired && !timing && pdl_enabled();
     if (timing)
         for (cudaEvent_t& e : b->ev_t)
             if (!e) CUDA_TRY(cudaEventCreate(&e));
     b->timed[0] = b->timed[1] = b->timed[2] = false;
     auto mark = [&](int i, cudaStream_t s) { return timing ? cudaEventRecord(b->ev_t[i], s) : cudaSuccess; };
-    if (L.n_pairs || b->n_long_pairs) {
+    if (paired) {
         const bool ladder_batch = L.ladder;
         nr::RestArgs ra;
         if ((rc = rest_args(b, b->d_order, L.count, st, &ra))) return rc;
+        const size_t n_flag_words = b->flags_bytes / sizeof(int);
+        const nr::pr::NextBank nb = {b->d_counters + 32 * (b->bank ^ 1), b->d_flags ? b->d_flags + (b->bank ^ 1) * n_flag_words : nullptr,
+                                     (int)n_flag_words};
         int wpb = kWarpsPerBlock;
         if (const char* e = getenv("NR_WPB")) wpb = std::max(4, std::min(kWarpsPerBlock, atoi(e)));
         const int blocks = std::max(1, std::min(g_ctx.sm_count, L.count + L.n_pairs));
@@ -417,15 +437,15 @@
             const size_t smem = (size_t)wpb * stride * sizeof(int4);
             if (smem > nrl::kMaxDynShared) return fail(NR_ERR_ARG, "launch needs %zu bytes of shared memory", smem);
             CUDA_TRY(nrl::launch_pair_round2(blocks, wpb * 32, smem, st, static_cast<const nr::pr::Pair2*>(b->d_pairs), deal, b->d_tasks,
-                                             ra, b->d_pool, k, b->d_counters, stride, b->d_out, b->d_state, b->d_kept));
+                                             ra, b->d_pool, k, counters(b), stride, b->d_out, b->d_state, b->d_kept, nb, pdl));
         } else {
             const int stride = pair_ladder_smem_int4(L.pair_R, L.R);
             const size_t smem = (size_t)wpb * stride * sizeof(int4);
             if (smem > nrl::kMaxDynShared) return fail(NR_ERR_ARG, "launch needs %zu bytes of shared memory", smem);
             CUDA_TRY(nrl::launch_pair_ladder(blocks, wpb * 32, smem, st, static_cast<const nr::pr::Pair3*>(b->d_pairs), deal, b->d_ltasks,
-                                             ra, b->qsrc ? b->qsrc->d_pool : b->d_pool, b->d_pool, b->d_lregs, k, b->d_counters, stride,
-                                             b->d_prung, b->d_out, b->d_sel, b->d_counters + 2, b->d_redo,
-                                             b->qsrc ? b->qsrc->d_state : nullptr));
+                                             ra, b->qsrc ? b->qsrc->d_pool : b->d_pool, b->d_pool, b->d_lregs, k, counters(b), stride,
+                                             b->d_prung, b->d_out, b->d_sel, counters(b) + 2, b->d_redo,
+                                             b->qsrc ? b->qsrc->d_state : nullptr, nb, pdl));
         }
         CUDA_TRY(cudaGetLastError());
         CUDA_TRY(mark(3, st));
@@ -433,29 +453,32 @@
         ++launches;
         if (!b->pairs3.empty()) {
             CUDA_TRY(mark(4, st));
-            if ((rc = launch_rest(b, st, k, b->d_redo, 0, std::max(1, std::min(g_ctx.sm_count, 2 * L.n_pairs)), L.redo_R,
-                                  b->d_counters + 2, b->d_counters + 3))) return rc;
+            if ((rc = launch_rest(b, st, k, b->d_redo, 0, std::max(1, std::min(kRedoBlocks, 2 * L.n_pairs)), L.redo_R,
+                                  counters(b) + 2, counters(b) + 3, pdl))) return rc;
             CUDA_TRY(mark(5, st));
             b->timed[2] = timing;
-            CUDA_TRY(cudaMemcpyAsync(b->h_redo_count, b->d_counters + 2, sizeof(int), cudaMemcpyDeviceToHost, st));
-            CUDA_TRY(cudaMemcpyAsync(b->h_redo_count + 1, b->d_counters + 4, sizeof(int), cudaMemcpyDeviceToHost, st));
+            if (!pdl) {
+                CUDA_TRY(cudaMemcpyAsync(b->h_redo_count, counters(b) + 2, sizeof(int), cudaMemcpyDeviceToHost, st));
+                CUDA_TRY(cudaMemcpyAsync(b->h_redo_count + 1, counters(b) + 4, sizeof(int), cudaMemcpyDeviceToHost, st));
+            }
             ++launches;
         }
     } else if (L.count) {
         CUDA_TRY(mark(0, st));
-        if ((rc = launch_rest(b, st, k, b->d_order, L.count, L.blocks, L.R, nullptr, b->d_counters))) return rc;
+        if ((rc = launch_rest(b, st, k, b->d_order, L.count, L.blocks, L.R, nullptr, counters(b), false))) return rc;
         CUDA_TRY(mark(1, st));
         b->timed[0] = timing;
         ++launches;
     }
-    if (b->flag) {
-        if (b->n_reads) CUDA_TRY(cudaMemcpyAsync(b->h_sel, b->d_sel, sizeof(int4) * b->n_reads, cudaMemcpyDeviceToHost, st));
-    } else if (b->n_out) {
-        CUDA_TRY(cudaMemcpyAsync(b->h_out, b->d_out, sizeof(int4) * b->n_out, cudaMemcpyDeviceToHost, st));
-    }
-    if (b->flags_bytes) {
-        if (!b->h_spin) { int rc2 = cached_alloc((void**)&b->h_spin, 64, BUF_PIN); if (rc2) return rc2; }
-        CUDA_TRY(cudaMemcpyAsync(b->h_spin, b->d_counters + kSpinSlot, sizeof(int), cudaMemcpyDeviceToHost, st));
+    if (b->flags_bytes && !b->h_spin) { int rc2 = cached_alloc((void**)&b->h_spin, 64, BUF_PIN); if (rc2) return rc2; }
+    b->copies_pending = pdl;
+    if (!pdl) {
+        if (b->flag) {
+            if (b->n_reads) CUDA_TRY(cudaMemcpyAsync(b->h_sel, b->d_sel, sizeof(int4) * b->n_reads, cudaMemcpyDeviceToHost, st));
+        } else if (b->n_out) {
+            CUDA_TRY(cudaMemcpyAsync(b->h_out, b->d_out, sizeof(int4) * b->n_out, cudaMemcpyDeviceToHost, st));
+        }
+        if (b->flags_bytes) CUDA_TRY(cudaMemcpyAsync(b->h_spin, counters(b) + kSpinSlot, sizeof(int), cudaMemcpyDeviceToHost, st));
     }
     CUDA_TRY(cudaEventRecord(b->ev_done, st));
     b->stats.kernel_launches = launches;
@@ -466,9 +489,28 @@
 
 int redo_long_reads(nr_batch* b);
 
+int run_fetched_soon(nr_batch* b, cudaStream_t st) { return run_batch(b, st ? st : g_ctx.stream, false); }
+
+int settle_copies(nr_batch* b) {
+    if (!b->copies_pending) return NR_OK;
+    if (b->flag) {
+        if (b->n_reads) CUDA_TRY(cudaMemcpy(b->h_sel, b->d_sel, sizeof(int4) * b->n_reads, cudaMemcpyDeviceToHost));
+    } else if (b->n_out) {
+        CUDA_TRY(cudaMemcpy(b->h_out, b->d_out, sizeof(int4) * b->n_out, cudaMemcpyDeviceToHost));
+    }
+    int c[32];
+    CUDA_TRY(cudaMemcpy(c, counters(b), sizeof(c), cudaMemcpyDeviceToHost));
+    if (b->h_redo_count) { b->h_redo_count[0] = c[2]; b->h_redo_count[1] = c[4]; }
+    if (b->h_spin) *b->h_spin = c[kSpinSlot];
+    b->copies_pending = false;
+    return NR_OK;
+}
+
 int fetch_raw(nr_batch* b) {
     if (!b->ran) return fail(NR_ERR_ARG, "batch was not run");
     CUDA_TRY(cudaEventSynchronize(b->ev_done));
+    int rc = settle_copies(b);
+    if (rc) return rc;
     if (b->h_spin && *b->h_spin)
         return fail(NR_ERR_CUDA, "a stripe of a long read gave up waiting for the stripe above it; the results of this batch are not valid");
     if (b->n_long_pairs && b->h_redo_count && b->h_redo_count[1] > 0 && !b->long_redone) return redo_long_reads(b);
@@ -746,7 +788,7 @@
     t->n_reads = cnt;
     t->n_out = (size_t)t->rung_off.back();
     int rc = commit_batch(t);
-    if (!rc) rc = run_batch(t, st);
+    if (!rc) rc = run_batch(t, st, false);
     if (!rc) rc = fetch_raw(t);
     if (!rc)
         for (int j = 0; j < cnt; ++j) b->h_sel[b->ltasks[tids[j]].read] = t->h_sel[j];
@@ -818,7 +860,7 @@
     cached_free(b->d_out, b->out_bytes, BUF_DEV);
     cached_free(b->h_out, b->out_bytes, BUF_PIN);
     cached_free(b->d_scratch, b->scratch_bytes, BUF_SCRATCH);
-    cached_free(b->d_flags, b->flags_bytes, BUF_DEV);
+    cached_free(b->d_flags, 2 * b->flags_bytes, BUF_DEV);
     cached_free(b->d_state, b->state_bytes, BUF_DEV);
     if (b->d_kept) cached_free(b->d_kept, sizeof(uint32_t) * 128 * kWarpsPerBlock * (size_t)g_ctx.sm_count, BUF_DEV);
     cached_free(b->d_sel, b->sel_bytes, BUF_DEV);
@@ -976,7 +1018,7 @@
 
 int nr_batch_run(nr_batch_t* b, void* stream) {
     if (!b) return fail(NR_ERR_ARG, "nr_batch_run: NULL batch");
-    return run_batch(b, stream ? (cudaStream_t)stream : g_ctx.stream);
+    return run_batch(b, stream ? (cudaStream_t)stream : g_ctx.stream, true);
 }
 
 int nr_batch_fetch_alns(nr_batch_t* b, nr_aln_t* out) {
@@ -1098,9 +1140,11 @@
     out->n_rest = b->launch.count;
     if (b->ran) {
         CUDA_TRY(cudaEventSynchronize(b->ev_done));
+        int rc = settle_copies(b);
+        if (rc) return rc;
         if (b->round2_exit) {
             unsigned long long skipped[2];
-            CUDA_TRY(cudaMemcpy(skipped, b->d_counters + nr::pr::kExitSlot, sizeof(skipped), cudaMemcpyDeviceToHost));
+            CUDA_TRY(cudaMemcpy(skipped, counters(b) + nr::pr::kExitSlot, sizeof(skipped), cudaMemcpyDeviceToHost));
             out->paired_cells -= 2 * (int64_t)skipped[0];
             out->paired_useful_cells -= (int64_t)(skipped[1] / 32);
         }
@@ -1129,7 +1173,7 @@
     if (n_tasks > 0 && !out) return fail(NR_ERR_ARG, "nr_score_tasks: out is NULL");
     nr_batch_t* b = nr_batch_create_tasks(sc, n_tasks, queries, qlen, targets, tlen);
     if (!b) return g_code;
-    int rc = nr_batch_run(b, nullptr);
+    int rc = run_batch(b, g_ctx.stream, false);
     if (!rc) rc = nr_batch_fetch_alns(b, out);
     g_last_stats = b->stats;
     nr_batch_destroy(b);
@@ -1142,7 +1186,7 @@
     if (n_reads > 0 && !out) return fail(NR_ERR_ARG, "nr_round2_region: out is NULL");
     nr_batch_t* b = nr_batch_create_round2(sc, left, n_left, motif, motif_len, T, n_reads, cores, core_len);
     if (!b) return g_code;
-    int rc = nr_batch_run(b, nullptr);
+    int rc = run_batch(b, g_ctx.stream, false);
     if (!rc) rc = nr_batch_fetch_alns(b, out);
     g_last_stats = b->stats;
     nr_batch_destroy(b);
@@ -1157,7 +1201,7 @@
     nr_batch_t* b = nr_batch_create_round3(sc, left, n_left, right, n_right, motif, motif_len, n_reads, cores,
                                            core_len, kmin, kmax);
     if (!b) return g_code;
-    int rc = nr_batch_run(b, nullptr);
+    int rc = run_batch(b, g_ctx.stream, false);
     if (!rc) rc = nr_batch_fetch_round3(b, rung_offset, rungs, sum_k, n_k, top_score);
     g_last_stats = b->stats;
     nr_batch_destroy(b);
@@ -1328,7 +1372,7 @@
     trace.mark("estimate: round-2 add (pack, threads)");
     for (Group& G : groups) {
         if (G.rc) { const int rc1 = G.rc; const std::string msg = G.err; cleanup(); return fail(rc1, "%s", msg.c_str()); }
-        if (G.b2 && ((rc = nr_batch_commit(G.b2)) || (rc = nr_batch_run(G.b2, aux_stream_for(G.b2))))) { cleanup(); return rc; }
+        if (G.b2 && ((rc = nr_batch_commit(G.b2)) || (rc = run_fetched_soon(G.b2, aux_stream_for(G.b2))))) { cleanup(); return rc; }
         trace.mark("estimate: round-2 commit + run");
     }
     std::vector<int32_t> kmin, kmax;
@@ -1359,7 +1403,7 @@
             if ((rc = nr_batch_add_round3_reuse(G.b3, (int)i, R.right, R.n_right, kmin.data(), kmax.data()))) { cleanup(); return rc; }
         }
         trace.mark("estimate: select 2 + round-3 add");
-        if ((rc = nr_batch_commit(G.b3)) || (rc = nr_batch_run(G.b3, aux_stream_for(G.b3)))) { cleanup(); return rc; }
+        if ((rc = nr_batch_commit(G.b3)) || (rc = run_fetched_soon(G.b3, aux_stream_for(G.b3)))) { cleanup(); return rc; }
         trace.mark("estimate: round-3 commit + run");
     }
     for (Group& G : groups) {
diff --git a/nanorepeat_b200/csrc/nr_batch.h b/nanorepeat_b200/csrc/nr_batch.h
--- a/nanorepeat_b200/csrc/nr_batch.h
+++ b/nanorepeat_b200/csrc/nr_batch.h
@@ -127,6 +127,9 @@
     size_t state_bytes = 0;
     int* d_flags = nullptr;
     size_t flags_bytes = 0;
+    int bank = 0;
+    long long n_runs = 0;
+    bool copies_pending = false;
     nrh::Launch launch = {};
     nrh::Pool pool;
     std::vector<nrh::RegionInfo> regions;
@@ -157,6 +160,7 @@
     nr_stats_t stats = {};
     bool ran = false;
     cudaStream_t run_stream = nullptr;
+    cudaStream_t upload_ordered = nullptr;
     cudaEvent_t ev_uploaded = nullptr;
     cudaEvent_t ev_done = nullptr;
     int refs = 1;
diff --git a/nanorepeat_b200/csrc/nr_kernels.cuh b/nanorepeat_b200/csrc/nr_kernels.cuh
--- a/nanorepeat_b200/csrc/nr_kernels.cuh
+++ b/nanorepeat_b200/csrc/nr_kernels.cuh
@@ -140,6 +140,9 @@
         }
     __syncwarp();
 }
+
+__device__ __forceinline__ void grid_dep_trigger() { asm volatile("griddepcontrol.launch_dependents;" ::: "memory"); }
+__device__ __forceinline__ void grid_dep_wait() { asm volatile("griddepcontrol.wait;" ::: "memory"); }
 
 __device__ __forceinline__ u64 shfl_up64(u64 v) {
     unsigned lo = __shfl_up_sync(kFull, (unsigned)v, 1);
@@ -956,6 +959,8 @@
     const int lane = threadIdx.x & 31;
     const int warp = threadIdx.x >> 5;
     int4* prof = smem + warp * smem_stride;
+    grid_dep_trigger();
+    grid_dep_wait();
     TaskCursor cur(n_order_dev ? *n_order_dev : ra.n_order, counter);
     for (;;) {
         const int oi = cur.next();
diff --git a/nanorepeat_b200/csrc/nr_launch.h b/nanorepeat_b200/csrc/nr_launch.h
--- a/nanorepeat_b200/csrc/nr_launch.h
+++ b/nanorepeat_b200/csrc/nr_launch.h
@@ -10,16 +10,17 @@
                          const nr::RestArgs& ra, const uint32_t* pool, const nr::ScoreW& k, int* counter, int stride, int4* out);
 cudaError_t launch_ladder(bool flag, int blocks, int threads, size_t smem, cudaStream_t st, const nr::LadderTask* tasks,
                           const nr::RestArgs& ra, const int* n_order_dev, const uint32_t* qpool, const uint32_t* pool,
-                          const nr::LadderRegion* regs, const nr::ScoreW& k, int* counter, int stride, int4* out, int4* sel);
+                          const nr::LadderRegion* regs, const nr::ScoreW& k, int* counter, int stride, int4* out, int4* sel,
+                          bool pdl);
 cudaError_t launch_pair_round2(int blocks, int threads, size_t smem, cudaStream_t st, const nr::pr::Pair2* pairs,
                                const nr::pr::Deal& deal, const nr::Task* tasks, const nr::RestArgs& ra, const uint32_t* pool,
                                const nr::ScoreW& k, int* counter, int stride, int4* out, uint32_t* state,
-                               uint32_t* kept);
+                               uint32_t* kept, const nr::pr::NextBank& nb, bool pdl);
 cudaError_t launch_pair_ladder(int blocks, int threads, size_t smem, cudaStream_t st, const nr::pr::Pair3* pairs,
                                const nr::pr::Deal& deal, const nr::LadderTask* tasks, const nr::RestArgs& ra,
                                const uint32_t* qpool, const uint32_t* pool, const nr::LadderRegion* regs, const nr::ScoreW& k,
                                int* counter, int stride, uint2* prung, int4* out, int4* sel, int* redo_count, int32_t* redo,
-                               const uint32_t* qstate);
+                               const uint32_t* qstate, const nr::pr::NextBank& nb, bool pdl);
 
 template <class F>
 inline cudaError_t prepare(F fn, bool& done) {
@@ -30,4 +31,25 @@
     return e;
 }
 
+template <class... P, class... A>
+inline cudaError_t launch_kernel(bool pdl, void (*fn)(P...), int blocks, int threads, size_t smem, cudaStream_t st, A... args) {
+    cudaLaunchConfig_t cfg = {};
+    cfg.gridDim = dim3(blocks);
+    cfg.blockDim = dim3(threads);
+    cfg.dynamicSmemBytes = smem;
+    cfg.stream = st;
+    cudaLaunchAttribute at[1];
+    at[0].id = cudaLaunchAttributeProgrammaticStreamSerialization;
+    at[0].val.programmaticStreamSerializationAllowed = 1;
+    cfg.attrs = at;
+    cfg.numAttrs = pdl ? 1 : 0;
+    cudaError_t e = cudaLaunchKernelEx(&cfg, fn, args...);
+    if (e != cudaSuccess && pdl) {
+        cudaGetLastError();
+        cfg.numAttrs = 0;
+        e = cudaLaunchKernelEx(&cfg, fn, args...);
+    }
+    return e;
 }
+
+}
diff --git a/nanorepeat_b200/csrc/nr_launch_ladder.cu b/nanorepeat_b200/csrc/nr_launch_ladder.cu
--- a/nanorepeat_b200/csrc/nr_launch_ladder.cu
+++ b/nanorepeat_b200/csrc/nr_launch_ladder.cu
@@ -3,7 +3,8 @@
 namespace nrl {
 cudaError_t launch_ladder(bool flag, int blocks, int threads, size_t smem, cudaStream_t st, const nr::LadderTask* tasks,
                           const nr::RestArgs& ra, const int* n_order_dev, const uint32_t* qpool, const uint32_t* pool,
-                          const nr::LadderRegion* regs, const nr::ScoreW& k, int* counter, int stride, int4* out, int4* sel) {
+                          const nr::LadderRegion* regs, const nr::ScoreW& k, int* counter, int stride, int4* out, int4* sel,
+                          bool pdl) {
     static std::mutex mu;
     static bool done[2] = {false, false};
     {
@@ -11,8 +12,7 @@
         cudaError_t e = flag ? prepare(nr::ladder_kernel<true, true>, done[1]) : prepare(nr::ladder_kernel<true, false>, done[0]);
         if (e != cudaSuccess) return e;
     }
-    if (flag) nr::ladder_kernel<true, true><<<blocks, threads, smem, st>>>(tasks, ra, n_order_dev, qpool, pool, regs, k, counter, stride, out, sel);
-    else nr::ladder_kernel<true, false><<<blocks, threads, smem, st>>>(tasks, ra, n_order_dev, qpool, pool, regs, k, counter, stride, out, sel);
-    return cudaGetLastError();
+    return launch_kernel(pdl, flag ? nr::ladder_kernel<true, true> : nr::ladder_kernel<true, false>, blocks, threads, smem, st, tasks, ra,
+                         n_order_dev, qpool, pool, regs, k, counter, stride, out, sel);
 }
 }
diff --git a/nanorepeat_b200/csrc/nr_launch_pair2.cu b/nanorepeat_b200/csrc/nr_launch_pair2.cu
--- a/nanorepeat_b200/csrc/nr_launch_pair2.cu
+++ b/nanorepeat_b200/csrc/nr_launch_pair2.cu
@@ -5,7 +5,7 @@
 cudaError_t launch_pair_round2(int blocks, int threads, size_t smem, cudaStream_t st, const nr::pr::Pair2* pairs,
                                const nr::pr::Deal& deal, const nr::Task* tasks, const nr::RestArgs& ra, const uint32_t* pool,
                                const nr::ScoreW& k, int* counter, int stride, int4* out, uint32_t* state,
-                               uint32_t* kept) {
+                               uint32_t* kept, const nr::pr::NextBank& nb, bool pdl) {
     static std::mutex mu;
     static bool done = false;
     {
@@ -13,7 +13,7 @@
         cudaError_t e = prepare(nr::pr::pair_round2_kernel, done);
         if (e != cudaSuccess) return e;
     }
-    nr::pr::pair_round2_kernel<<<blocks, threads, smem, st>>>(pairs, deal, tasks, ra, pool, k, counter, stride, out, state, kept);
-    return cudaGetLastError();
+    return launch_kernel(pdl, nr::pr::pair_round2_kernel, blocks, threads, smem, st, pairs, deal, tasks, ra, pool, k, counter, stride,
+                         out, state, kept, nb);
 }
 }
diff --git a/nanorepeat_b200/csrc/nr_launch_pair3.cu b/nanorepeat_b200/csrc/nr_launch_pair3.cu
--- a/nanorepeat_b200/csrc/nr_launch_pair3.cu
+++ b/nanorepeat_b200/csrc/nr_launch_pair3.cu
@@ -6,7 +6,7 @@
                                const nr::pr::Deal& deal, const nr::LadderTask* tasks, const nr::RestArgs& ra,
                                const uint32_t* qpool, const uint32_t* pool, const nr::LadderRegion* regs, const nr::ScoreW& k,
                                int* counter, int stride, uint2* prung, int4* out, int4* sel, int* redo_count, int32_t* redo,
-                               const uint32_t* qstate) {
+                               const uint32_t* qstate, const nr::pr::NextBank& nb, bool pdl) {
     static std::mutex mu;
     static bool done = false;
     {
@@ -14,8 +14,7 @@
         cudaError_t e = prepare(nr::pr::pair_ladder_kernel, done);
         if (e != cudaSuccess) return e;
     }
-    nr::pr::pair_ladder_kernel<<<blocks, threads, smem, st>>>(pairs, deal, tasks, ra, qpool, pool, regs, k, counter, stride, prung,
-                                                             out, sel, redo_count, redo, qstate);
-    return cudaGetLastError();
+    return launch_kernel(pdl, nr::pr::pair_ladder_kernel, blocks, threads, smem, st, pairs, deal, tasks, ra, qpool, pool, regs, k,
+                         counter, stride, prung, out, sel, redo_count, redo, qstate, nb);
 }
 }
diff --git a/nanorepeat_b200/csrc/nr_pair_kernels.cuh b/nanorepeat_b200/csrc/nr_pair_kernels.cuh
--- a/nanorepeat_b200/csrc/nr_pair_kernels.cuh
+++ b/nanorepeat_b200/csrc/nr_pair_kernels.cuh
@@ -444,6 +444,7 @@
                     if (x > 0xffffu) { st_hi = lane; raw_hi = 0; }
                     if (x & 0xffffu) { st_lo = lane; raw_lo = 0; }
                 }
+                grid_dep_wait();
                 slow_until(st, min(nsteps, ((mc + 32 + 15) >> 4) << 4), one, four);
             }
             if (MULTI) {
@@ -493,6 +494,17 @@
     d.static_pairs = n_pairs < room ? n_pairs : room;
     return d;
 }
+struct NextBank {
+    int* counters;
+    int* flags;
+    int n_flags;
+};
+__device__ __forceinline__ void zero_next_bank(const NextBank& nb) {
+    grid_dep_wait();
+    if (blockIdx.x == 0 && threadIdx.x < 32) nb.counters[threadIdx.x] = 0;
+    for (int i = (int)(blockIdx.x * blockDim.x + threadIdx.x); i < nb.n_flags; i += (int)(gridDim.x * blockDim.x)) nb.flags[i] = 0;
+}
+
 __device__ __forceinline__ int next_item(const Deal& dl, bool& first, int* counter) {
     if (dl.nb_long < 0) {
         const int n = dl.n_rest + dl.n_pairs;
@@ -502,6 +514,7 @@
             return i < n ? i : -1;
         }
         int i = 0;
+        grid_dep_wait();
         if ((threadIdx.x & 31) == 0) i = atomicAdd(counter, 1);
         i = __shfl_sync(kFull, i, 0) + (blockDim.x >> 5) * (int)gridDim.x;
         return i < n ? i : -1;
@@ -518,6 +531,7 @@
         }
     }
     int d = 0;
+    grid_dep_wait();
     if ((threadIdx.x & 31) == 0) d = atomicAdd(counter, 1);
     d = __shfl_sync(kFull, d, 0);
     const int rest_left = dl.n_rest - dl.static_rest;
@@ -547,6 +561,7 @@
     sw.check_col = pt.check_col; sw.period = pt.period;
     sw.kept_io = kept + (size_t)((blockIdx.x * (blockDim.x >> 5) + (threadIdx.x >> 5)) * 128);
     sw.run(one, four, 0);
+    grid_dep_wait();
     if (sw.exit_st >= 0 && lane == 0) {
         const unsigned long long cols32 = 32ull * (unsigned)ta.t_len - (32ull * (unsigned)sw.exit_st - 496ull);
         atomicAdd(&skipped[0], (unsigned long long)R * cols32);
@@ -654,16 +669,18 @@
 __global__ void __launch_bounds__(32 * kWarpsPerBlock, 1)
 pair_round2_kernel(const Pair2* __restrict__ pairs, Deal dl, const Task* __restrict__ tasks, RestArgs ra,
                    const uint32_t* __restrict__ pool, ScoreW scw, int* counter, int smem_stride, int4* out, u32* state,
-                   u32* kept) {
+                   u32* kept, NextBank nb) {
     extern __shared__ uint4 psmem[];
     const ScoreView<true> sc(scw);
     const int lane = threadIdx.x & 31, warp = threadIdx.x >> 5;
     uint4* prof = psmem + warp * smem_stride;
+    grid_dep_trigger();
     bool first = true;
     for (;;) {
         const int i = next_item(dl, first, counter);
         if (i < 0) break;
         if (i < ra.n_order) {
+            grid_dep_wait();
             const int e = ra.order[i];
             if (e & kPairEntry) {
                 const Pair2 mp = pairs[(e & ~kPairEntry) >> kCodeBits];
@@ -680,6 +697,7 @@
         pair2_dispatch<kMinR>(pair_rows(q), pt, tasks, pool, prof, lane, (u32)sc.one, sc.four, out, state,
                               reinterpret_cast<unsigned long long*>(counter + kExitSlot), kept);
     }
+    zero_next_bank(nb);
 }
 #endif
 
@@ -765,6 +783,7 @@
     __syncwarp();
     build_profile<R>(prof, qpool + ta.q_word, q_a, qpool + tb.q_word, q_b, lane * R, lane, false);
     __syncwarp();
+    grid_dep_wait();
     {
         Sweep<R, kPF> sw;
         sw.prof = prof; sw.twords = pool + reg.fwd_word; sw.t_len = reg.n_left + reg.m * kmax; sw.lane = lane;
@@ -894,16 +913,18 @@
                    const uint32_t* __restrict__ qpool, const uint32_t* __restrict__ pool,
                    const LadderRegion* __restrict__ regs, ScoreW scw, int* counter,
                    int smem_stride, uint2* prung, int4* out, int4* sel, int* redo_count, int32_t* redo,
-                   const u32* __restrict__ qstate) {
+                   const u32* __restrict__ qstate, NextBank nb) {
     extern __shared__ uint4 psmem[];
     const ScoreView<true> sc(scw);
     const int lane = threadIdx.x & 31, warp = threadIdx.x >> 5;
     uint4* prof = psmem + warp * smem_stride;
+    grid_dep_trigger();
     bool first = true;
     for (;;) {
         const int i = next_item(dl, first, counter);
         if (i < 0) break;
         if (i < ra.n_order) {
+            grid_dep_wait();
             const int e = ra.order[i];
             if (e & kPairEntry) {
                 const Pair3 mp = pairs[(e & ~kPairEntry) >> kCodeBits];
@@ -923,6 +944,7 @@
         }
         pair3_dispatch<kMinR>(rows, pt, tasks, qpool, pool, regs, prof, lane, (u32)sc.one, sc.four, sc.min_score, prung, sel, redo_count, redo, qstate);
     }
+    zero_next_bank(nb);
 }
 #endif
 
```
